# Ipsedo/MARLClassification

Measured on AMD Instinct MI355X. Metric: agent-env-steps/sec, higher is better.
Workload: dtype f32; 1 GPU; RESISC45 256x256x3, 16 agents, 16 steps, f=12, README dims (configs[2]); full train iteration: rollout + A2C loss + BPTT backward + Adam; batch_per_gpu=256, global_batch=256, parallelism=dp1, rng=library (Philox4x32-10), launch=eager

## Files before the change

include/marl_hip.h:

```cpp
#ifndef MARL_HIP_H
#define MARL_HIP_H

#include <stddef.h>
#include <stdint.h>

#ifdef __cplusplus
extern "C" {
#endif

#define MARL_ABI_VERSION 5

#define MARL_OK 0
#define MARL_EINVAL (-1)
#define MARL_ELIMIT (-2)
#define MARL_EHIP (-3)
#define MARL_ESIZE (-4)

#define MARL_COUNTERS_BYTES 32

#define MARL_MAX_CNN_LAYERS 5
#define MARL_MAX_ACTIONS 16

typedef struct marl_config {
    int32_t nb_agents;
// ... 55 lines not shown
int marl_graph_end(void* stream, void** graph_exec_out);
int marl_graph_launch(void* graph_exec, void* stream);
int marl_graph_destroy(void* graph_exec);

int marl_episode_forward(const marl_config* cfg, const void* weights_ws, size_t weights_ws_bytes,
                         void* episode_ws, size_t episode_ws_bytes,
                         const void* img, const int64_t* pos0,
                         const float* h0, const float* c0, const float* hc0, const float* cc0,
                         const float* noise, const int64_t* forced_actions,
                         uint64_t rng_seed, uint64_t rng_offset, const void* counters,
                         float* step_preds, float* step_logp, float* step_values,
                         int64_t* step_pos, int64_t* step_actions,
                         int train, void* stream);

int marl_episode_backward(const marl_config* cfg, void* weights_ws, size_t weights_ws_bytes,
                          void* episode_ws, size_t episode_ws_bytes,
                          const void* img, const float* g_preds, const float* g_logp,
                          const float* g_values, float* const* grads_host, void* stream);

int marl_episode_backward_img(const marl_config* cfg, void* weights_ws, size_t weights_ws_bytes,
                              void* episode_ws, size_t episode_ws_bytes,
                              const void* img, const float* g_preds, const float* g_logp,
                              const float* g_values, float* const* grads_host, float* d_img,
                              void* stream);

int marl_episode_forward_probs(const marl_config* cfg, const void* weights_ws, size_t weights_ws_bytes,
                               void* episode_ws, size_t episode_ws_bytes,
                               const void* img, const int64_t* pos0,
                               const float* h0, const float* c0, const float* hc0, const float* cc0,
                               const float* noise, const int64_t* forced_actions,
                               uint64_t rng_seed, uint64_t rng_offset, const void* counters,
                               float* step_preds, float* step_logp, float* step_values,
                               int64_t* step_pos, int64_t* step_actions, float* step_probs,
                               int train, void* stream);

int marl_episode_backward_probs(const marl_config* cfg, void* weights_ws, size_t weights_ws_bytes,
                                void* episode_ws, size_t episode_ws_bytes,
                                const void* img, const float* g_preds, const float* g_logp,
                                const float* g_values, float* const* grads_host, float* d_img,
                                const float* g_probs, void* stream);

int marl_backward_heads_event(void* hip_event);

int marl_comm_matrix(const float* m_dev, int nb_agents);

size_t marl_comm_grad_scratch_bytes(const marl_config* cfg);
int marl_comm_grad(const marl_config* cfg, const void* weights_ws, size_t weights_ws_bytes,
                   const void* ws, size_t ws_bytes, int nb_steps, float* d_comm,
                   void* scratch, size_t scratch_bytes, void* stream);

int marl_a2c_loss_fwd_bwd(const marl_config* cfg, void* episode_ws, size_t episode_ws_bytes,
                          const float* step_preds, const float* step_logp,
                          const float* step_values, const int64_t* y, float gamma,
                          float* g_preds, float* g_logp, float* g_values,
                          float* scalars_out, double* adv_stats, int phase, void* stream);

int marl_a2c_loss_entropy_fwd_bwd(const marl_config* cfg, void* episode_ws, size_t episode_ws_bytes,
                                  const float* step_preds, const float* step_logp,
                                  const float* step_values, const int64_t* y, float gamma,
                                  const float* step_probs, float entropy_coef,
                                  float* g_preds, float* g_logp, float* g_values, float* g_probs,
                                  float* scalars_out, double* adv_stats, int phase, void* stream);

int marl_advantages(const marl_config* cfg, void* episode_ws, size_t episode_ws_bytes,
                    const float* step_preds, const float* step_values, const int64_t* y,
                    float gamma, float lam, float* advn, float* ret, double* adv_stats, int phase,
                    void* stream);

int marl_ppo_loss_fwd_bwd(const marl_config* cfg, void* episode_ws, size_t episode_ws_bytes,
                          const float* step_preds, const float* step_logp, const float* step_values,
                          const int64_t* y, const float* old_logp, const float* advn, const float* ret,
                          float clip_eps, const float* step_probs, float entropy_coef,
                          float* g_preds, float* g_logp, float* g_values, float* g_probs,
                          float* scalars_out, void* stream);

#define MARL_GRAD_CLIP_BLOCKS 1024
#define MARL_GRAD_CLIP_SCRATCH_BYTES (MARL_GRAD_CLIP_BLOCKS * 8)
int marl_grad_clip(float* grads, int64_t n, float max_norm, float grad_scale, float* norm_out,
                   void* scratch, size_t scratch_bytes, void* stream);

int marl_adam_step(float* params, const float* grads, float* exp_avg, float* exp_avg_sq,
                   int64_t n, int64_t step, float lr, float beta1, float beta2, float eps,
                   float grad_scale, const void* counters, void* stream);

int marl_step_forward(const marl_config* cfg, const void* weights_ws, size_t weights_ws_bytes,
                      void* episode_ws, size_t episode_ws_bytes,
                      const float* obs, const float* msg, const float* norm_pos,
                      const float* h, const float* c, const float* hc, const float* cc,
                      float* probs, float* values, float* preds, float* new_msg,
                      float* h_out, float* c_out, float* hc_out, float* cc_out,
                      const float* noise, uint64_t rng_seed, uint64_t rng_offset,
                      int64_t* actions_out, float* logp_out, void* stream);

int marl_step_forward_train(const marl_config* cfg, const void* weights_ws, size_t weights_ws_bytes,
                            void* step_ws, size_t step_ws_bytes,
                            const float* obs, const float* msg, const float* norm_pos,
                            const float* h, const float* c, const float* hc, const float* cc,
                            float* probs, float* values, float* preds, float* new_msg,
                            float* h_out, float* c_out, float* hc_out, float* cc_out,
                            const float* noise, uint64_t rng_seed, uint64_t rng_offset,
                            int64_t* actions_out, float* logp_out, void* stream);

int marl_step_backward(const marl_config* cfg, void* weights_ws, size_t weights_ws_bytes,
                       void* step_ws, size_t step_ws_bytes, const float* obs,
                       const float* g_probs, const float* g_logp, const float* g_values,
                       const float* g_preds, const float* g_msg, const float* g_h, const float* g_c,
                       const float* g_hc, const float* g_cc, float* const* grads_host,
                       float* d_msg, float* d_h, float* d_c, float* d_hc, float* d_cc, void* stream);

int marl_normalize_positions(const int64_t* pos, float* out, int rows, int h, int w, void* stream);

int marl_gemm_nt(const float* a, int lda, const float* b, int ldb, const float* bias,
                 float* c, int ldc, int m, int n, int k, int accumulate, void* stream);
int marl_gemm_nt_weights(const float* a, int lda, const float* b, int ldb, const float* bias,
                         float* c, int ldc, int m, int n, int k, int accumulate,
                         void* image_scratch, void* stream);
size_t marl_gemm_weight_image_bytes(int n, int k);
int marl_gemm_tn(const float* a, int lda, const float* b, int ldb, float* c, int ldc,
                 int ni, int nj, int64_t rows, float* scratch, size_t scratch_bytes, void* stream);
size_t marl_gemm_tn_scratch(int ni, int nj, int64_t rows);
size_t marl_image_bytes(int64_t rows, int k);
int marl_image_build(const float* src, int ld, int64_t rows, int k, void* image, void* stream);
int marl_gemm_nt_images(const void* a3, const void* b3, const float* bias, float* c, int ldc, int m, int n,
                        int k, int accumulate, int variant, void* stream);
int marl_gemm_nt_images_batch(int count, const void* const* a3, const void* const* b3, float* const* c,
                              const int* n, const int* ldc, int m, int k, int accumulate, int variant,
                              void* stream);
int marl_lstm_images(const void* u3, int nin, const void* h3, const void* wih3, const void* whh3,
                     const float* bias, const float* c_prev, float* h_next, float* c_next, float* gates,
                     void* h3_next, int m, int n, int ld_state, int ld_gates, int variant, int cells,
                     void* stream);
size_t marl_gemm_tn_images_scratch(int ni, int nj, int64_t rows);
int marl_gemm_tn_images(const void* a3, const void* b3, float* c, int ldc, int ni, int nj, int64_t rows,
                        float* colsum, float* scratch, size_t scratch_bytes, void* stream);
size_t marl_gemm_tn_images_cell_scratch(int ni, int nih, int nhh, int64_t rows);
int marl_gemm_tn_images_cell(const void* g3, int ni, const void* u3, int nih, const void* h3, int nhh, int64_t rows,
                             float* c_ih, int ld_ih, float* c_hh, int ld_hh, float* colsum, float* scratch,
                             size_t scratch_bytes, void* stream);
int marl_ln_silu_fwd(const float* z, int ldz, const float* gamma, const float* beta,
                     float* out, int ldo, float* stats, int m, int n, void* stream);

int marl_cnn_wgrad(const float* dz, const void* img, int img_u8, const int32_t* pos,
                   const float* zin, const float* gst, const float* gamma, const float* beta,
                   int64_t rows, int nb, int c_img, int h, int w, int cin, int cout, int hin,
                   int groups, float* dw, float* db, float* scratch, size_t scratch_bytes,
                   void* stream);
size_t marl_cnn_wgrad_scratch(int64_t rows, int cin, int cout, int hin, int groups, int first);

int marl_tune(const char* key, int value);
int marl_tune_get(const char* key, int dflt);

int marl_profile_begin(int kernel_class, int max_launches);
int marl_profile_end(double* total_ms, int* launches);

int marl_debug_buffer(const marl_config* cfg, int train, const char* name, int t,
                      int64_t* offset_floats, int* ld);

int marl_plan_query(const marl_config* cfg, int train, const char* key, int* value);

#ifdef __cplusplus
}
#endif
#endif
```

marlclassification_amd/_lib.py:

```python

from __future__ import annotations

import ctypes as C
import os
from typing import Optional

MARL_MAX_CNN_LAYERS = 5
MARL_MAX_ACTIONS = 16
MARL_ABI_VERSION = 5
MARL_COUNTERS_BYTES = 32
MARL_GRAD_CLIP_SCRATCH_BYTES = 1024 * 8

_HERE = os.path.dirname(os.path.abspath(__file__))
LIB_PATH = os.environ.get("MARL_LIB_PATH") or os.path.join(_HERE, "csrc", "libmarl_hip.so")


class MarlConfig(C.Structure):

    _fields_ = [
        ("nb_agents", C.c_int32),
        ("batch", C.c_int32),
        ("nb_steps", C.c_int32),
        ("img_c", C.c_int32),
        ("img_h", C.c_int32),
        ("img_w", C.c_int32),
        ("window", C.c_int32),
        ("cnn_layers", C.c_int32),
        ("cnn_ch", C.c_int32 * (MARL_MAX_CNN_LAYERS + 1)),
        ("cnn_groups", C.c_int32 * MARL_MAX_CNN_LAYERS),
        ("n_b", C.c_int32),
        ("n_a", C.c_int32),
        ("n_m", C.c_int32),
        ("n_m_o", C.c_int32),
        ("n_d", C.c_int32),
        ("nb_action", C.c_int32),
        ("nb_class", C.c_int32),
        ("nlb", C.c_int32),
        ("nla", C.c_int32),
        ("actions", (C.c_int32 * 2) * MARL_MAX_ACTIONS),
        ("img_u8", C.c_int32),
    ]


_NAMES = (
    "POS_W POS_B POS_LNW POS_LNB "
    "ENC_W0 ENC_B0 ENC_LN0W ENC_LN0B ENC_W1 ENC_B1 ENC_LN1W ENC_LN1B "
    "DEC_W0 DEC_B0 DEC_LN0W DEC_LN0B DEC_W1 DEC_B1 DEC_LN1W DEC_LN1B "
    "LB_WIH LB_WHH LB_BIH LB_BHH LA_WIH LA_WHH LA_BIH LA_BHH "
    "POL_W0 POL_B0 POL_LNW POL_LNB POL_W1 POL_B1 "
    "CRI_W0 CRI_B0 CRI_LNW CRI_LNB CRI_W1 CRI_B1 "
    "PRE_W0 PRE_B0 PRE_LNW PRE_LNB PRE_W1 PRE_B1"
).split()
P = {name: 20 + i for i, name in enumerate(_NAMES)}
MARL_NPARAMS = 20 + len(_NAMES)

EXPORTS = (
    "marl_abi_version marl_last_error marl_param_numel marl_workspace_sizes marl_pack_weights "
    "marl_patch_gather marl_transition marl_episode_forward marl_episode_backward "
    "marl_a2c_loss_fwd_bwd marl_adam_step marl_step_forward marl_gemm_nt marl_gemm_tn "
    "marl_gemm_tn_scratch marl_gemm_nt_weights marl_gemm_weight_image_bytes marl_ln_silu_fwd marl_debug_buffer "
    "marl_profile_begin marl_profile_end marl_normalize_positions "
    "marl_cnn_wgrad marl_cnn_wgrad_scratch marl_tune marl_tune_get marl_draw_episode "
    "marl_counters_set marl_counters_tick marl_graph_begin marl_graph_end marl_graph_launch "
    "marl_graph_destroy marl_image_bytes marl_image_build marl_gemm_nt_images marl_gemm_nt_images_batch "
    "marl_lstm_images marl_gemm_tn_images marl_gemm_tn_images_scratch marl_plan_query "
    "marl_gemm_tn_images_cell marl_gemm_tn_images_cell_scratch marl_backward_heads_event "
    "marl_step_forward_train marl_step_backward marl_episode_backward_img "
    "marl_episode_forward_probs marl_episode_backward_probs marl_a2c_loss_entropy_fwd_bwd "
    "marl_advantages marl_ppo_loss_fwd_bwd marl_grad_clip marl_comm_matrix "
    "marl_comm_grad marl_comm_grad_scratch_bytes"
).split()

_lib: Optional[C.CDLL] = None

_vp, _i, _i64, _f, _sz = C.c_void_p, C.c_int, C.c_int64, C.c_float, C.c_size_t
_u64 = C.c_uint64
_cfgp = C.POINTER(MarlConfig)


def _declare(lib: C.CDLL) -> None:
    lib.marl_abi_version.restype = _i
    lib.marl_last_error.restype = C.c_char_p
    lib.marl_param_numel.restype = _i64
    lib.marl_param_numel.argtypes = [_cfgp, _i]
    lib.marl_workspace_sizes.argtypes = [_cfgp, _i, C.POINTER(_sz), C.POINTER(_sz)]
    lib.marl_pack_weights.argtypes = [_cfgp, C.POINTER(_vp), _vp, _sz, _vp]
    lib.marl_patch_gather.argtypes = [_vp, _vp, _vp, _i, _i, _i, _i, _i, _i, _vp]
    lib.marl_transition.argtypes = [_vp, _vp, _vp, C.POINTER(C.c_int32), _i, _i, _i, _i, _i, _vp]
    lib.marl_episode_forward.argtypes = ([_cfgp, _vp, _sz, _vp, _sz] + [_vp] * 8 + [_u64, _u64, _vp] + [_vp] * 5 +
                                         [_i, _vp])
    lib.marl_episode_forward_probs.argtypes = ([_cfgp, _vp, _sz, _vp, _sz] + [_vp] * 8 + [_u64, _u64, _vp] +
                                               [_vp] * 6 + [_i, _vp])
    lib.marl_draw_episode.argtypes = [_cfgp, _u64, _u64, _vp] + [_vp] * 7
    lib.marl_counters_set.argtypes = [_vp, _u64, _i64, _f, _f, _f, _vp]
    lib.marl_counters_tick.argtypes = [_vp, _f, _f, _f, _vp]
    lib.marl_graph_begin.argtypes = [_vp]
    lib.marl_graph_end.argtypes = [_vp, C.POINTER(_vp)]
    lib.marl_graph_launch.argtypes = [_vp, _vp]
    lib.marl_graph_destroy.argtypes = [_vp]
    lib.marl_episode_backward.argtypes = [_cfgp, _vp, _sz, _vp, _sz, _vp, _vp, _vp, _vp, C.POINTER(_vp), _vp]
    lib.marl_episode_backward_img.argtypes = ([_cfgp, _vp, _sz, _vp, _sz, _vp, _vp, _vp, _vp, C.POINTER(_vp), _vp,
                                               _vp])
    lib.marl_episode_backward_probs.argtypes = ([_cfgp, _vp, _sz, _vp, _sz, _vp, _vp, _vp, _vp, C.POINTER(_vp), _vp,
                                                 _vp, _vp])
    lib.marl_a2c_loss_entropy_fwd_bwd.argtypes = (
        [_cfgp, _vp, _sz, _vp, _vp, _vp, _vp, _f, _vp, _f, _vp, _vp, _vp, _vp, _vp, _vp, _i, _vp]
    )
    lib.marl_a2c_loss_fwd_bwd.argtypes = (
        [_cfgp, _vp, _sz, _vp, _vp, _vp, _vp, _f, _vp, _vp, _vp, _vp, _vp, _i, _vp]
    )
    lib.marl_advantages.argtypes = [_cfgp, _vp, _sz, _vp, _vp, _vp, _f, _f, _vp, _vp, _vp, _i, _vp]
    lib.marl_ppo_loss_fwd_bwd.argtypes = ([_cfgp, _vp, _sz] + [_vp] * 7 + [_f, _vp, _f] + [_vp] * 6)
    lib.marl_grad_clip.argtypes = [_vp, _i64, _f, _f, _vp, _vp, _sz, _vp]
    lib.marl_adam_step.argtypes = [_vp, _vp, _vp, _vp, _i64, _i64, _f, _f, _f, _f, _f, _vp, _vp]
    lib.marl_step_forward.argtypes = ([_cfgp, _vp, _sz, _vp, _sz] + [_vp] * 15 + [_vp, _u64, _u64, _vp, _vp] +
                                      [_vp])
    lib.marl_step_forward_train.argtypes = lib.marl_step_forward.argtypes
    lib.marl_step_backward.argtypes = [_cfgp, _vp, _sz, _vp, _sz] + [_vp] * 10 + [C.POINTER(_vp)] + [_vp] * 6
    lib.marl_normalize_positions.argtypes = [_vp, _vp, _i, _i, _i, _vp]
    lib.marl_gemm_nt.argtypes = [_vp, _i, _vp, _i, _vp, _vp, _i, _i, _i, _i, _i, _vp]
    lib.marl_gemm_nt_weights.argtypes = [_vp, _i, _vp, _i, _vp, _vp, _i, _i, _i, _i, _i, _vp, _vp]
    lib.marl_gemm_weight_image_bytes.restype = _sz
    lib.marl_gemm_weight_image_bytes.argtypes = [_i, _i]
    lib.marl_gemm_tn.argtypes = [_vp, _i, _vp, _i, _vp, _i, _i, _i, _i64, _vp, _sz, _vp]
    lib.marl_gemm_tn_scratch.restype = _sz
    lib.marl_gemm_tn_scratch.argtypes = [_i, _i, _i64]
    lib.marl_ln_silu_fwd.argtypes = [_vp, _i, _vp, _vp, _vp, _i, _vp, _i, _i, _vp]
    lib.marl_image_bytes.restype = _sz
    lib.marl_image_bytes.argtypes = [_i64, _i]
    lib.marl_image_build.argtypes = [_vp, _i, _i64, _i, _vp, _vp]
    lib.marl_gemm_nt_images.argtypes = [_vp, _vp, _vp, _vp, _i, _i, _i, _i, _i, _i, _vp]
    lib.marl_gemm_nt_images_batch.argtypes = [_i, C.POINTER(_vp), C.POINTER(_vp), C.POINTER(_vp), C.POINTER(_i),
                                              C.POINTER(_i), _i, _i, _i, _i, _vp]
    lib.marl_gemm_tn_images_scratch.restype = _sz
    lib.marl_gemm_tn_images_scratch.argtypes = [_i, _i, _i64]
    lib.marl_gemm_tn_images.argtypes = [_vp, _vp, _vp, _i, _i, _i, _i64, _vp, _vp, _sz, _vp]
    lib.marl_lstm_images.argtypes = [_vp, _i] + [_vp] * 9 + [_i] * 6 + [_vp]
    lib.marl_cnn_wgrad.argtypes = ([_vp, _vp, _i, _vp, _vp, _vp, _vp, _vp, _i64] + [_i] * 8 +
                                   [_vp, _vp, _vp, _sz, _vp])
    lib.marl_cnn_wgrad_scratch.restype = _sz
    lib.marl_cnn_wgrad_scratch.argtypes = [_i64, _i, _i, _i, _i, _i]
    lib.marl_tune.argtypes = [C.c_char_p, _i]
    lib.marl_tune_get.argtypes = [C.c_char_p, _i]
    lib.marl_profile_begin.argtypes = [_i, _i]
    lib.marl_profile_end.argtypes = [C.POINTER(C.c_double), C.POINTER(_i)]
    lib.marl_debug_buffer.argtypes = [_cfgp, _i, C.c_char_p, _i, C.POINTER(_i64), C.POINTER(_i)]
    lib.marl_gemm_tn_images_cell_scratch.restype = _sz
    lib.marl_gemm_tn_images_cell_scratch.argtypes = [_i, _i, _i, _i64]
    lib.marl_gemm_tn_images_cell.argtypes = [_vp, _i, _vp, _i, _vp, _i, _i64, _vp, _i, _vp, _i, _vp, _vp, _sz, _vp]
    lib.marl_plan_query.argtypes = [_cfgp, _i, C.c_char_p, C.POINTER(_i)]
    lib.marl_backward_heads_event.argtypes = [_vp]
    lib.marl_comm_matrix.argtypes = [_vp, _i]
    lib.marl_comm_grad_scratch_bytes.restype = _sz
    lib.marl_comm_grad_scratch_bytes.argtypes = [_cfgp]
    lib.marl_comm_grad.argtypes = [_cfgp, _vp, _sz, _vp, _sz, _i, _vp, _vp, _sz, _vp]
    for name in EXPORTS:
        fn = getattr(lib, name)
        if fn.restype is C.c_int and name not in ("marl_abi_version", "marl_tune_get"):
            fn.restype = _i


def load() -> C.CDLL:
    global _lib
    if _lib is not None:
        return _lib
    if not os.path.exists(LIB_PATH):
        raise RuntimeError(
            f"{LIB_PATH} is missing: the HIP library is the only implementation of this "
            "package (no CPU fallback). Build it with `make -C marlclassification_amd/csrc` "
            "or `python -c 'import __graft_entry__ as g; g.build()'`."
        )
    lib = C.CDLL(LIB_PATH)
    missing = [s for s in EXPORTS if not hasattr(lib, s)]
    if missing:
        raise RuntimeError(f"{LIB_PATH} lacks symbols {missing}")
    _declare(lib)
    if lib.marl_abi_version() != MARL_ABI_VERSION:
        raise RuntimeError("libmarl_hip.so ABI version mismatch; rebuild it")
    _lib = lib
    return lib


def check(rc: int) -> None:
    if rc != 0:
        msg = load().marl_last_error().decode("utf-8", "replace")
        raise RuntimeError(f"libmarl_hip error {rc}: {msg}")
```

marlclassification_amd/csrc/common.h:

```cpp
#pragma once

#include <hip/hip_runtime.h>
#include <stdint.h>
#include <stdio.h>

#include "../../include/marl_hip.h"
#include "split.h"

namespace marl {

constexpr int kWave = 64;

inline int p4(int x) { return (x + 3) & ~3; }
inline int64_t cdiv(int64_t a, int64_t b) { return (a + b - 1) / b; }

void set_error(const char* fmt, ...);

int tune_get(const char* key, int dflt);
int tune_set(const char* key, int value);

__device__ __forceinline__ float rcp_fast(float x) { return __builtin_amdgcn_rcpf(x); }
__device__ __forceinline__ float sigmoid_acc(float x) { return rcp_fast(1.0f + __expf(-x)); }
__device__ __forceinline__ float tanh_fast(float x) { return 1.0f - 2.0f * rcp_fast(1.0f + __expf(2.0f * x)); }
__device__ __forceinline__ float silu_fast(float y) { return y * sigmoid_acc(y); }
// ... 6 lines not shown
    int x = __float_as_int(v);
#define MARL_DPP_ADD(ctrl, rmask)                         \
    x = __float_as_int(__int_as_float(x) +                \
                       __int_as_float(__builtin_amdgcn_update_dpp(0, x, ctrl, rmask, 0xf, false)))
    MARL_DPP_ADD(0x111, 0xf);
    MARL_DPP_ADD(0x112, 0xf);
    MARL_DPP_ADD(0x114, 0xf);
    MARL_DPP_ADD(0x118, 0xf);
    MARL_DPP_ADD(0x142, 0xa);
    MARL_DPP_ADD(0x143, 0xc);
#undef MARL_DPP_ADD
    return __int_as_float(__builtin_amdgcn_readlane(x, 63));
}

#define MARL_HIP_CHECK(expr)                                                        \
    do {                                                                            \
        hipError_t e_ = (expr);                                                     \
        if (e_ != hipSuccess) {                                                     \
            marl::set_error("%s failed: %s (%s:%d)", #expr, hipGetErrorString(e_),  \
                            __FILE__, __LINE__);                                    \
            return MARL_EHIP;                                                       \
        }                                                                           \
    } while (0)

#define MARL_LAUNCH_CHECK() MARL_HIP_CHECK(hipGetLastError())

#define MARL_TRY(expr)             \
    do {                           \
        int rc_ = (expr);          \
        if (rc_ != MARL_OK) return rc_; \
    } while (0)

struct GemmSeg {
    const float* a;
    const float* b;
    int lda, ldb, k;
    const void* b3;
    int kt3;
};

struct GemmProb {
    GemmSeg seg[2];
    int nseg;
    int m, n;
    float* c;
    int ldc;
    const float* bias;
    int accumulate;
    const float* c_prev;
    float* h_next;
    float* c_next;
    float* gates;
    int ld_state, ld_gates;
};

constexpr int kMaxGemmBatch = 4;
struct GemmBatch {
    GemmProb p[kMaxGemmBatch];
    int count;
    int gx, gy;
    int xcd_map;
    int single_buf;
#ifdef MARL_KERNEL_TS
    long long* ts;
#endif
};

__device__ __forceinline__ void xcd_tile(unsigned gx, unsigned gy, unsigned gz, unsigned& bx,
                                         unsigned& by, unsigned& bz) {
    const unsigned T = gx * gy * gz, L = blockIdx.x;
    const unsigned per = T >> 3, rem = T & 7, xcd = L & 7, slot = L >> 3;
    const unsigned q = (xcd < rem ? xcd * (per + 1) : rem * (per + 1) + (xcd - rem) * per) + slot;
    bz = q / (gx * gy);
    const unsigned r = q - bz * gx * gy;
    bx = r / gy;
    by = r - bx * gy;
}
int xcd_map_enabled();

GemmProb gemm_prob(const float* a, int lda, const float* b, int ldb, int k, float* c, int ldc,
                   int m, int n, const float* bias = nullptr, int accumulate = 0);
void gemm_add_seg(GemmProb& p, const float* a, int lda, const float* b, int ldb, int k);

int launch_gemm_nt(const GemmBatch& batch, hipStream_t st);
int launch_gemm_lstm(const GemmBatch& batch, hipStream_t st);

int split_mode();
size_t split_image_floats(int rows, int k);
struct SplitDesc {
    const float* src;
    void* dst;
    int rows, k, ld, kt;
};
constexpr int kMaxSplitDesc = 64;
struct SplitBatch {
    SplitDesc d[kMaxSplitDesc];
    int count;
};
int launch_split_weights(const SplitBatch& b, hipStream_t st);
void split_registry_reset();
void split_registry_add(const float* base, int rows, int ld, int k, const void* image);
struct SplitRegistryScope {
    SplitRegistryScope() = default;
    SplitRegistryScope(const SplitRegistryScope&) = delete;
    ~SplitRegistryScope() { split_registry_reset(); }
};
int launch_gemm_nt_split(const GemmBatch& batch, int max_m, int max_n, int64_t blocks128, hipStream_t st);
int launch_gemm_lstm_split(const GemmBatch& batch, int max_m, int max_n, hipStream_t st);
int launch_gemm_tn_split(const float* a, int lda, const float* b, int ldb, float* out, int ldo,
                         int64_t stride, int ni, int nj, int64_t rows, int64_t rows_per_split,
                         float* csum, dim3 grid, int gx, int gy, int gz, hipStream_t st);

struct G3Seg {
    const char* a3;
    const char* b3;
    int a_row0, b_row0;
    int steps;
};
struct G3Prob {
    G3Seg seg[2];
    int nseg;
    int m, n;
    float* c;
    int ldc;
    const float* bias;
    int accumulate;
    const float* c_prev;
    float* h_next;
    float* c_next;
    float* gates;
    int ld_state, ld_gates;
    char* h3;
    int h3_row0, h3_steps;
};
constexpr int kMaxG3 = 4;
struct G3Batch {
    G3Prob p[kMaxG3];
    int count;
    int gx, gy, xcd_map;
    int safe;
#ifdef MARL_G3_ABLATE
    long long* clk;
#endif
};
G3Prob g3_prob(const void* a3, int a_row0, const void* b3, int b_row0, int k, float* c, int ldc, int m, int n,
               const float* bias = nullptr, int accumulate = 0);
void g3_add_seg(G3Prob& p, const void* a3, int a_row0, const void* b3, int b_row0, int k);
int launch_gemm_nt3(const G3Batch& batch, hipStream_t st, int variant = 0);
int launch_gemm_lstm3(const G3Batch& batch, hipStream_t st, int variant = 0);
int g3_lstm_plan(const G3Batch& batch);
struct G3TnArgs {
    const char* a3;
    const char* b3;
    int a_steps, b_steps;
    int a_row0, b_row0;
    float* out;
    int ldo;
    int64_t out_split_stride;
    int ni, nj;
    int64_t rows, rows_per_split;
    float* csum;
    int gx, gy, gz, safe;
    int j_first;
#ifdef MARL_G3_ABLATE
    int abl;
#endif
};
struct G3TnPlan {
    int variant, splits;
    int64_t rows_per_split;
};
G3TnPlan g3_tn_plan(int ni, int nj, int64_t rows);
constexpr int kMaxTnCell = 4;
struct G3TnCell {
    G3TnArgs t[kMaxTnCell];
    int nt, n256;
    int gx, gz;
    int teams;
};
bool g3_tn_cell_ok(int ni, int nj_ih, int nj_hh, int64_t rows);
G3TnPlan g3_tn_cell_plan(int ni, int nj_ih, int nj_hh, int64_t rows);
size_t g3_tn_cell_scratch_bytes(int ni, int nj_ih, int nj_hh, int64_t rows);
int launch_gemm_tn3_cell(G3TnArgs ih, G3TnArgs hh, const G3TnPlan& plan, hipStream_t st);
size_t g3_tn_scratch_bytes(int ni, int nj, int64_t rows);
int launch_gemm_tn3(G3TnArgs a, const G3TnPlan& plan, hipStream_t st);

struct ImgDesc {
    const float* src;
    void* dst;
    int64_t rows;
    int k, ld;
};
constexpr int kMaxImgDesc = 64;
struct ImgBatch {
    ImgDesc d[kMaxImgDesc];
    int count;
};
int launch_images(const ImgBatch& b, hipStream_t st);

constexpr int kProfClasses = 6;
void prof_before(int cls, hipStream_t st);
void prof_after(int cls, hipStream_t st);
int profile_begin(int cls, int max_launches);
int profile_end(double* total_ms, int* launches);

struct RedQueue;
size_t gemm_tn_scratch_bytes(int ni, int nj, int64_t rows);
struct TnQueue;
int launch_gemm_tn(const float* a, int lda, const float* b, int ldb, float* c, int ldc, int ni,
                   int nj, int64_t rows, float* scratch, size_t scratch_bytes, hipStream_t st,
                   float* colsum_out = nullptr, RedQueue* q = nullptr, TnQueue* tq = nullptr);

struct TnBatchProb {
    const float* a;
    const float* b;
    float* out;
    float* csum;
    int64_t stride, rows, rows_per_split;
    int lda, ldb, ldo, ni, nj, gx, gy, first_block;
};
constexpr int kMaxTnBatch = 12;
struct TnBatch {
    TnBatchProb p[kMaxTnBatch];
    int count;
};
struct TnQueue {
    struct Item {
        const float* a;
        const float* b;
        float* c;
        float* colsum;
// ... 43 lines not shown
                       float* dot_out = nullptr);
int ln_bwd_blocks(int64_t m, int n);
int launch_ln_silu_bwd_rank(const float* g, int ldg, int kin, const float* bt, int ldbt,
                            const float* z, int ldz, const float* stats, const float* gamma,
                            const float* beta, float* dz, int lddz, float* part, int64_t m, int n,
                            hipStream_t st);
int launch_ln_silu_bwd(const float* da, int ldda, const float* z, int ldz, const float* stats,
                       const float* gamma, const float* beta, float* dz, int lddz, float* part,
                       int64_t m, int n, hipStream_t st);
int launch_reduce_affine(float* part, int64_t nparts, int n, float* dgamma, float* dbeta,
                         int accumulate, hipStream_t st, RedQueue* q = nullptr);

int gn_fwd_im2col_supported(int P, int C);
int launch_gn_silu_fwd(const float* z, const float* gamma, const float* beta, float* out,
                       int64_t ldo, int out_chw, float* stats, int64_t rows, int P, int C, int G,
                       hipStream_t st, float* cols = nullptr, int ldk = 0, int hin = 0);
int gn_bwd_blocks(int64_t rows, int C);
int launch_gn_silu_bwd(const float* da, int64_t ldda, int da_chw, const float* z,
                       const float* stats, const float* gamma, const float* beta, float* dz,
                       float* part, int64_t rows, int P, int C, int G, hipStream_t st);

int launch_agg_msg(const float* m, float* out, int ld, int na, int nb, int n, hipStream_t st);
int launch_mix_msg(const float* m, float* out, int ld, int na, int nb, int n, const float* mix, int transpose,
                   hipStream_t st);
int mix_msg_max_agents();
int comm_grad_blocks(int64_t pairs, int* per_out);
int comm_grad_supported(int na, int n, int n2, int ldw);
int launch_comm_grad(const float* dz, int lddz, const float* msg, int ldmsg, const float* w, int ldw, int na, int nb,
                     int steps, int n2, int n, float* part, float* out, hipStream_t st);

int launch_pos_embed_fwd(const int32_t* pos, const float* npos_in, int h, int w, const float* W, const float* b,
                         const float* gamma, const float* beta, float* npos4, float* z, int ldz,
                         float* stats, float* out, int ldo, int64_t rows, int nd, hipStream_t st);

int launch_lstm_cell_bwd(const float* dh, int lddh, float* dc, int lddc, float* gates, int ldg,
                         const float* c_prev, const float* c_new, int ldc, int64_t rows, int n,
                         hipStream_t st);
struct LstmBwdBatch;
int launch_lstm_cell_bwd_batch(LstmBwdBatch& b, int count, hipStream_t st);
int launch_lstm_cell_bwd2(const float* dh0, int lddh0, float* dc0, int lddc0, float* gates0,
                          int ldg0, const float* cp0, const float* cn0, int ldc0, int n0,
                          const float* dh1, int lddh1, float* dc1, int lddc1, float* gates1,
                          int ldg1, const float* cp1, const float* cn1, int ldc1, int n1,
                          int64_t rows, hipStream_t st);

struct SampleArgs {
    const float* a_pol;
    int ld_a, nla;
    const float* w1;
    int ldw;
    const float* b1;
    const float* noise;
    uint64_t rng_seed, rng_ctr;
    const uint64_t* rng_off_dev;
    int rng_on;
    const int64_t* forced;
    const int32_t* pos_in;
    int32_t* pos_out;
    int64_t* step_pos;
    int64_t* step_actions;
    float* step_logp;
    float* probs;
    int32_t* actions_i32;
    int R, nA, H, W, f;
    int32_t table[MARL_MAX_ACTIONS][2];
    const float* pe_W;
    const float* pe_b;
    const float* pe_gamma;
    const float* pe_beta;
    float* pe_npos;
    float* pe_z;
    float* pe_stats;
    float* pe_out;
    int pe_ldz, pe_ldo, pe_nd;
    char* pe_img;
    int pe_row0, pe_steps, pe_col0;
};
int launch_sample(const SampleArgs& a, hipStream_t st);

int launch_draw_episode(uint64_t seed, uint64_t offset, const uint64_t* offset_dev, int64_t* pos0,
                        int R, int H, int W, int f, float* h0, float* c0, int n_b, float* hc0,
                        float* cc0, int n_a, float* noise, int64_t n_noise, hipStream_t st);

struct PermDesc {
    const float* src;
    float* dst;
    int rows, cols;
    int dst_ld;
    int rd, rs1, rs2;
    int cd, cs1, cs2;
    const float* src2;
};
constexpr int kMaxPerm = 56;
struct PermBatch {
    PermDesc d[kMaxPerm];
    int count;
};
int launch_permute(const PermBatch& b, hipStream_t st);

struct Counters {
    uint64_t rng_offset;
    uint64_t step;
    float lr_over_bc1;
    float inv_sqrt_bc2;
    float pad[2];
};
static_assert(sizeof(Counters) == MARL_COUNTERS_BYTES, "counter block layout");
int launch_counters_set(Counters* c, uint64_t rng_offset, int64_t step, float lr, float beta1,
                        float beta2, int tick, hipStream_t st);

int launch_adam(float* p, const float* g, float* m, float* v, int64_t n, float lr_over_bc1,
                float inv_sqrt_bc2, float beta1, float beta2, float eps, float grad_scale,
                hipStream_t st, const Counters* cnt = nullptr);

int launch_fill(float* p, int64_t n, float v, hipStream_t st);
int launch_add2d(const float* a, int64_t lda, const float* b, int64_t ldb, float* out, int64_t ldo,
                 int64_t rows, int cols, hipStream_t st);
int launch_copy2d(const float* src, int64_t lds, float* dst, int64_t ldd, int64_t rows, int cols,
                  hipStream_t st);
int launch_i64_to_i32(const int64_t* src, int32_t* dst, int64_t n, hipStream_t st);
int launch_policy_dlogits(const float* dlogp, const float* probs, const int32_t* actions,
                          float* out, int ld, int64_t rows, int nA, hipStream_t st);
int launch_policy_dlogits_probs(const float* dlogp, const float* dprobs, const float* probs,
                                const int32_t* actions, float* out, int ld, int64_t rows, int nA,
                                hipStream_t st);
int launch_acc2d(float* dst, int64_t ldd, const float* src, int64_t lds, int64_t rows, int cols,
                 hipStream_t st);
int launch_rowdot(const float* a, int lda, const float* w, const float* b, float* out,
                  int64_t rows, int n, hipStream_t st);

struct PanelLayer {
    const float* w;
    int ldw;
    const float* bias;
    const float* gamma;
    const float* beta;
    int n;
    float* z;
    int ldz;
    float* stats;
    float* a;
    int lda;
    char* a3;
    int a3_row0, a3_steps, a3_col0;
};
constexpr int kPanelMaxLayers = 4;
struct PanelFwdProb {
    const float* x;
    int ldx, k0;
    int agg_na, agg_nb;
    float* xbar;
    int m, nlayers;
    PanelLayer layer[kPanelMaxLayers];
    int by_batch, g_na, g_nb, agg_at, ld_xbar;
    const float* mix;
};
struct PanelFwdBatch {
    PanelFwdProb p[2];
    int count;
    int off_panel1, off_red, off_part, off_prm;
    int off_mix;
    int has_sample, panel_blocks;
    int epi_prob;
    int ln_narrow_max;
    SampleArgs sample;
#ifdef MARL_KERNEL_TS
    long long* ts;
#endif
};
int panel_chain_supported(int na, int n_msg, int threads);
int panel_supported(int k0, int n0, int n1);
int panel_sample_supported(int n_actions);
int launch_panel_fwd(PanelFwdBatch& b, hipStream_t st);

struct LstmBwdArgs {
    const float* dh;
    float* dc;
    float* gates;
    const float* c_prev;
    const float* c_new;
    int lddh, lddc, ldg, ldc, n;
// ... 312 lines not shown
```

marlclassification_amd/csrc/episode.hip:

```cpp
#include <math.h>
#include <stdlib.h>
#include <string.h>

#include "common.h"

namespace marl {

struct Dims {
    int na, nb, ns;
    int64_t R, NR;
    int H, W, c_img, f;
    int L;
    int ch[MARL_MAX_CNN_LAYERS + 1];
    int grp[MARL_MAX_CNN_LAYERS];
    int hw[MARL_MAX_CNN_LAYERS + 1];
    int P[MARL_MAX_CNN_LAYERS];
    int K[MARL_MAX_CNN_LAYERS];
    int ldk[MARL_MAX_CNN_LAYERS];
    int nf, nin;
    int n_b, n_a, n_m, nm2, n_mo, n_d, nA, nC, nlb, nla;
    int ld_nin, ld_nb, ld_na, ld_nm, ld_nm2, ld_nmo, ld_nd, ld_nla, ld_nlb, ld_gb, ld_ga, ld_nC,
        ld_nA;
    int ld_dbl;
};
// ... 814 lines not shown
    pe.x = c.Hs(t + 1);
    pe.ldx = d.ld_nb;
    pe.k0 = d.n_b;
    pe.m = (int)d.R;
    pe.nlayers = 2;
    pe.layer[0] = PanelLayer{c.wp(MARL_P_ENC_W0), d.ld_nb, c.wp(MARL_P_ENC_B0),
                             c.wp(MARL_P_ENC_LN0W), c.wp(MARL_P_ENC_LN0B), d.nm2,
                             keep ? c.at(c.e.ZE1, t) : nullptr, d.ld_nm2,
                             keep ? c.at(c.e.STE1, t) : nullptr, c.at(c.e.AE1, t), d.ld_nm2};
    pe.layer[1] = PanelLayer{c.wp(MARL_P_ENC_W1), d.ld_nm2, c.wp(MARL_P_ENC_B1),
                             c.wp(MARL_P_ENC_LN1W), c.wp(MARL_P_ENC_LN1B), d.n_m,
                             keep ? c.at(c.e.ZE2, t) : nullptr, d.ld_nm,
                             keep ? c.at(c.e.STE2, t) : nullptr, c.MSGs(t + 1), d.ld_nm};
}
static void fill_pol_prob(const Ctx& c, int t, PanelFwdProb& pp) {
    const Dims& d = c.d;
    const bool keep = c.train != 0;
    pp.x = c.HCs(t + 1);
    pp.ldx = d.ld_na;
    pp.k0 = d.n_a;
    pp.m = (int)d.R;
    pp.nlayers = 1;
    pp.layer[0] = PanelLayer{c.wp(MARL_P_POL_W0), d.ld_na, c.wp(MARL_P_POL_B0),
                             c.wp(MARL_P_POL_LNW), c.wp(MARL_P_POL_LNB), d.nla,
                             keep ? c.at(c.e.ZP1, t) : nullptr, d.ld_nla,
                             keep ? c.at(c.e.STP1, t) : nullptr, c.at(c.e.AP1, t), d.ld_nla};
}

static int step_encode_policy(const Ctx& c, int t, int which) {
    const Dims& d = c.d;
    const int R = (int)d.R;
    hipStream_t st = c.st;
    if (use_panels(d)) {
        PanelFwdBatch pb{};
        pb.count = 0;
        if (which & 1) fill_enc_prob(c, t, pb.p[pb.count++]);
        if (which & 2) fill_pol_prob(c, t, pb.p[pb.count++]);
        return launch_panel_fwd(pb, st);
    }
    if (which == 3) {
        MARL_TRY(gemm2(c,
                       gemm_prob(c.Hs(t + 1), d.ld_nb, c.wp(MARL_P_ENC_W0), d.ld_nb, d.n_b,
                                 c.at(c.e.ZE1, t), d.ld_nm2, R, d.nm2, c.wp(MARL_P_ENC_B0)),
                       gemm_prob(c.HCs(t + 1), d.ld_na, c.wp(MARL_P_POL_W0), d.ld_na, d.n_a,
                                 c.at(c.e.ZP1, t), d.ld_nla, R, d.nla, c.wp(MARL_P_POL_B0))));
    } else if (which == 1) {
        MARL_TRY(gemm1(c, gemm_prob(c.Hs(t + 1), d.ld_nb, c.wp(MARL_P_ENC_W0), d.ld_nb, d.n_b,
                                    c.at(c.e.ZE1, t), d.ld_nm2, R, d.nm2, c.wp(MARL_P_ENC_B0))));
    } else {
        MARL_TRY(gemm1(c, gemm_prob(c.HCs(t + 1), d.ld_na, c.wp(MARL_P_POL_W0), d.ld_na, d.n_a,
                                    c.at(c.e.ZP1, t), d.ld_nla, R, d.nla, c.wp(MARL_P_POL_B0))));
    }
    if (which & 2)
        MARL_TRY(launch_ln_silu_fwd(c.at(c.e.ZP1, t), d.ld_nla, c.wp(MARL_P_POL_LNW),
                                    c.wp(MARL_P_POL_LNB), c.at(c.e.AP1, t), d.ld_nla,
                                    c.at(c.e.STP1, t), d.R, d.nla, st));
    if (which & 1) {
        MARL_TRY(launch_ln_silu_fwd(c.at(c.e.ZE1, t), d.ld_nm2, c.wp(MARL_P_ENC_LN0W),
                                    c.wp(MARL_P_ENC_LN0B), c.at(c.e.AE1, t), d.ld_nm2,
                                    c.at(c.e.STE1, t), d.R, d.nm2, st));
        MARL_TRY(gemm1(c, gemm_prob(c.at(c.e.AE1, t), d.ld_nm2, c.wp(MARL_P_ENC_W1), d.ld_nm2,
                                    d.nm2, c.at(c.e.ZE2, t), d.ld_nm, R, d.n_m,
                                    c.wp(MARL_P_ENC_B1))));
        MARL_TRY(launch_ln_silu_fwd(c.at(c.e.ZE2, t), d.ld_nm, c.wp(MARL_P_ENC_LN1W),
                                    c.wp(MARL_P_ENC_LN1B), c.MSGs(t + 1), d.ld_nm,
                                    c.at(c.e.STE2, t), d.R, d.n_m, st));
    }
    return MARL_OK;
}

static bool use_chain(const Dims& d) {
    return use_panels(d) && panel_chain_supported(d.na, d.n_m, 256) && d.n_mo <= 384 && d.nm2 <= 384 &&
           d.n_m <= 384 && tune_get("panel_chain", 1) != 0 &&
           (!g_comm || d.n_b <= 384);
}
static bool use_panel_sample(const Dims& d) {
    static int enabled = -1;
    if (enabled < 0) {
        const char* e = getenv("MARL_PANEL_SAMPLE");
        enabled = (e && e[0] == '0') ? 0 : 1;
    }
    return enabled && panel_sample_supported(d.nA);
}
static int step_chain(const Ctx& c, int t, const SampleArgs* sample = nullptr) {
    const Dims& d = c.d;
    PanelFwdBatch pb{};
    pb.count = 2;
    PanelFwdProb& pe = pb.p[0];
    fill_enc_prob(c, t, pe);
    pe.by_batch = panel_chain_by_batch(d.na);
    pe.g_na = d.na;
    pe.g_nb = d.nb;
    if (t + 1 < d.ns) {
        fill_dec_layers(c, t + 1, pe.layer + 2);
        pe.nlayers = 4;
        pe.agg_at = 2;
        pe.xbar = c.at(c.e.MBAR, t + 1);
        pe.ld_xbar = d.ld_nm;
        pe.mix = g_comm;
    }
    fill_pol_prob(c, t, pb.p[1]);
    if (sample && use_panel_sample(d)) {
        pb.epi_prob = 2;
        pb.sample = *sample;
    }
    return launch_panel_fwd(pb, c.st);
}

static int step_core(const Ctx& c, int t, const StepIn& in) {
    MARL_TRY(step_cnn(c, t, in));
    MARL_TRY(step_decode(c, t));
    MARL_TRY(step_pos_lstm(c, t, in));
    return step_encode_policy(c, t, 3);
}

struct SideStream {
    hipStream_t s = nullptr;
    hipEvent_t ev[64];
    int next = 0;
    int init() {
        if (s) return MARL_OK;
        MARL_HIP_CHECK(hipStreamCreateWithFlags(&s, hipStreamNonBlocking));
        for (auto& e : ev) MARL_HIP_CHECK(hipEventCreateWithFlags(&e, hipEventDisableTiming));
        return MARL_OK;
    }
    int order(hipStream_t from, hipStream_t to) {
        hipEvent_t e = ev[next];
        next = (next + 1) % 64;
        MARL_HIP_CHECK(hipEventRecord(e, from));
        MARL_HIP_CHECK(hipStreamWaitEvent(to, e, 0));
        return MARL_OK;
    }
};
static SideStream g_side;

static bool use_side_stream() {
    static int enabled = -1;
    (void)enabled;
    return false;
}

static int heads_batched(const Ctx& c, int t0, int64_t rows, float* values, float* preds) {
    const Dims& d = c.d;
    hipStream_t st = c.st;
    if (c.e.g3 && tune_get("g3_lstm", 1) != 0) {
        const int r1 = (int)((int64_t)(t0 + 1) * d.R);
        G3Batch g{};
        g.p[0] = g3_prob(c.img(c.e.HC3), r1, c.wp3k(MARL_P_CRI_W0), 0, d.n_a, c.at(c.e.ZC1), d.ld_nla, (int)rows, d.nla,
                         c.wp(MARL_P_CRI_B0));
        g.p[1] = g3_prob(c.img(c.e.H3), r1, c.wp3k(MARL_P_PRE_W0), 0, d.n_b, c.at(c.e.ZQ1), d.ld_nlb, (int)rows, d.nlb,
                         c.wp(MARL_P_PRE_B0));
        g.count = 2;
        MARL_TRY(launch_gemm_nt3(g, st));
    } else
    MARL_TRY(gemm2(c,
                   gemm_prob(c.HCs(t0 + 1), d.ld_na, c.wp(MARL_P_CRI_W0), d.ld_na, d.n_a,
                             c.at(c.e.ZC1), d.ld_nla, (int)rows, d.nla, c.wp(MARL_P_CRI_B0)),
                   gemm_prob(c.Hs(t0 + 1), d.ld_nb, c.wp(MARL_P_PRE_W0), d.ld_nb, d.n_b,
                             c.at(c.e.ZQ1), d.ld_nlb, (int)rows, d.nlb, c.wp(MARL_P_PRE_B0))));
    const bool vdot = d.nla <= 384;
    MARL_TRY(launch_ln_silu_fwd(c.at(c.e.ZC1), d.ld_nla, c.wp(MARL_P_CRI_LNW), c.wp(MARL_P_CRI_LNB),
                                c.at(c.e.AC1), d.ld_nla, c.at(c.e.STC1), rows, d.nla, st,
                                vdot ? c.wp(MARL_P_CRI_W1) : nullptr, c.wp(MARL_P_CRI_B1), values));
    MARL_TRY(launch_ln_silu_fwd(c.at(c.e.ZQ1), d.ld_nlb, c.wp(MARL_P_PRE_LNW), c.wp(MARL_P_PRE_LNB),
                                c.at(c.e.AQ1), d.ld_nlb, c.at(c.e.STQ1), rows, d.nlb, st));
    if (!vdot)
// ... 69 lines not shown
static int load_state(const Ctx& c, const float* h, const float* cc_, const float* hc,
                      const float* cca, const float* msg) {
    const Dims& d = c.d;
    PermQueue q(c.st);
    q.push(copy_desc(h, d.n_b, c.Hs(0), d.ld_nb, d.R, d.n_b));
    q.push(copy_desc(cc_, d.n_b, c.Cs(0), d.ld_nb, d.R, d.n_b));
    q.push(copy_desc(hc, d.n_a, c.HCs(0), d.ld_na, d.R, d.n_a));
    q.push(copy_desc(cca, d.n_a, c.CCs(0), d.ld_na, d.R, d.n_a));
    q.push(copy_desc(msg, d.n_m, c.MSGs(0), d.ld_nm, d.R, msg ? d.n_m : d.ld_nm));
    q.flush();
    MARL_TRY(q.rc);
    if (c.e.g3) {
        ImgBatch ib{};
        ib.d[0] = ImgDesc{h, c.img(c.e.H3), d.R, d.n_b, d.n_b};
        ib.d[1] = ImgDesc{hc, c.img(c.e.HC3), d.R, d.n_a, d.n_a};
        ib.count = 2;
        MARL_TRY(launch_images(ib, c.st));
    }
    return MARL_OK;
}


static int pack_weights(const Dims& d, const WLayout& w, const float* const* params, float* W,
                        hipStream_t st) {
    PermQueue q(st);
    for (int i = 0; i < MARL_NPARAMS; ++i) {
        const ParamMeta m = param_meta(d, i);
        if (m.kind == PK_NONE) continue;
        const float* src = params[i];
        if (!src) {
            set_error("parameter %d is null", i);
            return MARL_EINVAL;
        }
        if (m.kind == PK_MATRIX) {
            q.push(perm(src, W + w.wp[i], m.n, m.k, w.ldp[i], 1, m.k, 0, 1, 1, 0));
            q.push(perm(src, W + w.wt[i], m.k, m.n, w.ldt[i], 1, 1, 0, 1, m.k, 0));
        } else if (m.kind == PK_CONV) {
            const int ci = m.k / 9;
            q.push(perm(src, W + w.wp[i], m.n, m.k, w.ldp[i], 1, m.k, 0, ci, 1, 9));
            q.push(perm(src, W + w.wt[i], m.k, m.n, w.ldt[i], ci, 1, 9, 1, m.k, 0));
        } else {
            q.push(perm(src, W + w.wp[i], 1, m.n, m.n, 1, 0, 0, 1, 1, 0));
        }
    }
    q.push(perm(params[MARL_P_LB_BIH], W + w.bsum_b, 1, 4 * d.n_b, 4 * d.n_b, 1, 0, 0, 1, 1, 0,
                params[MARL_P_LB_BHH]));
    q.push(perm(params[MARL_P_LA_BIH], W + w.bsum_a, 1, 4 * d.n_a, 4 * d.n_a, 1, 0, 0, 1, 1, 0,
                params[MARL_P_LA_BHH]));
    q.flush();
    MARL_TRY(q.rc);
    for (int i = 0; i < MARL_NPARAMS; ++i) {
        const ParamMeta m = param_meta(d, i);
        if (!w.wf[i]) continue;
        const int steps = m.k / 16;
        q.push(perm(W + w.wp[i], W + w.wf[i], (m.n / 16) * steps * 4, 64, 64, steps * 4, 16 * w.ldp[i], 4, 4,
                    w.ldp[i], 1));
    }
    q.flush();
    MARL_TRY(q.rc);
    SplitBatch sb{};
    sb.count = 0;
    for (int i = 0; i < MARL_NPARAMS; ++i) {
        const ParamMeta m = param_meta(d, i);
        if (m.kind != PK_MATRIX) continue;
        sb.d[sb.count++] = SplitDesc{W + w.wp[i], W + w.wp3[i], m.n, m.k, w.ldp[i], (m.k + 31) / 32};
        sb.d[sb.count++] = SplitDesc{W + w.wt[i], W + w.wt3[i], m.k, m.n, w.ldt[i], (m.n + 31) / 32};
    }
    MARL_TRY(launch_split_weights(sb, st));
    ImgBatch ib{};
    ib.count = 0;
    for (int i = 0; i < MARL_NPARAMS; ++i) {
        const ParamMeta m = param_meta(d, i);
        if (m.kind != PK_MATRIX || !w.wp3k[i]) continue;
        if (ib.count + 2 > kMaxImgDesc) {
            MARL_TRY(launch_images(ib, st));
            ib.count = 0;
        }
        ib.d[ib.count++] = ImgDesc{W + w.wp[i], W + w.wp3k[i], m.n, m.k, w.ldp[i]};
        ib.d[ib.count++] = ImgDesc{W + w.wt[i], W + w.wt3k[i], m.k, m.n, w.ldt[i]};
    }
    return launch_images(ib, st);
}

static void register_split_images(const Dims& d, const WLayout& w, const float* W) {
    split_registry_reset();
    for (int i = 0; i < MARL_NPARAMS; ++i) {
        const ParamMeta m = param_meta(d, i);
        if (m.kind != PK_MATRIX) continue;
        split_registry_add(W + w.wp[i], m.n, w.ldp[i], m.k, W + w.wp3[i]);
        split_registry_add(W + w.wt[i], m.k, w.ldt[i], m.n, W + w.wt3[i]);
    }
}

static int unpack_grads(const Ctx& c, float* const* grads, int which = 0) {
    PermQueue q(c.st);
    for (int i = 0; i < MARL_NPARAMS; ++i) {
        const bool head = i >= MARL_P_POL_W0 && i <= MARL_P_PRE_B1;
        if ((which == 1 && !head) || (which == 2 && head)) continue;
        const ParamMeta m = param_meta(c.d, i);
        if (m.kind == PK_MATRIX) {
            q.push(perm(c.gp(i), grads[i], m.n, m.k, m.k, 1, c.w.ldp[i], 0, 1, 1, 0));
        } else if (m.kind == PK_CONV) {
            const int ci = m.k / 9;
            q.push(perm(c.gp(i), grads[i], m.n, m.k, m.k, 1, c.w.ldp[i], 0, 9, 1, ci));
        }
    }
    if (which != 1) {
        q.push(perm(grads[MARL_P_LB_BIH], grads[MARL_P_LB_BHH], 1, 4 * c.d.n_b, 4 * c.d.n_b, 1, 0, 0, 1, 1, 0));
        q.push(perm(grads[MARL_P_LA_BIH], grads[MARL_P_LA_BHH], 1, 4 * c.d.n_a, 4 * c.d.n_a, 1, 0, 0, 1, 1, 0));
    }
    q.flush();
    return q.rc;
}

static int tn(const Ctx& c, const float* a, int lda, const float* b, int ldb, int pidx, int ni,
              int nj, int64_t rows, float* bias = nullptr) {
    RedQueue* q = c.defer_this(gemm_tn_scratch_bytes(ni, nj, rows)) ? c.rq : nullptr;
    return launch_gemm_tn(a, lda, b, ldb, c.gp(pidx), c.w.ldp[pidx], ni, nj, rows, c.at(c.e.TNS),
                          c.e.tns_bytes, c.st, bias, q, q ? c.tq : nullptr);
}
static int tn3(const Ctx& c, const char* a3, int ni, const char* b3, int nj, int pidx, int64_t rows, float* bias) {
    const G3TnPlan plan = g3_tn_plan(ni, nj, rows);
    if (g3_tn_scratch_bytes(ni, nj, rows) > c.e.tns_bytes) {
        set_error("tn3: scratch too small");
        return MARL_ESIZE;
    }
    float* scratch = c.at(c.e.TNS);
    G3TnArgs a{};
    a.a3 = a3;
    a.b3 = b3;
    a.a_steps = img_steps(ni);
    a.b_steps = img_steps(nj);
    a.out = scratch;
    a.ldo = nj;
    a.out_split_stride = (int64_t)ni * nj;
    a.ni = ni;
    a.nj = nj;
    a.rows = rows;
    a.csum = bias ? scratch + (size_t)plan.splits * ni * nj : nullptr;
    MARL_TRY(launch_gemm_tn3(a, plan, c.st));
    return launch_slab_reduce(scratch, (int64_t)ni * nj, plan.splits, c.gp(pidx), c.w.ldp[pidx], ni, nj, a.csum, bias, c.st);
}
static int tn3_cell(const Ctx& c, const char* g3, int ni, const char* u3, int nin, int p_ih, const char* h3, int nh,
                    int p_hh, int64_t rows, float* bias) {
    const G3TnPlan plan = g3_tn_cell_plan(ni, nin, nh, rows);
    if (g3_tn_cell_scratch_bytes(ni, nin, nh, rows) > c.e.tns_bytes) {
        set_error("tn3_cell: scratch too small");
        return MARL_ESIZE;
    }
    float* s_ih = c.at(c.e.TNS);
    float* s_hh = s_ih + (size_t)plan.splits * ni * nin;
    float* s_cs = s_hh + (size_t)plan.splits * ni * nh;
    G3TnArgs ih{}, hh{};
    ih.a3 = hh.a3 = g3;
    ih.a_steps = hh.a_steps = img_steps(ni);
    ih.ni = hh.ni = ni;
    ih.rows = hh.rows = rows;
    ih.b3 = u3;
    ih.b_steps = img_steps(nin);
    ih.nj = ih.ldo = nin;
    ih.out = s_ih;
    ih.out_split_stride = (int64_t)ni * nin;
    ih.csum = bias ? s_cs : nullptr;
    hh.b3 = h3;
    hh.b_steps = img_steps(nh);
    hh.nj = hh.ldo = nh;
// ... 129 lines not shown
                                    c.at(c.e.DAP1), d.ld_nla, (int)NR, d.nla)));
        MARL_TRY(ln_bwd(c, c.at(c.e.DAP1), d.ld_nla, c.at(c.e.ZP1, 0), d.ld_nla, c.at(c.e.STP1, 0),
                        MARL_P_POL_LNW, MARL_P_POL_LNB, NR, d.nla, grads, 0));
    }
    MARL_TRY(tn(c, c.at(c.e.DAP1), d.ld_nla, c.HCs(1), d.ld_na, MARL_P_POL_W0, d.nla, d.n_a, NR, grads[MARL_P_POL_B0]));
    {
        GemmProb ph = gemm_prob(c.at(c.e.DAQ1), d.ld_nlb, c.wt(MARL_P_PRE_W0), d.ld_nlb, d.nlb,
                                c.DHs(1), d.ld_nb, (int)NR, d.n_b);
        GemmProb pa = gemm_prob(c.at(c.e.DAP1), d.ld_nla, c.wt(MARL_P_POL_W0), d.ld_nla, d.nla,
                                c.DHCs(1), d.ld_na, (int)NR, d.n_a);
        gemm_add_seg(pa, c.at(c.e.DAC1), d.ld_nla, c.wt(MARL_P_CRI_W0), d.ld_nla, d.nla);
        MARL_TRY(gemm2(c, ph, pa));
    }
    if (sb) {
        MARL_TRY(launch_acc2d(c.DHs(ns), d.ld_nb, sb->g_h, d.n_b, d.R, d.n_b, st));
        MARL_TRY(launch_acc2d(c.DHCs(ns), d.ld_na, sb->g_hc, d.n_a, d.R, d.n_a, st));
    }

    const bool heads_early = g_heads_event != nullptr && !sb;
    if (heads_early) {
        if (c.tq) MARL_TRY(launch_tn_queue(tq, c.rq, st));
        MARL_TRY(rq.flush());
        MARL_TRY(unpack_grads(c, grads, 1));
        MARL_HIP_CHECK(hipEventRecord(g_heads_event, st));
    }

    const size_t s_nmo = (size_t)d.R * d.ld_dbl, s_nm2 = (size_t)d.R * d.ld_nm2,
                 s_nm = (size_t)d.R * d.ld_nm;
    const bool panels = use_panels(d) && d.n_mo <= 384 && d.nm2 <= 384 && d.n_m <= 384;
    if (!panels) {
        MARL_TRY(launch_tn_queue(tq, c.rq, st));
        c.rq = nullptr;
        c.tq = nullptr;
    }
    const bool enc_last = sb && sb->g_msg;
    if (enc_last) {
        const int t = ns - 1;
        float* dze2 = c.at(c.e.DZE2) + (size_t)t * s_nm;
        float* dae1 = c.at(c.e.DAE1) + (size_t)t * s_nm2;
        MARL_TRY(launch_copy2d(sb->g_msg, d.n_m, dze2, d.ld_nm, d.R, d.n_m, st));
        MARL_TRY(ln_bwd(c, dze2, d.ld_nm, c.at(c.e.ZE2, t), d.ld_nm, c.at(c.e.STE2, t), MARL_P_ENC_LN1W,
                        MARL_P_ENC_LN1B, d.R, d.n_m, grads, 0));
        MARL_TRY(gemm1(c, gemm_prob(dze2, d.ld_nm, c.wt(MARL_P_ENC_W1), p4(d.n_m), d.n_m, dae1, d.ld_nm2, R,
                                    d.nm2)));
        MARL_TRY(ln_bwd(c, dae1, d.ld_nm2, c.at(c.e.ZE1, t), d.ld_nm2, c.at(c.e.STE1, t), MARL_P_ENC_LN0W,
                        MARL_P_ENC_LN0B, d.R, d.nm2, grads, 0));
        MARL_TRY(gemm1(c, gemm_prob(dae1, d.ld_nm2, c.wt(MARL_P_ENC_W0), p4(d.nm2), d.nm2, c.DHs(ns), d.ld_nb, R,
                                    d.n_b, nullptr, 1)));
    }
    const bool ride = panels && !use_side_stream();
    const bool dl_in_loop = ride;
    bool action_done = false;
    bool belief_done = false;
    const bool chain = ride && use_chain(d);
    const bool g3 = c.e.g3;
    const int skip_f32 = g3 && dl_in_loop && g3_tn_enabled(d);
    const int pln_blocks = chain ? panel_chain_blocks(d.na, d.nb) : panel_bwd_blocks(R);
    for (int t = ns - 1; t >= 0; --t) {
        const int first = (t == ns - 1);
        {
            LstmBwdBatch lb{};
            int nc = 0;
            if (!belief_done)
                lb.a[nc++] = LstmBwdArgs{c.DHs(t + 1), c.at(c.e.DC), c.at(c.e.GB, t), c.Cs(t), c.Cs(t + 1), d.ld_nb,
                                         d.ld_nb, d.ld_gb, d.ld_nb, d.n_b, g3 ? c.img(c.e.GB3) : nullptr,
                                         (int)((int64_t)t * d.R), img_steps(4 * d.n_b), skip_f32};
            if (!action_done)
                lb.a[nc++] = LstmBwdArgs{c.DHCs(t + 1), c.at(c.e.DCC), c.at(c.e.GA, t), c.CCs(t), c.CCs(t + 1), d.ld_na,
                                         d.ld_na, d.ld_ga, d.ld_na, d.n_a, g3 ? c.img(c.e.GA3) : nullptr,
                                         (int)((int64_t)t * d.R), img_steps(4 * d.n_a), skip_f32};
            lb.rows = d.R;
            if (nc) MARL_TRY(launch_lstm_cell_bwd_batch(lb, nc, st));
        }
        action_done = belief_done = false;
        const bool side = panels && use_side_stream();
        Ctx cs = c;
        if (side) {
            MARL_TRY(g_side.init());
            cs.st = g_side.s;
            MARL_TRY(g_side.order(c.st, cs.st));
        }
        hipStream_t st = cs.st;
        float* ddbar = c.at(c.e.DDBAR) + (size_t)t * s_nmo;
        {
            GemmBatch gb{};
            gb.p[0] = gemm_prob(c.at(c.e.GB, t), d.ld_gb, c.wt(MARL_P_LB_WHH), d.ld_gb, 4 * d.n_b,
                                c.DHs(t), d.ld_nb, R, d.n_b, nullptr, 1);
            gb.p[1] = gemm_prob(c.at(c.e.GA, t), d.ld_ga, c.wt(MARL_P_LA_WHH), d.ld_ga, 4 * d.n_a,
                                c.DHCs(t), d.ld_na, R, d.n_a, nullptr, 1);
            GemmProb p = gemm_prob(c.at(c.e.GB, t), d.ld_gb,
                                   c.wt(MARL_P_LB_WIH) + (size_t)d.nf * d.ld_gb, d.ld_gb, 4 * d.n_b,
                                   ddbar, d.ld_dbl, R, d.n_mo);
            gemm_add_seg(p, c.at(c.e.GA, t), d.ld_ga, c.wt(MARL_P_LA_WIH) + (size_t)d.nf * d.ld_ga,
                         d.ld_ga, 4 * d.n_a);
            if (side) {
                gb.count = 2;
                MARL_TRY(launch_gemm_nt(gb, c.st));
                MARL_TRY(gemm1(cs, p));
            } else if (dl_in_loop) {
                gb.p[2] = gemm_prob(c.at(c.e.GB, t), d.ld_gb,
                                    c.wt(MARL_P_LB_WIH) + (size_t)d.nf * d.ld_gb, d.ld_gb, 4 * d.n_b,
                                    ddbar, d.ld_dbl, R, d.n_mo + d.n_d);
                gb.p[3] = gemm_prob(c.at(c.e.GA, t), d.ld_ga,
                                    c.wt(MARL_P_LA_WIH) + (size_t)d.nf * d.ld_ga, d.ld_ga, 4 * d.n_a,
                                    c.at(c.e.DDBAR2) + (size_t)t * s_nmo, d.ld_dbl, R, d.n_mo + d.n_d);
                gb.count = 4;
                if (g3) {
                    const int r0 = (int)((int64_t)t * d.R);
                    G3Batch g{};
                    g.p[0] = g3_prob(c.img(c.e.GB3), r0, c.wt3k(MARL_P_LB_WHH), 0, 4 * d.n_b, c.DHs(t), d.ld_nb, R,
                                     d.n_b, nullptr, 1);
                    g.p[1] = g3_prob(c.img(c.e.GA3), r0, c.wt3k(MARL_P_LA_WHH), 0, 4 * d.n_a, c.DHCs(t), d.ld_na, R,
                                     d.n_a, nullptr, 1);
                    g.p[2] = g3_prob(c.img(c.e.GB3), r0, c.wt3k(MARL_P_LB_WIH), d.nf, 4 * d.n_b, ddbar, d.ld_dbl, R,
                                     d.n_mo + d.n_d);
                    g.p[3] = g3_prob(c.img(c.e.GA3), r0, c.wt3k(MARL_P_LA_WIH), d.nf, 4 * d.n_a,
                                     c.at(c.e.DDBAR2) + (size_t)t * s_nmo, d.ld_dbl, R, d.n_mo + d.n_d);
                    g.count = 4;
                    MARL_TRY(launch_gemm_nt3(g, c.st));
                } else {
                    MARL_TRY(launch_gemm_nt(gb, c.st));
                }
            } else {
                gb.p[2] = p;
                gb.count = 3;
                MARL_TRY(launch_gemm_nt(gb, c.st));
            }
        }
        float* dad1 = c.at(c.e.DAD1) + (size_t)t * s_nm2;
        if (panels) {
            const size_t pblk = (size_t)pln_blocks * 2;
            PanelBwdProb pd{};
            pd.da = ddbar;
            pd.ldda = d.ld_dbl;
            if (dl_in_loop) {
                pd.da2 = c.at(c.e.DDBAR2) + (size_t)t * s_nmo;
                pd.ldda2 = d.ld_dbl;
            }
            pd.m = R;
            pd.nlayers = 2;
            pd.layer[0] = PanelBwdLayer{c.at(c.e.ZD2, t), d.ld_nmo, c.at(c.e.STD2, t),
                                        c.wp(MARL_P_DEC_LN1W), c.wp(MARL_P_DEC_LN1B), d.n_mo, ddbar,
                                        d.ld_dbl, c.at(c.e.PLN[0]) + (size_t)t * pblk * d.n_mo,
                                        c.wt(MARL_P_DEC_W1), p4(d.n_mo), d.nm2};
            pd.layer[1] = PanelBwdLayer{c.at(c.e.ZD1, t), d.ld_nm2, c.at(c.e.STD1, t),
                                        c.wp(MARL_P_DEC_LN0W), c.wp(MARL_P_DEC_LN0B), d.nm2, dad1,
                                        d.ld_nm2, c.at(c.e.PLN[1]) + (size_t)t * pblk * d.nm2,
                                        c.wt(MARL_P_DEC_W0), p4(d.nm2), d.n_m};
            pd.dx = c.at(c.e.DMBAR);
            pd.lddx = d.ld_nm;
            pd.accumulate = 0;
            if (ride && t > 0) {
                pd.has_cell = 1;
                pd.cell = LstmBwdArgs{c.DHCs(t), c.at(c.e.DCC), c.at(c.e.GA, t - 1), c.CCs(t - 1),
                                      c.CCs(t), d.ld_na, d.ld_na, d.ld_ga, d.ld_na, d.n_a,
                                      g3 ? c.img(c.e.GA3) : nullptr, (int)((int64_t)(t - 1) * d.R), img_steps(4 * d.n_a),
                                      skip_f32};
                pd.cell_rows = d.R;
                action_done = true;
            }
            if (chain) {
                pd.by_batch = panel_chain_by_batch(d.na);
                pd.g_na = d.na;
                pd.g_nb = d.nb;
                if (t > 0) {
                    pd.nlayers = 4;
                    pd.agg_at = 2;
                    pd.mix = g_comm;
                    pd.layer[2] = PanelBwdLayer{c.at(c.e.ZE2, t - 1), d.ld_nm, c.at(c.e.STE2, t - 1),
                                                c.wp(MARL_P_ENC_LN1W), c.wp(MARL_P_ENC_LN1B), d.n_m,
                                                c.at(c.e.DZE2) + (size_t)(t - 1) * s_nm, d.ld_nm,
                                                c.at(c.e.PLN[2]) + (size_t)(t - 1) * pblk * d.n_m,
                                                c.wt(MARL_P_ENC_W1), p4(d.n_m), d.nm2};
                    pd.layer[3] = PanelBwdLayer{c.at(c.e.ZE1, t - 1), d.ld_nm2, c.at(c.e.STE1, t - 1),
                                                c.wp(MARL_P_ENC_LN0W), c.wp(MARL_P_ENC_LN0B), d.nm2,
                                                c.at(c.e.DAE1) + (size_t)(t - 1) * s_nm2, d.ld_nm2,
                                                c.at(c.e.PLN[3]) + (size_t)(t - 1) * pblk * d.nm2,
                                                c.wt(MARL_P_ENC_W0), p4(d.nm2), d.n_b};
                    pd.dx = c.DHs(t);
                    pd.lddx = d.ld_nb;
                    pd.accumulate = 1;
                    pd.has_cellb = 1;
                    pd.cellb = LstmBwdArgs{c.DHs(t), c.at(c.e.DC), c.at(c.e.GB, t - 1), c.Cs(t - 1), c.Cs(t),
                                           d.ld_nb, d.ld_nb, d.ld_gb, d.ld_nb, d.n_b, g3 ? c.img(c.e.GB3) : nullptr,
                                           (int)((int64_t)(t - 1) * d.R), img_steps(4 * d.n_b), skip_f32};
                    belief_done = true;
                }
                MARL_TRY(launch_panel_bwd(pd, st));
                MARL_TRY(gate_image_fallback(c, pd, t - 1));
                continue;
            }
            MARL_TRY(launch_panel_bwd(pd, st));
            MARL_TRY(gate_image_fallback(c, pd, t - 1));
            if (t > 0) {
                float* dze2 = c.at(c.e.DZE2) + (size_t)(t - 1) * s_nm;
                float* dae1 = c.at(c.e.DAE1) + (size_t)(t - 1) * s_nm2;
                PanelBwdProb pe{};
                pe.da = c.at(c.e.DMBAR);
                pe.ldda = d.ld_nm;
                pe.agg_na = d.na;
                pe.agg_nb = d.nb;
                if (g_comm) {
                    MARL_TRY(launch_mix_msg(c.at(c.e.DMBAR), c.at(c.e.DMBAR), d.ld_nm, d.na, d.nb, d.ld_nm, g_comm,
                                            1, st));
                    pe.agg_na = pe.agg_nb = 0;
                }
                pe.m = R;
                pe.nlayers = 2;
                pe.layer[0] = PanelBwdLayer{c.at(c.e.ZE2, t - 1), d.ld_nm, c.at(c.e.STE2, t - 1),
// ... 297 lines not shown
    }
    WLayout w;
    make_wlayout(d, w);
    if (weights_ws_bytes < w.total * sizeof(float)) {
        set_error("pack_weights: weights workspace too small (%zu of %zu bytes)", weights_ws_bytes,
                  w.total * sizeof(float));
        return MARL_ESIZE;
    }
    return pack_weights(d, w, params_host, static_cast<float*>(weights_ws),
                        static_cast<hipStream_t>(stream));
}

int marl_patch_gather(const float* img, const int64_t* pos, float* obs, int nb_agents, int batch,
                      int c, int h, int w, int f, void* stream) {
    if (!img || !pos || !obs || nb_agents < 1 || batch < 1 || c < 1 || f < 1 || h < f || w < f) {
        set_error("patch_gather: bad argument");
        return MARL_EINVAL;
    }
    return launch_patch_gather(img, pos, obs, nb_agents, batch, c, h, w, f,
                               static_cast<hipStream_t>(stream));
}

}

namespace marl {
__global__ void transition_kernel(const int64_t* __restrict__ pos_in,
                                  const int64_t* __restrict__ actions,
                                  int64_t* __restrict__ pos_out, SampleArgs tbl, int rows, int nA,
                                  int H, int W, int f) {
    const int r = blockIdx.x * blockDim.x + threadIdx.x;
    if (r >= rows) return;
    int a = (int)actions[r];
    a = a < 0 ? 0 : (a >= nA ? nA - 1 : a);
    const int64_t p0 = pos_in[r * 2], p1 = pos_in[r * 2 + 1];
    const int64_t q0 = p0 + tbl.table[a][0], q1 = p1 + tbl.table[a][1];
    const bool ok = q0 >= 0 && q0 + f < H && q1 >= 0 && q1 + f < W;
    pos_out[r * 2] = ok ? q0 : p0;
    pos_out[r * 2 + 1] = ok ? q1 : p1;
}
}

extern "C" {

int marl_transition(const int64_t* pos_in, const int64_t* actions, int64_t* pos_out,
                    const int32_t* table_host, int nb_action, int rows, int h, int w, int f,
                    void* stream) {
    if (!pos_in || !actions || !pos_out || !table_host || nb_action < 1 ||
        nb_action > MARL_MAX_ACTIONS || rows < 1) {
        set_error("transition: bad argument");
        return MARL_EINVAL;
    }
    SampleArgs tbl;
    memset(&tbl, 0, sizeof(tbl));
    for (int j = 0; j < nb_action; ++j) {
        tbl.table[j][0] = table_host[2 * j];
        tbl.table[j][1] = table_host[2 * j + 1];
    }
    hipLaunchKernelGGL(transition_kernel, dim3((unsigned)cdiv(rows, 256)), dim3(256), 0,
                       static_cast<hipStream_t>(stream), pos_in, actions, pos_out, tbl, rows,
                       nb_action, h, w, f);
    MARL_LAUNCH_CHECK();
    return MARL_OK;
}

static int episode_forward_all(const marl_config* cfg, const void* weights_ws, size_t weights_ws_bytes,
                               void* episode_ws, size_t episode_ws_bytes, const void* img, const int64_t* pos0,
                               const float* h0, const float* c0, const float* hc0, const float* cc0,
                               const float* noise, const int64_t* forced_actions, uint64_t rng_seed,
                               uint64_t rng_offset, const void* counters, float* step_preds, float* step_logp,
                               float* step_values, int64_t* step_pos, int64_t* step_actions, float* step_probs,
                               int train, void* stream) {
    Ctx c;
    SplitRegistryScope reg_scope;
    MARL_TRY(make_ctx(cfg, weights_ws, weights_ws_bytes, episode_ws, episode_ws_bytes, train, stream, c));
    if (!img || !pos0 || !h0 || !c0 || !hc0 || !cc0 || !step_preds || !step_logp || !step_values) {
        set_error("episode_forward: null argument");
        return MARL_EINVAL;
    }
    if (c.d.ns >= 65536) {
        set_error("episode_forward: more than 65535 steps");
        return MARL_ELIMIT;
    }
    const Dims& d = c.d;
    MARL_TRY(launch_i64_to_i32(pos0, c.POSs(0), d.R * 2, c.st));
    MARL_TRY(load_state(c, h0, c0, hc0, cc0, nullptr));
    StepIn in;
    in.img = img;
    in.img_u8 = cfg->img_u8 != 0;
    const bool side = use_side_stream();
    Ctx c2 = c;
    if (side) {
        MARL_TRY(g_side.init());
        c2.st = g_side.s;
    }
    bool decoded_ahead = false;
    const bool chain = !side && use_chain(d);
    for (int t = 0; t < d.ns; ++t) {
        MARL_TRY(step_cnn(c, t, in));
        if (side && t > 0)
            MARL_TRY(g_side.order(c2.st, c.st));
        else if (!decoded_ahead)
            MARL_TRY(step_decode(c, t));
        MARL_TRY(step_pos_lstm(c, t, in, t > 0));
        SampleArgs a;
        fill_sample_args(c, cfg, t, a);
        a.noise = noise ? noise + (size_t)t * d.R * d.nA : nullptr;
        a.rng_on = !noise && !forced_actions;
        a.rng_seed = rng_seed ^ 0x9E3779B97F4A7C15ull;
        a.rng_ctr = (rng_offset << 16) + (uint64_t)t;
        a.rng_off_dev = counters ? &static_cast<const Counters*>(counters)->rng_offset : nullptr;
        a.forced = forced_actions ? forced_actions + (size_t)t * d.R : nullptr;
        a.step_pos = step_pos ? step_pos + (size_t)t * d.R * 2 : nullptr;
        a.step_actions = step_actions ? step_actions + (size_t)t * d.R : nullptr;
        a.step_logp = step_logp + (size_t)t * d.R;
        if (t + 1 < d.ns) {
            a.pe_W = c.wp(MARL_P_POS_W);
            a.pe_b = c.wp(MARL_P_POS_B);
            a.pe_gamma = c.wp(MARL_P_POS_LNW);
            a.pe_beta = c.wp(MARL_P_POS_LNB);
            a.pe_npos = c.at(c.e.NPOS, t + 1);
            a.pe_z = c.at(c.e.ZPOS, t + 1);
            a.pe_stats = c.at(c.e.STPOS, t + 1);
            a.pe_out = c.at(c.e.U, t + 1) + d.nf + d.n_mo;
            a.pe_ldz = d.ld_nd;
            a.pe_ldo = d.ld_nin;
            a.pe_nd = d.n_d;
            if (c.u3_by_producers) {
                a.pe_img = c.img(c.e.U3);
                a.pe_row0 = c.u3_row(t + 1);
                a.pe_steps = img_steps(d.nin);
                a.pe_col0 = d.nf + d.n_mo;
            }
        }
        if (chain) {
            MARL_TRY(step_chain(c, t, &a));
        } else if (side) {
            MARL_TRY(g_side.order(c.st, c2.st));
            MARL_TRY(step_encode_policy(c2, t, 1));
            if (t + 1 < d.ns) MARL_TRY(step_decode(c2, t + 1));
            MARL_TRY(step_encode_policy(c, t, 2));
        } else {
            MARL_TRY(step_encode_policy(c, t, 3));
        }
        decoded_ahead = chain && t + 1 < d.ns;
        if (!side && !chain && t + 1 < d.ns) MARL_TRY(step_decode(c, t + 1, &a, &decoded_ahead));
        if (chain ? !use_panel_sample(d) : !decoded_ahead) MARL_TRY(launch_sample(a, c.st));
    }
    if (side) MARL_TRY(g_side.order(c2.st, c.st));
    MARL_TRY(heads_batched(c, 0, d.NR, step_values, step_preds));
    if (step_probs) MARL_TRY(launch_copy2d(c.PROBSs(0), d.nA, step_probs, d.nA, d.NR, d.nA, c.st));
    return MARL_OK;
}

int marl_episode_forward(const marl_config* cfg, const void* weights_ws, size_t weights_ws_bytes,
                         void* episode_ws, size_t episode_ws_bytes, const void* img, const int64_t* pos0, const float* h0, const float* c0,
                         const float* hc0, const float* cc0, const float* noise,
                         const int64_t* forced_actions, uint64_t rng_seed, uint64_t rng_offset,
                         const void* counters, float* step_preds, float* step_logp,
                         float* step_values, int64_t* step_pos, int64_t* step_actions, int train,
                         void* stream) {
    return episode_forward_all(cfg, weights_ws, weights_ws_bytes, episode_ws, episode_ws_bytes, img, pos0, h0, c0,
                               hc0, cc0, noise, forced_actions, rng_seed, rng_offset, counters, step_preds,
                               step_logp, step_values, step_pos, step_actions, nullptr, train, stream);
}

int marl_episode_forward_probs(const marl_config* cfg, const void* weights_ws, size_t weights_ws_bytes,
                               void* episode_ws, size_t episode_ws_bytes, const void* img, const int64_t* pos0,
                               const float* h0, const float* c0, const float* hc0, const float* cc0,
                               const float* noise, const int64_t* forced_actions, uint64_t rng_seed,
                               uint64_t rng_offset, const void* counters, float* step_preds, float* step_logp,
                               float* step_values, int64_t* step_pos, int64_t* step_actions, float* step_probs,
                               int train, void* stream) {
    if (!step_probs) {
        set_error("episode_forward_probs: null step_probs");
        return MARL_EINVAL;
    }
    return episode_forward_all(cfg, weights_ws, weights_ws_bytes, episode_ws, episode_ws_bytes, img, pos0, h0, c0,
                               hc0, cc0, noise, forced_actions, rng_seed, rng_offset, counters, step_preds,
                               step_logp, step_values, step_pos, step_actions, step_probs, train, stream);
}

static int episode_backward_entry(const char* who, bool need_dimg, const marl_config* cfg, void* weights_ws,
                                  size_t weights_ws_bytes, void* episode_ws, size_t episode_ws_bytes, const void* img,
                                  const float* g_preds, const float* g_logp, const float* g_values,
                                  float* const* grads_host, float* d_img, const float* g_probs, void* stream) {
    Ctx c;
// ... 258 lines not shown
                          float gamma, float* g_preds, float* g_logp, float* g_values,
                          float* scalars_out, double* adv_stats, int phase, void* stream) {
    return a2c_loss_all(cfg, episode_ws, episode_ws_bytes, false, "a2c_loss", step_preds, step_logp, step_values, y,
                        gamma, nullptr, 0.f, g_preds, g_logp, g_values, nullptr, scalars_out, adv_stats, phase,
                        stream);
}

int marl_a2c_loss_entropy_fwd_bwd(const marl_config* cfg, void* episode_ws, size_t episode_ws_bytes,
                                  const float* step_preds, const float* step_logp, const float* step_values,
                                  const int64_t* y, float gamma, const float* step_probs, float entropy_coef,
                                  float* g_preds, float* g_logp, float* g_values, float* g_probs,
                                  float* scalars_out, double* adv_stats, int phase, void* stream) {
    return a2c_loss_all(cfg, episode_ws, episode_ws_bytes, !step_probs || !g_probs || !(entropy_coef >= 0.f),
                        "a2c_loss_entropy", step_preds, step_logp, step_values, y, gamma, step_probs, entropy_coef,
                        g_preds, g_logp, g_values, g_probs, scalars_out, adv_stats, phase, stream);
}

int marl_advantages(const marl_config* cfg, void* episode_ws, size_t episode_ws_bytes, const float* step_preds,
                    const float* step_values, const int64_t* y, float gamma, float lam, float* advn, float* ret,
                    double* adv_stats, int phase, void* stream) {
    AdvArgs a;
    MARL_TRY(loss_entry(cfg, episode_ws, episode_ws_bytes,
                        !episode_ws || !step_preds || !step_values || !y || !advn || !ret || !adv_stats ||
                            phase < 0 || phase > 2 || !(lam >= 0.f && lam <= 1.f),
                        "advantages", step_preds, step_values, y, a));
    a.advn = advn;
    a.ret = ret;
    a.adv_stats = adv_stats;
    a.gamma = gamma;
    a.lam = lam;
    a.phase = phase;
    return launch_advantages(a, static_cast<hipStream_t>(stream));
}

int marl_ppo_loss_fwd_bwd(const marl_config* cfg, void* episode_ws, size_t episode_ws_bytes,
                          const float* step_preds, const float* step_logp, const float* step_values,
                          const int64_t* y, const float* old_logp, const float* advn, const float* ret,
                          float clip_eps, const float* step_probs, float entropy_coef, float* g_preds, float* g_logp,
                          float* g_values, float* g_probs, float* scalars_out, void* stream) {
    PpoArgs a;
    MARL_TRY(loss_entry(cfg, episode_ws, episode_ws_bytes,
                        !episode_ws || !step_preds || !step_logp || !step_values || !y || !old_logp || !advn ||
                            !ret || !scalars_out || !(clip_eps > 0.f) ||
                            (step_probs == nullptr) != (g_probs == nullptr) ||
                            (step_probs && !(entropy_coef >= 0.f)),
                        "ppo_loss", step_preds, step_values, y, a));
    fill_loss_grads(a, cfg, step_logp, step_probs, entropy_coef, g_preds, g_logp, g_values, g_probs, scalars_out);
    a.old_logp = old_logp;
    a.advn = advn;
    a.ret = ret;
    a.clip_eps = clip_eps;
    return launch_ppo_loss(a, static_cast<hipStream_t>(stream));
}

int marl_grad_clip(float* grads, int64_t n, float max_norm, float grad_scale, float* norm_out, void* scratch,
                   size_t scratch_bytes, void* stream) {
    if (!grads || n < 0 || !(max_norm > 0.f) || !(grad_scale > 0.f) || !norm_out || !scratch ||
        (reinterpret_cast<uintptr_t>(scratch) & 7) != 0) {
        set_error("grad_clip: bad argument");
        return MARL_EINVAL;
    }
    if (scratch_bytes < MARL_GRAD_CLIP_SCRATCH_BYTES) {
        set_error("grad_clip: scratch too small (%zu of %d bytes)", scratch_bytes, MARL_GRAD_CLIP_SCRATCH_BYTES);
        return MARL_ESIZE;
    }
    return launch_grad_clip(grads, n, max_norm, grad_scale, norm_out, static_cast<double*>(scratch),
                            static_cast<hipStream_t>(stream));
}

int marl_adam_step(float* params, const float* grads, float* exp_avg, float* exp_avg_sq, int64_t n,
                   int64_t step, float lr, float beta1, float beta2, float eps, float grad_scale,
                   const void* counters, void* stream) {
    if (!params || !grads || !exp_avg || !exp_avg_sq || n < 0 || step < 1) {
        set_error("adam: bad argument");
        return MARL_EINVAL;
    }
    const double bc1 = 1.0 - pow((double)beta1, (double)step);
    const double bc2 = 1.0 - pow((double)beta2, (double)step);
    return launch_adam(params, grads, exp_avg, exp_avg_sq, n, (float)((double)lr / bc1),
                       (float)(1.0 / sqrt(bc2)), beta1, beta2, eps, grad_scale,
                       static_cast<hipStream_t>(stream), static_cast<const Counters*>(counters));
}

}

static int step_forward(const marl_config* cfg, const void* weights_ws, size_t weights_ws_bytes, void* episode_ws,
                        size_t episode_ws_bytes, const float* obs, const float* msg, const float* norm_pos,
                        const float* h, const float* cc_, const float* hc, const float* cca, float* probs,
                        float* values, float* preds, float* new_msg, float* h_out, float* c_out, float* hc_out,
                        float* cc_out, const float* noise, uint64_t rng_seed, uint64_t rng_offset,
                        int64_t* actions_out, float* logp_out, int train, void* stream) {
    Ctx c;
    SplitRegistryScope reg_scope;
    MARL_TRY(make_ctx(cfg, weights_ws, weights_ws_bytes, episode_ws, episode_ws_bytes, train, stream, c));
    if (!obs || !msg || !norm_pos || !h || !cc_ || !hc || !cca || !probs || !values || !preds ||
        !new_msg || !h_out || !c_out || !hc_out || !cc_out) {
        set_error("step_forward: null argument");
        return MARL_EINVAL;
    }
    const Dims& d = c.d;
    MARL_TRY(load_state(c, h, cc_, hc, cca, msg));
    StepIn in;
    in.obs = obs;
    in.npos = norm_pos;
    MARL_TRY(step_core(c, 0, in));
    SampleArgs a;
    fill_sample_args(c, cfg, 0, a);
    a.probs = probs;
    if (actions_out && logp_out) {
        a.noise = noise;
        a.rng_on = !noise;
        a.rng_seed = rng_seed ^ 0x9E3779B97F4A7C15ull;
        a.rng_ctr = rng_offset << 16;
        a.step_actions = actions_out;
        a.step_logp = logp_out;
    } else {
        a.step_logp = nullptr;
    }
    MARL_TRY(launch_sample(a, c.st));
    MARL_TRY(heads_batched(c, 0, d.R, values, preds));
    MARL_TRY(launch_copy2d(c.MSGs(1), d.ld_nm, new_msg, d.n_m, d.R, d.n_m, c.st));
    MARL_TRY(launch_copy2d(c.Hs(1), d.ld_nb, h_out, d.n_b, d.R, d.n_b, c.st));
    MARL_TRY(launch_copy2d(c.Cs(1), d.ld_nb, c_out, d.n_b, d.R, d.n_b, c.st));
    MARL_TRY(launch_copy2d(c.HCs(1), d.ld_na, hc_out, d.n_a, d.R, d.n_a, c.st));
    MARL_TRY(launch_copy2d(c.CCs(1), d.ld_na, cc_out, d.n_a, d.R, d.n_a, c.st));
    if (train)
        MARL_TRY(launch_copy2d(probs, d.nA, c.PROBSs(0), d.nA, d.R, d.nA, c.st));
    return MARL_OK;
}

extern "C" {

int marl_step_forward(const marl_config* cfg, const void* weights_ws, size_t weights_ws_bytes,
                      void* episode_ws, size_t episode_ws_bytes, const float* obs, const float* msg, const float* norm_pos, const float* h,
                      const float* cc_, const float* hc, const float* cca, float* probs,
                      float* values, float* preds, float* new_msg, float* h_out, float* c_out,
                      float* hc_out, float* cc_out, const float* noise, uint64_t rng_seed,
                      uint64_t rng_offset, int64_t* actions_out, float* logp_out, void* stream) {
    return step_forward(cfg, weights_ws, weights_ws_bytes, episode_ws, episode_ws_bytes, obs, msg, norm_pos, h, cc_,
                        hc, cca, probs, values, preds, new_msg, h_out, c_out, hc_out, cc_out, noise, rng_seed,
                        rng_offset, actions_out, logp_out, 0, stream);
}

int marl_step_forward_train(const marl_config* cfg, const void* weights_ws, size_t weights_ws_bytes,
                            void* step_ws, size_t step_ws_bytes, const float* obs, const float* msg,
                            const float* norm_pos, const float* h, const float* c, const float* hc,
                            const float* cc, float* probs, float* values, float* preds, float* new_msg,
                            float* h_out, float* c_out, float* hc_out, float* cc_out, const float* noise,
                            uint64_t rng_seed, uint64_t rng_offset, int64_t* actions_out, float* logp_out,
                            void* stream) {
    if (!cfg) {
        set_error("step_forward_train: null configuration");
        return MARL_EINVAL;
    }
    marl_config one = *cfg;
    one.nb_steps = 1;
    return step_forward(&one, weights_ws, weights_ws_bytes, step_ws, step_ws_bytes, obs, msg, norm_pos, h, c, hc, cc,
                        probs, values, preds, new_msg, h_out, c_out, hc_out, cc_out, noise, rng_seed, rng_offset,
                        actions_out, logp_out, 1, stream);
}

int marl_step_backward(const marl_config* cfg, void* weights_ws, size_t weights_ws_bytes, void* step_ws,
                       size_t step_ws_bytes, const float* obs, const float* g_probs, const float* g_logp,
                       const float* g_values, const float* g_preds, const float* g_msg, const float* g_h,
                       const float* g_c, const float* g_hc, const float* g_cc, float* const* grads_host,
                       float* d_msg, float* d_h, float* d_c, float* d_hc, float* d_cc, void* stream) {
// ... 260 lines not shown
```

marlclassification_amd/csrc/gemm.hip:

```cpp
#include <stdlib.h>

#include "common.h"

namespace marl {

typedef float f32x16 __attribute__((ext_vector_type(16)));

constexpr int BK = 32;



__device__ __forceinline__ void lds_barrier() {
    asm volatile("s_waitcnt lgkmcnt(0)\n\ts_barrier" ::: "memory");
}

template <int BM, int BN, int WM, int WN, bool LSTM, int GROUPS>
__global__ __launch_bounds__(256 * GROUPS) void gemm_nt_kernel(const GemmBatch batch) {
    constexpr int BK = 32;
    constexpr int LDS_K = BK + 4;
    constexpr int KC = BK / 4;
    constexpr int TM = BM / WM / 32;
    constexpr int TN = BN / WN / 32;
    constexpr int A_CH = BM * KC / 256;
    constexpr int B_CH = BN * KC / 256 / GROUPS;
// ... 744 lines not shown
int RedQueue::launch_pending() {
    if (rc == MARL_OK && stage1.count) rc = launch_red_batch(stage1, st);
    if (rc == MARL_OK && stage2.count) rc = launch_red_batch(stage2, st);
    stage1.count = stage2.count = 0;
    return rc;
}

int RedQueue::flush() {
    (void)launch_pending();
    off = 0;
    return rc;
}

GemmProb gemm_prob(const float* a, int lda, const float* b, int ldb, int k, float* c, int ldc,
                   int m, int n, const float* bias, int accumulate) {
    GemmProb p{};
    p.seg[0] = GemmSeg{a, b, lda, ldb, k};
    p.nseg = 1;
    p.m = m;
    p.n = n;
    p.c = c;
    p.ldc = ldc;
    p.bias = bias;
    p.accumulate = accumulate;
    return p;
}

void gemm_add_seg(GemmProb& p, const float* a, int lda, const float* b, int ldb, int k) {
    p.seg[1] = GemmSeg{a, b, lda, ldb, k};
    p.nseg = 2;
}


template <int BM, int BN, int WM, int WN, bool LSTM, int GROUPS>
static int launch_nt_variant(dim3 grid, const GemmBatch& batch_in, hipStream_t st) {
    GemmBatch batch = batch_in;
    batch.gx = (int)grid.x;
    batch.gy = (int)grid.y;
    batch.xcd_map = xcd_map_enabled() || (batch.count == 1 && !LSTM && tune_get("nt_xcd", 1));
    if (batch.xcd_map) grid = dim3(grid.x * grid.y * grid.z);
    constexpr size_t lds2 = (size_t)2 * (GROUPS * BM + BN) * (32 + 4) * sizeof(float);
    batch.single_buf = GROUPS == 1 && !LSTM && BM == 128 && true;
    const size_t lds = batch.single_buf ? lds2 / 2 : lds2;
    auto kern = gemm_nt_kernel<BM, BN, WM, WN, LSTM, GROUPS>;
    if (lds2 > 64 * 1024) {
        static bool raised = false;
        if (!raised) {
            MARL_HIP_CHECK(hipFuncSetAttribute(reinterpret_cast<const void*>(kern),
                                               hipFuncAttributeMaxDynamicSharedMemorySize, (int)lds2));
            raised = true;
        }
    }
    hipLaunchKernelGGL(kern, grid, dim3(256 * GROUPS), lds, st, batch);
    return MARL_OK;
}

int xcd_map_enabled() { return 0; }

static int gemm_groups() { return 1; }

static int check_prob(const GemmProb& p) {
    for (int s = 0; s < p.nseg; ++s) {
        const GemmSeg& g = p.seg[s];
        if (!g.a || !g.b || g.k <= 0 || (g.lda & 3) || (g.ldb & 3) ||
            (reinterpret_cast<uintptr_t>(g.a) & 15) || (reinterpret_cast<uintptr_t>(g.b) & 15) ||
            g.lda < p4(g.k) || g.ldb < p4(g.k)) {
            set_error("gemm: bad operand (seg %d: a=%p lda=%d b=%p ldb=%d k=%d)", s, (const void*)g.a,
                      g.lda, (const void*)g.b, g.ldb, g.k);
            return MARL_EINVAL;
        }
        const int64_t brows = p.h_next ? 4 * (int64_t)p.n : (int64_t)p.n;
        if ((int64_t)p.m * g.lda >= (1ll << 30) || brows * g.ldb >= (1ll << 30)) {
            set_error("gemm: operand of seg %d spans more than 4 GiB", s);
            return MARL_ELIMIT;
        }
    }
    if (p.m <= 0 || p.n <= 0) {
        set_error("gemm: empty problem m=%d n=%d", p.m, p.n);
        return MARL_EINVAL;
    }
    return MARL_OK;
}

int launch_gemm_nt(const GemmBatch& batch, hipStream_t st) {
    if (batch.count < 1 || batch.count > kMaxGemmBatch) return MARL_EINVAL;
    int max_m = 0, max_n = 0;
    int64_t blocks128 = 0;
    for (int i = 0; i < batch.count; ++i) {
        MARL_TRY(check_prob(batch.p[i]));
        if (!batch.p[i].c) return MARL_EINVAL;
        max_m = batch.p[i].m > max_m ? batch.p[i].m : max_m;
        max_n = batch.p[i].n > max_n ? batch.p[i].n : max_n;
        blocks128 += cdiv(batch.p[i].m, 128) * cdiv(batch.p[i].n, 128);
    }
    static const bool log_shapes = getenv("MARL_GEMM_LOG") != nullptr;
    if (log_shapes)
        for (int i = 0; i < batch.count; ++i)
            fprintf(stderr, "[gemm_nt] %d/%d m=%d n=%d k=%d+%d acc=%d bias=%d lda=%d ldc=%d\n", i,
                    batch.count, batch.p[i].m, batch.p[i].n, batch.p[i].seg[0].k,
                    batch.p[i].nseg > 1 ? batch.p[i].seg[1].k : 0, batch.p[i].accumulate,
                    batch.p[i].bias != nullptr, batch.p[i].seg[0].lda, batch.p[i].ldc);
    prof_before(1, st);
    if (split_mode()) {
        MARL_TRY(launch_gemm_nt_split(batch, max_m, max_n, blocks128, st));
    } else if (blocks128 >= 256 && max_n >= 96) {
        const int g = gemm_groups();
        dim3 grid((unsigned)cdiv(max_m, 128 * g), (unsigned)cdiv(max_n, 128), (unsigned)batch.count);
        if (g == 2)
            MARL_TRY((launch_nt_variant<128, 128, 2, 2, false, 2>(grid, batch, st)));
        else
            MARL_TRY((launch_nt_variant<128, 128, 2, 2, false, 1>(grid, batch, st)));
    } else {
        const int g = gemm_groups();
        dim3 grid((unsigned)cdiv(max_m, 64 * g), (unsigned)cdiv(max_n, 64), (unsigned)batch.count);
        if (g == 2)
            MARL_TRY((launch_nt_variant<64, 64, 2, 2, false, 2>(grid, batch, st)));
        else
            MARL_TRY((launch_nt_variant<64, 64, 2, 2, false, 1>(grid, batch, st)));
    }
    prof_after(1, st);
    MARL_LAUNCH_CHECK();
    return MARL_OK;
}

static int g_prof_class = -1;
static int g_prof_cap = 0, g_prof_n = 0;
static hipEvent_t* g_prof_ev = nullptr;

void prof_before(int cls, hipStream_t st) {
    if (cls == g_prof_class && g_prof_n < g_prof_cap) (void)hipEventRecord(g_prof_ev[2 * g_prof_n], st);
}
void prof_after(int cls, hipStream_t st) {
    if (cls == g_prof_class && g_prof_n < g_prof_cap) {
        (void)hipEventRecord(g_prof_ev[2 * g_prof_n + 1], st);
        ++g_prof_n;
    }
}

int profile_begin(int cls, int max_launches) {
    if (g_prof_ev) return MARL_EINVAL;
    g_prof_ev = new hipEvent_t[2 * (size_t)max_launches];
    for (int i = 0; i < 2 * max_launches; ++i) MARL_HIP_CHECK(hipEventCreate(&g_prof_ev[i]));
    g_prof_cap = max_launches;
    g_prof_n = 0;
    g_prof_class = cls;
    return MARL_OK;
}

int profile_end(double* total_ms, int* launches) {
    if (!g_prof_ev) return MARL_EINVAL;
    double tot = 0.0;
    for (int i = 0; i < g_prof_n; ++i) {
        MARL_HIP_CHECK(hipEventSynchronize(g_prof_ev[2 * i + 1]));
        float ms = 0.f;
        MARL_HIP_CHECK(hipEventElapsedTime(&ms, g_prof_ev[2 * i], g_prof_ev[2 * i + 1]));
        tot += ms;
    }
    for (int i = 0; i < 2 * g_prof_cap; ++i) (void)hipEventDestroy(g_prof_ev[i]);
    delete[] g_prof_ev;
    g_prof_ev = nullptr;
    if (total_ms) *total_ms = tot;
    if (launches) *launches = g_prof_n;
    g_prof_class = -1;
    g_prof_cap = g_prof_n = 0;
    return MARL_OK;
}

int launch_gemm_lstm(const GemmBatch& batch, hipStream_t st) {
    if (batch.count < 1 || batch.count > kMaxGemmBatch) return MARL_EINVAL;
    int max_m = 0, max_n = 0;
    for (int i = 0; i < batch.count; ++i) {
        const GemmProb& p = batch.p[i];
        MARL_TRY(check_prob(p));
        if (!p.bias || !p.c_prev || !p.h_next || !p.c_next) return MARL_EINVAL;
        max_m = p.m > max_m ? p.m : max_m;
        max_n = p.n > max_n ? p.n : max_n;
    }
    const int g = gemm_groups();
    dim3 grid((unsigned)cdiv(max_m, 128 * g), (unsigned)cdiv(max_n, 32), (unsigned)batch.count);
    prof_before(0, st);
    if (split_mode())
        MARL_TRY(launch_gemm_lstm_split(batch, max_m, max_n, st));
    else if (g == 2)
        MARL_TRY((launch_nt_variant<128, 128, 4, 1, true, 2>(grid, batch, st)));
    else
        MARL_TRY((launch_nt_variant<128, 128, 4, 1, true, 1>(grid, batch, st)));
    prof_after(0, st);
    MARL_LAUNCH_CHECK();
// ... 177 lines not shown
```

marlclassification_amd/csrc/gemm3.hip:

```cpp
#include <stdlib.h>

#include "common.h"
#include "split.h"

namespace marl {

typedef float f32x16 __attribute__((ext_vector_type(16)));
typedef short bf16x8 __attribute__((ext_vector_type(8)));
typedef __attribute__((address_space(3))) void* lds_ptr;

namespace {

template <int N>
__device__ __forceinline__ void wait_vm() {
    asm volatile("s_waitcnt vmcnt(%0)" ::"n"(N) : "memory");
}
__device__ __forceinline__ void wait_lgkm0() { asm volatile("s_waitcnt lgkmcnt(0)" ::: "memory"); }

typedef int i32x4 __attribute__((ext_vector_type(4)));
__device__ __forceinline__ i32x4 dma_rsrc(const void* base) {
    const unsigned long long a = reinterpret_cast<unsigned long long>(base);
    return i32x4{(int)__builtin_amdgcn_readfirstlane((unsigned)a), (int)(__builtin_amdgcn_readfirstlane((unsigned)(a >> 32)) & 0xffff),
                 0x7fffffff, 0x00020000};
}
// ... 1264 lines not shown
#endif
#define G3_LAUNCH(ABL_)                                                                                   \
    {                                                                                                     \
        auto kern = gemm_nt3_kernel<BM, BN, WM, WN, NST, LSTM, ABL_>;                                     \
        static bool raised = false;                                                                       \
        if (lds > 64 * 1024 && !raised) {                                                                 \
            MARL_HIP_CHECK(hipFuncSetAttribute(reinterpret_cast<const void*>(kern),                      \
                                               hipFuncAttributeMaxDynamicSharedMemorySize, (int)lds));    \
            raised = true;                                                                                \
        }                                                                                                 \
        hipLaunchKernelGGL(kern, grid, dim3(WM * WN * 64), lds, st, batch);                               \
    }
    if (abl == 0) G3_LAUNCH(0)
    else if (abl == 1) G3_LAUNCH(1)
#ifdef MARL_G3_ABLATE
    else if (abl == 2) G3_LAUNCH(2)
    else if (abl == 3) G3_LAUNCH(3)
    else if (abl == 4) G3_LAUNCH(4)
    else if (abl == 5) G3_LAUNCH(5)
    else if (abl == 6) G3_LAUNCH(6)
#endif
    else return MARL_EINVAL;
#undef G3_LAUNCH
#ifdef MARL_G3_ABLATE
    if (batch.clk) {
        long long h[4];
        MARL_HIP_CHECK(hipMemcpy(h, batch.clk, sizeof(h), hipMemcpyDeviceToHost));
        fprintf(stderr, "[g3 clk] block 0: %.1f us, %.0f MHz shader clock\n", (h[3] - h[1]) * 0.01,
                (double)(h[2] - h[0]) / ((h[3] - h[1]) * 0.01));
    }
#endif
    MARL_LAUNCH_CHECK();
    return MARL_OK;
}

template <int BM, int BN, int WM, int WN, int NST, bool LSTM>
static int launch_g3p_variant(G3Batch batch, int max_m, int max_n, hipStream_t st) {
    dim3 grid((unsigned)cdiv(max_m, BM), (unsigned)cdiv(max_n, LSTM ? 32 : BN), (unsigned)batch.count);
    batch.gx = (int)grid.x;
    batch.gy = (int)grid.y;
    bool same = true;
    for (int i = 1; i < batch.count; ++i) same = same && batch.p[i].m == batch.p[0].m && batch.p[i].n == batch.p[0].n;
    batch.xcd_map = tune_get("nt_xcd", 1) && !LSTM && (batch.count == 1 || same);
    if (batch.xcd_map) grid = dim3(grid.x * grid.y * grid.z);
    batch.safe = tune_get("g3_safe", 0);
#ifndef MARL_G3_ABLATE
    batch.safe = batch.safe != 0;
#endif
    constexpr size_t lds = (size_t)NST * (BM + BN) * kImgRowBytes;
    static_assert(lds <= 160 * 1024, "LDS ring");
    static_assert((size_t)WM * WN * 32 * 36 * 4 <= lds, "epilogue panels fit the ring");
    auto kern = gemm_nt3p_kernel<BM, BN, WM, WN, NST, LSTM>;
    static bool raised = false;
    if (!raised) {
        MARL_HIP_CHECK(hipFuncSetAttribute(reinterpret_cast<const void*>(kern), hipFuncAttributeMaxDynamicSharedMemorySize, (int)lds));
        raised = true;
    }
    hipLaunchKernelGGL(kern, grid, dim3(WM * WN * 64), lds, st, batch);
    MARL_LAUNCH_CHECK();
    return MARL_OK;
}

static int check_g3(const G3Prob& p, bool lstm) {
    if (p.m <= 0 || p.n <= 0 || p.nseg < 1 || p.nseg > 2) {
        set_error("g3: empty problem m=%d n=%d nseg=%d", p.m, p.n, p.nseg);
        return MARL_EINVAL;
    }
    for (int s = 0; s < p.nseg; ++s) {
        const G3Seg& g = p.seg[s];
        if (!g.a3 || !g.b3 || g.steps <= 0 || g.a_row0 < 0 || g.b_row0 < 0 ||
            (reinterpret_cast<uintptr_t>(g.a3) & 15) || (reinterpret_cast<uintptr_t>(g.b3) & 15)) {
            set_error("g3: bad operand image (seg %d)", s);
            return MARL_EINVAL;
        }
        const int64_t brows = g.b_row0 + (lstm ? 4 * (int64_t)p.n : (int64_t)p.n) + 32;
        if ((brows >> 5) * g.steps * kImgChunkBytes >= (1ll << 31) || 10ll * g.steps * kImgChunkBytes >= (1ll << 31)) {
            set_error("g3: operand image of seg %d too large for 32-bit offsets", s);
            return MARL_ELIMIT;
        }
    }
    return MARL_OK;
}

int launch_gemm_nt3(const G3Batch& batch, hipStream_t st, int variant) {
    if (batch.count < 1 || batch.count > kMaxG3) return MARL_EINVAL;
    int max_m = 0, max_n = 0;
    int64_t blocks128 = 0;
    for (int i = 0; i < batch.count; ++i) {
        MARL_TRY(check_g3(batch.p[i], false));
        if (!batch.p[i].c) return MARL_EINVAL;
        max_m = batch.p[i].m > max_m ? batch.p[i].m : max_m;
        max_n = batch.p[i].n > max_n ? batch.p[i].n : max_n;
        blocks128 += cdiv(batch.p[i].m, 128) * cdiv(batch.p[i].n, 128);
    }
    if (!variant) variant = tune_get("g3_nt_variant", 0);
    if (!variant) {
        variant = max_n >= 96 && blocks128 >= 256 ? 2 : 7;
        if (variant == 2 && blocks128 >= 1024 && batch.count == 1 && max_n % 256 == 0) variant = 21;
    }
    prof_before(1, st);
    int rc;
    if (variant == 1)
        rc = launch_g3_variant<256, 128, 4, 2, 4, false>(batch, max_m, max_n, st);
    else if (variant == 2)
        rc = launch_g3_variant<128, 128, 2, 2, 3, false>(batch, max_m, max_n, st);
#ifdef MARL_G3_ABLATE
    else if (variant == 4)
        rc = launch_g3_variant<128, 128, 2, 2, 6, false>(batch, max_m, max_n, st);
    else if (variant == 5)
        rc = launch_g3_variant<128, 128, 4, 2, 3, false>(batch, max_m, max_n, st);
    else if (variant == 6)
        rc = launch_g3_variant<256, 128, 4, 2, 3, false>(batch, max_m, max_n, st);
#endif
    else if (variant == 7)
        rc = launch_g3_variant<64, 64, 2, 2, 4, false>(batch, max_m, max_n, st);
    else if (variant == 11)
        rc = launch_g3_variant<128, 64, 4, 2, 3, false>(batch, max_m, max_n, st);
    else if (variant == 12)
        rc = launch_g3_variant<64, 64, 2, 2, 3, false>(batch, max_m, max_n, st);
    else if (variant == 21)
        rc = launch_g3p_variant<256, 256, 2, 4, 3, false>(batch, max_m, max_n, st);
    else if (variant == 22)
        rc = launch_g3p_variant<256, 128, 4, 2, 4, false>(batch, max_m, max_n, st);

    else
        rc = launch_g3_variant<128, 64, 2, 2, 4, false>(batch, max_m, max_n, st);
    prof_after(1, st);
    return rc;
}

int g3_lstm_plan(const G3Batch& batch) {
    int64_t t128 = 0, t64 = 0;
    for (int i = 0; i < batch.count; ++i) {
        t128 += cdiv(batch.p[i].m, 128) * cdiv(batch.p[i].n, 32);
        t64 += cdiv(batch.p[i].m, 64) * cdiv(batch.p[i].n, 32);
    }
    if (t128 >= 192) return 2;
    return t64 >= 384 ? 4 : 3;
}

int launch_gemm_lstm3(const G3Batch& batch, hipStream_t st, int variant) {
    if (batch.count < 1 || batch.count > kMaxG3) return MARL_EINVAL;
    int max_m = 0, max_n = 0;
    for (int i = 0; i < batch.count; ++i) {
        const G3Prob& p = batch.p[i];
        MARL_TRY(check_g3(p, true));
        if (!p.bias || !p.c_prev || !p.h_next || !p.c_next) return MARL_EINVAL;
        max_m = p.m > max_m ? p.m : max_m;
        max_n = p.n > max_n ? p.n : max_n;
    }
    if (!variant) variant = tune_get("g3_lstm_variant", 0);
    if (!variant) variant = g3_lstm_plan(batch);
    prof_before(0, st);
    int rc;
    if (variant == 1)
        rc = launch_g3_variant<256, 128, 8, 1, 4, true>(batch, max_m, max_n, st);
    else if (variant == 3)
        rc = launch_g3_variant<32, 128, 1, 4, 4, true>(batch, max_m, max_n, st);
    else if (variant == 4)
        rc = launch_g3_variant<64, 128, 2, 4, 4, true>(batch, max_m, max_n, st);
    else if (variant == 5)
        rc = launch_g3p_variant<256, 128, 4, 2, 4, true>(batch, max_m, max_n, st);
    else if (variant == 6)
        rc = launch_g3p_variant<256, 128, 2, 2, 4, true>(batch, max_m, max_n, st);
#ifdef MARL_G3_ABLATE
    else if (variant == 7)
        rc = launch_g3p_variant<256, 128, 2, 2, 3, true>(batch, max_m, max_n, st);
#endif
    else
        rc = launch_g3_variant<128, 128, 4, 1, 3, true>(batch, max_m, max_n, st);
    prof_after(0, st);
    return rc;
}

static bool tn_pipe() { return tune_get("g3_tn_pipe", 1) != 0; }

template <int BI, int BJ, int WI, int WJ, int NST, bool DB, int ABL = 0, bool PIPE = false>
static int launch_tn3_variant(const G3TnArgs& a, dim3 grid, hipStream_t st) {
    constexpr size_t lds = (size_t)NST * ((BI + BJ) / 16) * 16 * kImgRowBytes;
    static_assert(lds <= 160 * 1024 && (size_t)WI * WJ * 32 * 36 * 4 <= lds, "LDS ring / epilogue panels");
    auto kern = gemm_tn3_kernel<BI, BJ, WI, WJ, NST, DB, ABL, PIPE>;
    static bool raised = false;
// ... 343 lines not shown
```

marlclassification_amd/csrc/gemm_split.hip:

```cpp
#include <stdlib.h>

#include "common.h"

namespace marl {

typedef float f32x16 __attribute__((ext_vector_type(16)));
typedef short bf16x8 __attribute__((ext_vector_type(8)));
typedef __bf16 bf16x2_t __attribute__((ext_vector_type(2)));
typedef float f32x2_t __attribute__((ext_vector_type(2)));
typedef uint32_t u32x4 __attribute__((ext_vector_type(4)));

namespace {

constexpr int SK = 32;
constexpr int SROW = 80;

__device__ __forceinline__ void lds_barrier() {
    asm volatile("s_waitcnt lgkmcnt(0)\n\ts_barrier" ::: "memory");
}

__device__ __forceinline__ void split_store4(char* dst, int plane, float a, float b, float c, float d) {
    uint32_t a0, a1, a2, b0, b1, b2;
    split_pair(a, b, a0, a1, a2);
    split_pair(c, d, b0, b1, b2);
// ... 495 lines not shown
        o[32] = p2;
    }
}

size_t split_image_floats(int rows, int k) { return (size_t)rows * ((k + 31) / 32) * 48; }

int launch_split_weights(const SplitBatch& b, hipStream_t st) {
    if (b.count <= 0) return MARL_OK;
    if (b.count > kMaxSplitDesc) return MARL_EINVAL;
    int64_t mx = 0;
    for (int i = 0; i < b.count; ++i) {
        const int64_t t = (int64_t)b.d[i].rows * b.d[i].kt * 16;
        mx = t > mx ? t : mx;
    }
    int64_t gx = cdiv(mx, 256);
    gx = gx > 512 ? 512 : (gx < 1 ? 1 : gx);
    hipLaunchKernelGGL(split_weights_kernel, dim3((unsigned)gx, (unsigned)b.count), dim3(256), 0, st, b);
    MARL_LAUNCH_CHECK();
    return MARL_OK;
}

namespace {
struct SplitReg {
    const float* base;
    size_t floats;
    int ld, k;
    const char* image;
};
thread_local SplitReg g_reg[kMaxSplitDesc];
thread_local int g_nreg = 0;
bool split_lookup(const GemmSeg& g, const void*& b3, int& kt) {
    for (int i = 0; i < g_nreg; ++i) {
        const SplitReg& r = g_reg[i];
        if (g.b < r.base || g.b >= r.base + r.floats || g.ldb != r.ld || g.k != r.k) continue;
        const size_t off = (size_t)(g.b - r.base);
        if (off % (size_t)r.ld) return false;
        kt = (r.k + 31) / 32;
        b3 = r.image + (off / (size_t)r.ld) * (size_t)kt * 192;
        return true;
    }
    return false;
}
}

void split_registry_reset() { g_nreg = 0; }
void split_registry_add(const float* base, int rows, int ld, int k, const void* image) {
    if (g_nreg < kMaxSplitDesc)
        g_reg[g_nreg++] = SplitReg{base, (size_t)rows * ld, ld, k, static_cast<const char*>(image)};
}

int split_mode() { return tune_get("mfma_split", 1); }

template <int BN, bool LSTM>
static int launch_nt_split_variant(dim3 grid, const GemmBatch& batch_in, hipStream_t st) {
    GemmBatch batch = batch_in;
    batch.gx = (int)grid.x;
    batch.gy = (int)grid.y;
    batch.xcd_map = batch.count == 1 && !LSTM && tune_get("nt_xcd", 1);
    if (batch.xcd_map) grid = dim3(grid.x * grid.y * grid.z);
    bool pre = true;
    for (int i = 0; i < batch.count && pre; ++i)
        for (int sg = 0; sg < batch.p[i].nseg && pre; ++sg) {
            GemmSeg& g = batch.p[i].seg[sg];
            pre = split_lookup(g, g.b3, g.kt3);
            if (pre && (int64_t)(LSTM ? 4 : 1) * batch.p[i].n * g.kt3 * 192 >= (1ll << 32)) pre = false;
        }
    constexpr size_t lds = (size_t)3 * (128 + BN) * SROW;
#ifdef MARL_KERNEL_TS
    static long long* d_ts = nullptr;
    static int calls = 0;
    const int rec = ts_begin(&d_ts, calls++);
    batch.ts = rec ? d_ts : nullptr;
#endif
    if (pre)
        hipLaunchKernelGGL((gemm_nt_split_kernel<BN, LSTM, true>), grid, dim3(256), lds, st, batch);
    else
        hipLaunchKernelGGL((gemm_nt_split_kernel<BN, LSTM, false>), grid, dim3(256), lds, st, batch);
#ifdef MARL_KERNEL_TS
    if (rec) ts_report(pre ? "nt_split_pre" : "nt_split", d_ts, 4);
#endif
    return MARL_OK;
}

int launch_gemm_nt_split(const GemmBatch& batch, int max_m, int max_n, int64_t blocks128, hipStream_t st) {
    if (blocks128 >= 384 && max_n >= 96) {
        dim3 grid((unsigned)cdiv(max_m, 128), (unsigned)cdiv(max_n, 128), (unsigned)batch.count);
        return launch_nt_split_variant<128, false>(grid, batch, st);
    }
    dim3 grid((unsigned)cdiv(max_m, 128), (unsigned)cdiv(max_n, 64), (unsigned)batch.count);
    return launch_nt_split_variant<64, false>(grid, batch, st);
}

int launch_gemm_lstm_split(const GemmBatch& batch, int max_m, int max_n, hipStream_t st) {
    dim3 grid((unsigned)cdiv(max_m, 128), (unsigned)cdiv(max_n, 32), (unsigned)batch.count);
    return launch_nt_split_variant<128, true>(grid, batch, st);
}

int launch_gemm_tn_split(const float* a, int lda, const float* b, int ldb, float* out, int ldo,
                         int64_t stride, int ni, int nj, int64_t rows, int64_t rows_per_split,
                         float* csum, dim3 grid, int gx, int gy, int gz, hipStream_t st) {
    if (tune_get("tn_split_waves", 8) == 8)
        hipLaunchKernelGGL(gemm_tn_split_kernel<8>, grid, dim3(512), (size_t)3 * 256 * SROW, st, a, lda, b, ldb,
                           out, ldo, stride, ni, nj, rows, rows_per_split, csum, gx, gy, gz);
    else
        hipLaunchKernelGGL(gemm_tn_split_kernel<4>, grid, dim3(256), (size_t)3 * 256 * SROW, st, a, lda, b, ldb,
                           out, ldo, stride, ni, nj, rows, rows_per_split, csum, gx, gy, gz);
    return MARL_OK;
}

}
```

marlclassification_amd/csrc/rowops.hip:

```cpp
#include <stdarg.h>
#include <stdlib.h>

#include <ctype.h>
#include <stdlib.h>
#include <string.h>

#include "common.h"
#include "sample.h"

namespace marl {

static thread_local char g_err[512] = "";
void set_error(const char* fmt, ...) {
    va_list ap;
    va_start(ap, fmt);
    vsnprintf(g_err, sizeof(g_err), fmt, ap);
    va_end(ap);
}
const char* last_error() { return g_err; }

namespace {
struct Knob {
    char key[32];
    int value;
// ... 1098 lines not shown
                const float* dr = Ds + a * ldw;
                const float* mr = Ms + a2 * l.ldm;
                float s = 0.f;
                for (int k = 0; k < n; ++k) s = fmaf(dr[k], mr[k], s);
                acc[i] += s;
            }
        }
        __syncthreads();
    }
#pragma unroll
    for (int i = 0; i < 4; ++i) {
        const int e = tid + i * kCommGradThreads;
        if (e < nn) part[(size_t)blockIdx.x * nn + e] = acc[i];
    }
}

constexpr int kCommSumEntries = 16, kCommSumSlices = kCommGradThreads / kCommSumEntries;
__global__ __launch_bounds__(kCommGradThreads) void comm_grad_sum_kernel(const float* __restrict__ part, int blocks,
                                                                         int nn, float* __restrict__ out) {
    __shared__ double sl[kCommSumSlices][kCommSumEntries];
    const int el = threadIdx.x % kCommSumEntries, slice = threadIdx.x / kCommSumEntries;
    const int e = blockIdx.x * kCommSumEntries + el;
    const int chunk = (blocks + kCommSumSlices - 1) / kCommSumSlices;
    const int b0 = slice * chunk, b1 = b0 + chunk < blocks ? b0 + chunk : blocks;
    double s = 0.0;
    if (e < nn) {
        int b = b0;
        for (; b + 8 <= b1; b += 8) {
            float v[8];
#pragma unroll
            for (int u = 0; u < 8; ++u) v[u] = part[(size_t)(b + u) * nn + e];
#pragma unroll
            for (int u = 0; u < 8; ++u) s += (double)v[u];
        }
        for (; b < b1; ++b) s += (double)part[(size_t)b * nn + e];
    }
    sl[slice][el] = s;
    __syncthreads();
    if (slice == 0 && e < nn) {
        double t = 0.0;
#pragma unroll
        for (int q = 0; q < kCommSumSlices; ++q) t += sl[q][el];
        out[e] = (float)t;
    }
}

int comm_grad_max_agents() { return 32; }

int comm_grad_blocks(int64_t pairs, int* per_out) {
    if (pairs < 1) pairs = 1;
    const int64_t per = cdiv(pairs, (int64_t)kCommGradMaxBlocks);
    if (per_out) *per_out = (int)per;
    return (int)cdiv(pairs, per);
}

int comm_grad_supported(int na, int n, int n2, int ldw) {
    return na >= 1 && na <= comm_grad_max_agents() && n >= 1 && n2 >= 1 && ldw >= n && (ldw & 3) == 0 &&
           comm_grad_lds(na, n, n2, ldw).total * sizeof(float) <= kCommGradMaxLds;
}

int launch_comm_grad(const float* dz, int lddz, const float* msg, int ldmsg, const float* w, int ldw, int na, int nb,
                     int steps, int n2, int n, float* part, float* out, hipStream_t st) {
    if (!comm_grad_supported(na, n, n2, ldw) || n2 > lddz || n > ldmsg || nb < 1 || steps < 1) {
        set_error("mixing-matrix gradient: %d agents, %d x %d decoder weight outside the kernel's range (<= %d agents, "
                  "%zu bytes of LDS)", na, n2, n, comm_grad_max_agents(), kCommGradMaxLds);
        return MARL_ELIMIT;
    }
    const size_t lds = comm_grad_lds(na, n, n2, ldw).total * sizeof(float);
    if (lds > 64 * 1024)
        MARL_HIP_CHECK(hipFuncSetAttribute(reinterpret_cast<const void*>(comm_grad_kernel),
                                           hipFuncAttributeMaxDynamicSharedMemorySize, (int)kCommGradMaxLds));
    const int64_t pairs = (int64_t)steps * nb;
    int per = 1;
    const int blocks = comm_grad_blocks(pairs, &per);
    hipLaunchKernelGGL(comm_grad_kernel, dim3((unsigned)blocks), dim3(kCommGradThreads), lds, st, dz, lddz, msg, ldmsg,
                       w, ldw, na, nb, n2, n, pairs, per, part);
    MARL_LAUNCH_CHECK();
    hipLaunchKernelGGL(comm_grad_sum_kernel, dim3((unsigned)cdiv(na * na, kCommSumEntries)), dim3(kCommGradThreads), 0, st,
                       part, blocks, na * na, out);
    MARL_LAUNCH_CHECK();
    return MARL_OK;
}

__global__ void pos_embed_fwd_kernel(const int32_t* __restrict__ pos,
                                     const float* __restrict__ npos_in, int H, int W_,
                                     const float* __restrict__ W, const float* __restrict__ b,
                                     const float* __restrict__ gamma,
                                     const float* __restrict__ beta, float* __restrict__ npos4,
                                     float* __restrict__ z, int ldz, float* __restrict__ stats,
                                     float* __restrict__ out, int ldo, int64_t rows, int nd) {
    const int64_t r = (int64_t)blockIdx.x * blockDim.x + threadIdx.x;
    if (r >= rows) return;
    const float p0 = npos_in ? npos_in[r * 2] : (float)pos[r * 2] / (float)H;
    const float p1 = npos_in ? npos_in[r * 2 + 1] : (float)pos[r * 2 + 1] / (float)W_;
    if (npos4) {
        npos4[r * 4] = p0;
        npos4[r * 4 + 1] = p1;
    }
    float* zr = z + r * ldz;
    float s = 0.f;
    for (int j = 0; j < nd; ++j) {
        const float v = b[j] + p0 * W[4 * j] + p1 * W[4 * j + 1];
        zr[j] = v;
        s += v;
    }
    const float mean = s / (float)nd;
    float q = 0.f;
    for (int j = 0; j < nd; ++j) {
        const float d = zr[j] - mean;
        q += d * d;
    }
    const float rstd = 1.0f / sqrtf(q / (float)nd + 1e-5f);
    if (stats) {
        stats[r * 2] = mean;
        stats[r * 2 + 1] = rstd;
    }
    float* orow = out + r * ldo;
    for (int j = 0; j < nd; ++j) orow[j] = silu_f((zr[j] - mean) * rstd * gamma[j] + beta[j]);
}

int launch_pos_embed_fwd(const int32_t* pos, const float* npos_in, int h, int w, const float* W,
                         const float* b, const float* gamma, const float* beta, float* npos4,
                         float* z, int ldz, float* stats, float* out, int ldo, int64_t rows, int nd,
                         hipStream_t st) {
    hipLaunchKernelGGL(pos_embed_fwd_kernel, dim3((unsigned)cdiv(rows, 128)), dim3(128), 0, st, pos,
                       npos_in, h, w, W, b, gamma, beta, npos4, z, ldz, stats, out, ldo, rows, nd);
    MARL_LAUNCH_CHECK();
    return MARL_OK;
}

__global__ void lstm_cell_bwd_kernel(const LstmBwdBatch B) {
    if (B.vec4)
        lstm_cell_bwd_elem4(B.a[blockIdx.y], B.rows, (int64_t)blockIdx.x * blockDim.x + threadIdx.x);
    else
        lstm_cell_bwd_elem(B.a[blockIdx.y], B.rows, (int64_t)blockIdx.x * blockDim.x + threadIdx.x);
}

int launch_lstm_cell_bwd_batch(LstmBwdBatch& b, int count, hipStream_t st) {
    int nmax = 0;
    b.vec4 = 1;
    for (int i = 0; i < count; ++i) {
        nmax = b.a[i].n > nmax ? b.a[i].n : nmax;
        if (!lstm_bwd_vec4_ok(b.a[i])) b.vec4 = 0;
    }
    if (!b.vec4)
        for (int i = 0; i < count; ++i)
            if (b.a[i].g3) {
                set_error("lstm_cell_bwd: the gate-gradient image needs the 4-wide form");
                return MARL_EINVAL;
            }
    hipLaunchKernelGGL(lstm_cell_bwd_kernel, dim3((unsigned)cdiv(b.rows * (b.vec4 ? nmax / 4 : nmax), 256), (unsigned)count),
                       dim3(256), 0, st, b);
    MARL_LAUNCH_CHECK();
    return MARL_OK;
}

int launch_lstm_cell_bwd(const float* dh, int lddh, float* dc, int lddc, float* gates, int ldg,
                         const float* c_prev, const float* c_new, int ldc, int64_t rows, int n,
                         hipStream_t st) {
    LstmBwdBatch b{};
    b.a[0] = LstmBwdArgs{dh, dc, gates, c_prev, c_new, lddh, lddc, ldg, ldc, n, nullptr, 0, 0, 0};
    b.rows = rows;
    return launch_lstm_cell_bwd_batch(b, 1, st);
}

int launch_lstm_cell_bwd2(const float* dh0, int lddh0, float* dc0, int lddc0, float* gates0,
                          int ldg0, const float* cp0, const float* cn0, int ldc0, int n0,
                          const float* dh1, int lddh1, float* dc1, int lddc1, float* gates1,
                          int ldg1, const float* cp1, const float* cn1, int ldc1, int n1,
                          int64_t rows, hipStream_t st) {
    LstmBwdBatch b{};
    b.a[0] = LstmBwdArgs{dh0, dc0, gates0, cp0, cn0, lddh0, lddc0, ldg0, ldc0, n0, nullptr, 0, 0, 0};
    b.a[1] = LstmBwdArgs{dh1, dc1, gates1, cp1, cn1, lddh1, lddc1, ldg1, ldc1, n1, nullptr, 0, 0, 0};
    b.rows = rows;
    return launch_lstm_cell_bwd_batch(b, 2, st);
}

template <int MAXA>
__global__ __launch_bounds__(256) void sample_kernel(const SampleArgs A) {
    const int lane = threadIdx.x & 63;
    const int r = blockIdx.x * 4 + (threadIdx.x >> 6);
    if (r >= A.R) return;
    float p[MAXA];
    SamplePre<MAXA> S;
    sample_prefetch<MAXA>(A, r, lane, S);
    sample_row_logits<MAXA>(A, r, p, lane);
    sample_finish<MAXA>(A, r, p, lane, S);
}

int launch_sample(const SampleArgs& a, hipStream_t st) {
    if (a.nA > MARL_MAX_ACTIONS) return MARL_ELIMIT;
    if (a.nA <= 4)
        hipLaunchKernelGGL(sample_kernel<4>, dim3((unsigned)cdiv(a.R, 4)), dim3(256), 0, st, a);
    else
        hipLaunchKernelGGL(sample_kernel<MARL_MAX_ACTIONS>, dim3((unsigned)cdiv(a.R, 4)), dim3(256), 0, st, a);
    MARL_LAUNCH_CHECK();
    return MARL_OK;
}

__global__ __launch_bounds__(256) void draw_episode_kernel(
    uint64_t seed, uint64_t offset, const uint64_t* __restrict__ offset_dev,
// ... 15 lines not shown
                pos0[e] = (int64_t)(((uint64_t)uv[i] * span) >> 32);
            }
        }
        return;
    }
    rel -= q_pos;
    float* dst = nullptr;
    int64_t n = 0;
    uint32_t stream = 1;
    bool normal = true;
    if (rel < q_b) {
        dst = h0, n = nb_el, stream = 1;
    } else if ((rel -= q_b) < q_b) {
        dst = c0, n = nb_el, stream = 2;
    } else if ((rel -= q_b) < q_a) {
        dst = hc0, n = na_el, stream = 3;
    } else if ((rel -= q_a) < q_a) {
        dst = cc0, n = na_el, stream = 4;
    } else if ((rel -= q_a) < q_n) {
        dst = noise, n = n_noise, stream = 5, normal = false;
    } else {
        return;
    }
    const Philox4 u = philox4x32_10(seed, offset, (uint32_t)rel, stream | ((uint32_t)(rel >> 32) << 8));
    float v[4];
    if (normal) {
        const float r0 = sqrtf(-2.0f * logf(philox_u01(u.x))), r1 = sqrtf(-2.0f * logf(philox_u01(u.z)));
        const float a0 = 6.283185307179586f * philox_u01(u.y), a1 = 6.283185307179586f * philox_u01(u.w);
        v[0] = r0 * cosf(a0);
        v[1] = r0 * sinf(a0);
        v[2] = r1 * cosf(a1);
        v[3] = r1 * sinf(a1);
    } else {
        v[0] = -logf(philox_u01(u.x));
        v[1] = -logf(philox_u01(u.y));
        v[2] = -logf(philox_u01(u.z));
        v[3] = -logf(philox_u01(u.w));
    }
#pragma unroll
    for (int i = 0; i < 4; ++i)
        if (rel * 4 + i < n) dst[rel * 4 + i] = v[i];
}

int launch_draw_episode(uint64_t seed, uint64_t offset, const uint64_t* offset_dev, int64_t* pos0,
                        int R, int H, int W, int f, float* h0, float* c0, int n_b, float* hc0,
                        float* cc0, int n_a, float* noise, int64_t n_noise, hipStream_t st) {
    const int64_t nb_el = (int64_t)R * n_b, na_el = (int64_t)R * n_a;
    const int64_t q_pos = cdiv((int64_t)R * 2, 4), q_b = cdiv(nb_el, 4), q_a = cdiv(na_el, 4),
                  q_n = noise ? cdiv(n_noise, 4) : 0;
    const int64_t total = q_pos + 2 * q_b + 2 * q_a + q_n;
    hipLaunchKernelGGL(draw_episode_kernel, dim3((unsigned)cdiv(total, 256)), dim3(256), 0, st, seed,
                       offset, offset_dev, pos0, R, H, W, f, h0, c0, nb_el, hc0, cc0, na_el, noise, n_noise, q_pos,
                       q_b, q_a, q_n);
    MARL_LAUNCH_CHECK();
    return MARL_OK;
}

__global__ void permute_kernel(const PermBatch B) {
    const PermDesc& d = B.d[blockIdx.y];
    const int64_t tot = (int64_t)d.rows * d.cols;
    for (int64_t idx = (int64_t)blockIdx.x * blockDim.x + threadIdx.x; idx < tot;
         idx += (int64_t)gridDim.x * blockDim.x) {
        const int r = (int)(idx / d.cols), c = (int)(idx % d.cols);
        const int64_t so = (int64_t)(r / d.rd) * d.rs1 + (int64_t)(r % d.rd) * d.rs2 +
                           (int64_t)(c / d.cd) * d.cs1 + (int64_t)(c % d.cd) * d.cs2;
        float v = d.src ? d.src[so] : 0.f;
        if (d.src2) v += d.src2[so];
        d.dst[(int64_t)r * d.dst_ld + c] = v;
    }
}

int launch_permute(const PermBatch& b, hipStream_t st) {
    if (b.count <= 0) return MARL_OK;
    if (b.count > kMaxPerm) return MARL_EINVAL;
    int64_t mx = 0;
    for (int i = 0; i < b.count; ++i) {
        const int64_t t = (int64_t)b.d[i].rows * b.d[i].cols;
        mx = t > mx ? t : mx;
    }
    int64_t gx = cdiv(mx, 256);
    if (gx > 1024) gx = 1024;
    if (gx < 1) gx = 1;
    hipLaunchKernelGGL(permute_kernel, dim3((unsigned)gx, (unsigned)b.count), dim3(256), 0, st, b);
    MARL_LAUNCH_CHECK();
    return MARL_OK;
}

__global__ void adam_kernel(float* __restrict__ p, const float* __restrict__ g,
                            float* __restrict__ m, float* __restrict__ v, int64_t n,
                            float step_size, float inv_sqrt_bc2, float beta1, float beta2,
                            float eps, float grad_scale, const Counters* __restrict__ cnt) {
    if (cnt) {
        step_size = cnt->lr_over_bc1;
        inv_sqrt_bc2 = cnt->inv_sqrt_bc2;
    }
    for (int64_t i = (int64_t)blockIdx.x * blockDim.x + threadIdx.x; i < n;
         i += (int64_t)gridDim.x * blockDim.x) {
        const float gr = g[i] * grad_scale;
        const float mi = m[i] + (1.0f - beta1) * (gr - m[i]);
        const float vi = v[i] * beta2 + (1.0f - beta2) * (gr * gr);
        m[i] = mi;
        v[i] = vi;
        const float denom = sqrtf(vi) * inv_sqrt_bc2 + eps;
        p[i] = p[i] - step_size * (mi / denom);
    }
}

int launch_adam(float* p, const float* g, float* m, float* v, int64_t n, float lr_over_bc1,
                float inv_sqrt_bc2, float beta1, float beta2, float eps, float grad_scale,
                hipStream_t st, const Counters* cnt) {
    if (n <= 0) return MARL_OK;
    int64_t gx = cdiv(n, 256);
    if (gx > 4096) gx = 4096;
    hipLaunchKernelGGL(adam_kernel, dim3((unsigned)gx), dim3(256), 0, st, p, g, m, v, n,
                       lr_over_bc1, inv_sqrt_bc2, beta1, beta2, eps, grad_scale, cnt);
    MARL_LAUNCH_CHECK();
    return MARL_OK;
}

__global__ void counters_kernel(Counters* c, uint64_t rng_offset, int64_t step, float lr, float beta1,
                                float beta2, int tick) {
    if (blockIdx.x != 0 || threadIdx.x != 0) return;
    uint64_t off = rng_offset, st = (uint64_t)step;
    if (tick) {
        off = c->rng_offset + 1;
        st = c->step + 1;
    }
    c->rng_offset = off;
    c->step = st;
    const double bc1 = 1.0 - pow((double)beta1, (double)st);
    const double bc2 = 1.0 - pow((double)beta2, (double)st);
    c->lr_over_bc1 = (float)((double)lr / bc1);
    c->inv_sqrt_bc2 = (float)(1.0 / sqrt(bc2));
}

int launch_counters_set(Counters* c, uint64_t rng_offset, int64_t step, float lr, float beta1,
                        float beta2, int tick, hipStream_t st) {
    hipLaunchKernelGGL(counters_kernel, dim3(1), dim3(64), 0, st, c, rng_offset, step, lr, beta1, beta2, tick);
    MARL_LAUNCH_CHECK();
    return MARL_OK;
}

__global__ void fill_kernel(float* p, int64_t n, float v) {
    for (int64_t i = (int64_t)blockIdx.x * blockDim.x + threadIdx.x; i < n;
         i += (int64_t)gridDim.x * blockDim.x)
        p[i] = v;
}
int launch_fill(float* p, int64_t n, float v, hipStream_t st) {
    if (n <= 0) return MARL_OK;
    int64_t gx = cdiv(n, 256);
    if (gx > 8192) gx = 8192;
    hipLaunchKernelGGL(fill_kernel, dim3((unsigned)gx), dim3(256), 0, st, p, n, v);
    MARL_LAUNCH_CHECK();
    return MARL_OK;
}

__global__ void copy2d_kernel(const float* __restrict__ src, int64_t lds, float* __restrict__ dst,
                              int64_t ldd, int64_t rows, int cols) {
    const int64_t tot = rows * cols;
    for (int64_t i = (int64_t)blockIdx.x * blockDim.x + threadIdx.x; i < tot;
         i += (int64_t)gridDim.x * blockDim.x) {
        const int64_t r = i / cols;
        const int c = (int)(i % cols);
        dst[r * ldd + c] = src[r * lds + c];
    }
}
// ... 189 lines not shown
```

marlclassification_amd/engine.py:

```python

from __future__ import annotations

import ctypes as C
from dataclasses import dataclass, field
from typing import Dict, List, Optional, Sequence, Tuple

import torch as th

from . import _lib
from ._lib import MARL_NPARAMS, MarlConfig, P, check

CNN_SPECS: Dict[str, Tuple[List[int], List[int]]] = {
    "mnist": ([1, 8, 16], [2, 4]),
    "resisc45": ([3, 16, 32, 64], [2, 4, 8]),
    "aid": ([3, 16, 32, 64, 128], [2, 4, 8, 16]),
    "worldstrat": ([3, 16, 32, 64, 128, 256], [2, 4, 8, 16, 32]),
    "skin_cancer": ([3, 16, 32, 64], [2, 4, 8]),
}

_MW = "_ModelsWrapper__"
_CNN_PREFIX = _MW + "map_obs._Generic2dCnnModule__layers."
_LSTM = "._LSTMCellWrapper__lstm."


# ... 484 lines not shown

    def _check_ppo_bufs(self, out: EpisodeTensors, bufs: Tuple[th.Tensor, ...], what: str) -> None:
        if (len(bufs) not in (7, 8) or bufs[3].numel() != 7 or bufs[5].shape != out.step_values.shape or
                bufs[6].shape != out.step_values.shape):
            raise ValueError(f"{what}: buffers from new_ppo_bufs(out, entropy) needed")

    def advantages(
        self, out: EpisodeTensors, y: th.Tensor, gamma: float, lam: float, phase: int = 0,
        bufs: Optional[Tuple[th.Tensor, ...]] = None,
    ) -> Tuple[th.Tensor, ...]:
        cfg = self.cfg
        assert cfg is not None
        if not 0.0 <= lam <= 1.0:
            raise ValueError(f"gae_lambda must lie in [0, 1], got {lam}")
        if phase not in (0, 1, 2):
            raise ValueError(f"phase must be 0, 1 or 2, got {phase}")
        y = _need(y, th.int64, "y")
        if bufs is None:
            bufs = self.new_ppo_bufs(out, out.step_probs is not None)
        self._check_ppo_bufs(out, bufs, "advantages")
        ews = self.episode_ws(True)
        check(self.lib.marl_advantages(
            C.byref(cfg), ews.data_ptr(), _nbytes(ews), out.step_preds.data_ptr(), out.step_values.data_ptr(),
            y.data_ptr(), C.c_float(gamma), C.c_float(lam), bufs[5].data_ptr(), bufs[6].data_ptr(),
            bufs[4].data_ptr(), phase, _stream(self.device)))
        return bufs

    def ppo_loss(
        self, out: EpisodeTensors, y: th.Tensor, old_logp: th.Tensor, advn: th.Tensor, ret: th.Tensor,
        clip_eps: float, bufs: Optional[Tuple[th.Tensor, ...]] = None, entropy_coef: float = 0.0,
    ) -> Tuple[th.Tensor, ...]:
        cfg = self.cfg
        assert cfg is not None
        if not clip_eps > 0.0:
            raise ValueError(f"ppo_clip must be > 0, got {clip_eps}")
        if not entropy_coef >= 0.0:
            raise ValueError(f"entropy_coef must be >= 0, got {entropy_coef}")
        y = _need(y, th.int64, "y")
        ent = entropy_coef > 0.0
        if ent and out.step_probs is None:
            raise ValueError("ppo_loss(entropy_coef > 0) needs the episode's step_probs: episode_forward(probs=True)")
        want = tuple(out.step_log_probas.shape)
        ins = []
        for t, name in ((old_logp, "old_logp"), (advn, "advn"), (ret, "ret")):
            if not isinstance(t, th.Tensor) or tuple(t.shape) != want:
                raise ValueError(f"ppo_loss: {name} must be a tensor of shape {want}, got "
                                 f"{tuple(getattr(t, 'shape', ()))}")
            ins.append(_need(t, th.float32, name))
        if bufs is None:
            bufs = self.new_ppo_bufs(out, ent)
        self._check_ppo_bufs(out, bufs, "ppo_loss")
        if ent and (len(bufs) != 8 or bufs[7].shape != out.step_probs.shape):
            raise ValueError("ppo_loss(entropy_coef > 0): buffers from new_ppo_bufs(out, True) needed")
        probs = _need(out.step_probs, th.float32, "step_probs") if ent else None
        ews = self.episode_ws(True)
        check(self.lib.marl_ppo_loss_fwd_bwd(
            C.byref(cfg), ews.data_ptr(), _nbytes(ews), out.step_preds.data_ptr(),
            out.step_log_probas.data_ptr(), out.step_values.data_ptr(), y.data_ptr(), ins[0].data_ptr(),
            ins[1].data_ptr(), ins[2].data_ptr(), C.c_float(clip_eps), _ptr(probs), C.c_float(entropy_coef),
            bufs[0].data_ptr(), bufs[1].data_ptr(), bufs[2].data_ptr(), bufs[7].data_ptr() if ent else None,
            bufs[3].data_ptr(), _stream(self.device)))
        return bufs

    def grad_clip(self, grads: th.Tensor, max_norm: float, grad_scale: float = 1.0) -> th.Tensor:
        if not max_norm > 0.0:
            raise ValueError(f"max_grad_norm must be > 0, got {max_norm}")
        if not grad_scale > 0.0:
            raise ValueError(f"grad_scale must be > 0, got {grad_scale}")
        if not grads.is_cuda or grads.dtype != th.float32 or not grads.is_contiguous():
            raise RuntimeError("grad_clip: the gradient buffer must be a contiguous fp32 GPU tensor")
        if self._clip_scratch is None:
            self._clip_scratch = th.zeros(_lib.MARL_GRAD_CLIP_SCRATCH_BYTES // 8 + 1, dtype=th.float64,
                                          device=self.device)
        sc = self._clip_scratch
        check(self.lib.marl_grad_clip(grads.data_ptr(), grads.numel(), C.c_float(max_norm), C.c_float(grad_scale),
                                      sc[-1:].data_ptr(),
                                      sc.data_ptr(), _lib.MARL_GRAD_CLIP_SCRATCH_BYTES, _stream(self.device)))
        return sc[-1:].view(th.float32)[0]

    def adam(
        self, params: th.Tensor, grads: th.Tensor, exp_avg: th.Tensor, exp_avg_sq: th.Tensor,
        step: int, lr: float, betas: Tuple[float, float] = (0.9, 0.999), eps: float = 1e-8,
        grad_scale: float = 1.0, counters: Optional[th.Tensor] = None,
    ) -> None:
        for t in (params, grads, exp_avg, exp_avg_sq):
            if not t.is_cuda or t.dtype != th.float32 or not t.is_contiguous():
                raise RuntimeError("adam buffers must be contiguous fp32 GPU tensors")
        check(self.lib.marl_adam_step(
            params.data_ptr(), grads.data_ptr(), exp_avg.data_ptr(), exp_avg_sq.data_ptr(),
            params.numel(), step, lr, betas[0], betas[1], eps, grad_scale, _ptr(counters),
            _stream(self.device)))

    def step_forward(
        self, obs: th.Tensor, msg: th.Tensor, norm_pos: th.Tensor, h: th.Tensor, c: th.Tensor,
        hc: th.Tensor, cc: th.Tensor, noise: Optional[th.Tensor] = None,
        rng: Optional[Tuple[int, int]] = None, ws: Optional[th.Tensor] = None,
    ) -> Tuple[th.Tensor, ...]:
        cfg = self.cfg
        assert cfg is not None
        na, nb = cfg.nb_agents, cfg.batch
        dev = self.device
        ins = [_need(t, th.float32, n) for t, n in (
            (obs, "obs"), (msg, "msg"), (norm_pos, "norm_pos"), (h, "h"), (c, "c"), (hc, "hc"),
            (cc, "cc"))]
        outs = (
            th.empty(na, nb, cfg.nb_action, device=dev), th.empty(na, nb, device=dev),
            th.empty(na, nb, cfg.nb_class, device=dev), th.empty(na, nb, cfg.n_m, device=dev),
            th.empty(na, nb, cfg.n_b, device=dev), th.empty(na, nb, cfg.n_b, device=dev),
            th.empty(na, nb, cfg.n_a, device=dev), th.empty(na, nb, cfg.n_a, device=dev),
        )
        extra: Tuple[th.Tensor, ...] = ()
        nz = act = lp = None
        if noise is not None or rng is not None:
            nz = None if noise is None else _need(noise, th.float32, "noise")
            act = th.empty(na, nb, dtype=th.int64, device=dev)
            lp = th.empty(na, nb, device=dev)
            extra = (act, lp)
        seed, offset = rng if rng is not None else (0, 0)
        wws = self.packed_weights_ws()
        if ws is not None:
            if cfg.nb_steps != 1:
                raise RuntimeError("step_forward(ws=...): configure the engine with nb_steps = 1")
            self._check_ws(ws, "step_forward")
            fn, ews = self.lib.marl_step_forward_train, ws
        else:
            fn, ews = self.lib.marl_step_forward, self.episode_ws(False)
        self._agg(
            fn, C.byref(cfg), wws.data_ptr(), _nbytes(wws), ews.data_ptr(), _nbytes(ews),
            *[t.data_ptr() for t in ins], *[t.data_ptr() for t in outs], _ptr(nz), seed & _U64,
            offset & _U64, _ptr(act), _ptr(lp), _stream(dev))
        return outs + extra

    def _check_ws(self, ws: th.Tensor, what: str) -> None:
        if getattr(ws, "_marl_key", None) != (self._cfg_key, _tune_epoch):
            raise RuntimeError(
                f"{what}: the engine was re-configured (other batch size / image shape / layout knob) since "
                "this workspace was acquired - it no longer fits")

    def step_backward(
        self, ws: th.Tensor, obs: th.Tensor, grads: Dict[str, th.Tensor],
        g_probs: Optional[th.Tensor] = None, g_logp: Optional[th.Tensor] = None,
        g_values: Optional[th.Tensor] = None, g_preds: Optional[th.Tensor] = None,
        g_msg: Optional[th.Tensor] = None, g_h: Optional[th.Tensor] = None,
        g_c: Optional[th.Tensor] = None, g_hc: Optional[th.Tensor] = None,
        g_cc: Optional[th.Tensor] = None, want: Sequence[bool] = (True,) * 5,
        d_comm: Optional[th.Tensor] = None,
    ) -> Tuple[Optional[th.Tensor], ...]:
        cfg = self.cfg
        assert cfg is not None
        self._check_ws(ws, "step_backward")
        if d_comm is not None and self.comm is None:
            raise ValueError("step_backward(d_comm=...): the engine has no communication matrix")
        na, nb, dev = cfg.nb_agents, cfg.batch, self.device
        obs = _need(obs, th.float32, "obs")
        ups = [None if t is None else _need(t, th.float32, n) for t, n in (
            (g_probs, "g_probs"), (g_logp, "g_logp"), (g_values, "g_values"), (g_preds, "g_preds"),
            (g_msg, "g_msg"), (g_h, "g_h"), (g_c, "g_c"), (g_hc, "g_hc"), (g_cc, "g_cc"))]
        widths = (cfg.n_m, cfg.n_b, cfg.n_b, cfg.n_a, cfg.n_a)
        outs = tuple(th.empty(na, nb, n, device=dev) if w else None for n, w in zip(widths, want))
        wws = self.packed_weights_ws()
        self._agg(
            self.lib.marl_step_backward,
            C.byref(cfg), wws.data_ptr(), _nbytes(wws), ws.data_ptr(), _nbytes(ws), obs.data_ptr(),
            *[_ptr(t) for t in ups], self._table(grads), *[_ptr(t) for t in outs], _stream(dev))
        if d_comm is not None:
            self.comm_grad(ws, 1, d_comm)
        return outs

    def draw_episode(self, seed: int, offset: int, with_noise: bool = False,
                     into: Optional[Tuple[th.Tensor, ...]] = None,
                     counters: Optional[th.Tensor] = None):
        cfg = self.cfg
        assert cfg is not None
        na, nb, ns, dev = cfg.nb_agents, cfg.batch, cfg.nb_steps, self.device
# ... 87 lines not shown
```

marlclassification_amd/fused.py:

```python

from __future__ import annotations

from dataclasses import dataclass
from typing import Callable, Dict, List, Optional, Sequence, Tuple

import torch as th

from .engine import EpisodeTensors, HipEngine, ModelSpec


@dataclass
class EpisodeDraws:

    pos0: th.Tensor
    h0: th.Tensor
    c0: th.Tensor
    hc0: th.Tensor
    cc0: th.Tensor
    noise: Optional[th.Tensor]
    rng: Optional[Tuple[int, int]] = None


def draw_episode(spec: ModelSpec, na: int, nb: int, ns: int, sizes, device,
                 generator: Optional[th.Generator] = None) -> EpisodeDraws:
# ... 39 lines not shown

    def _views(self, flat: th.Tensor) -> Dict[str, th.Tensor]:
        out = {}
        for k, s in self.shapes.items():
            n = 1
            for d in s:
                n *= d
            out[k] = flat[self.offsets[k]: self.offsets[k] + n].view(s)
        return out

    def param_views(self) -> Dict[str, th.Tensor]:
        return self._views(self.params)

    def grad_views(self) -> Dict[str, th.Tensor]:
        return self._views(self.grads)

    def load(self, tensors: Dict[str, th.Tensor]) -> None:
        views = self.param_views()
        with th.no_grad():
            for k in self.names:
                views[k].copy_(tensors[k])


def check_ppo_options(ppo_epochs: int, ppo_clip: float, gae_lambda: float, max_grad_norm: Optional[float]) -> None:
    if isinstance(ppo_epochs, bool) or not isinstance(ppo_epochs, int) or ppo_epochs < 1:
        raise ValueError(f"ppo_epochs must be an integer >= 1, got {ppo_epochs!r}")
    if not ppo_clip > 0.0:
        raise ValueError(f"ppo_clip must be > 0, got {ppo_clip}")
    if not 0.0 <= gae_lambda <= 1.0:
        raise ValueError(f"gae_lambda must lie in [0, 1], got {gae_lambda}")
    if max_grad_norm is not None and not max_grad_norm > 0.0:
        raise ValueError(f"max_grad_norm must be > 0 or None, got {max_grad_norm}")


def ppo_options_on(ppo_epochs: int, ppo_clip: float, gae_lambda: float, max_grad_norm: Optional[float]) -> bool:
    return ppo_epochs != 1 or ppo_clip != 0.2 or gae_lambda != 1.0 or max_grad_norm is not None


class CommUpdate:

    def __init__(self, source, leaves: Sequence[th.Tensor], lr: float) -> None:
        if not lr > 0.0:
            raise ValueError(f"comm_lr must be > 0 or None, got {lr}")
        leaves = list(leaves)
        if not leaves:
            raise ValueError("comm_lr: the live communication source has no leaf that requires grad (a plain "
                             "callable offers no parameters(): pass a module or a tensor)")
        self.source = source
        self.opt = th.optim.Adam(leaves, lr=lr)
        self._d: Optional[th.Tensor] = None

    def buffer(self, eng: HipEngine) -> th.Tensor:
        na = eng.cfg.nb_agents
        if self._d is None or self._d.shape[0] != na or self._d.device != eng.device:
            self._d = th.empty(na, na, device=eng.device)
        return self._d

    def step(self, live: Optional[th.Tensor], allreduce, scale: float) -> None:
        if live is None or not live.requires_grad:
            raise RuntimeError("comm_lr: the communication source was evaluated without a graph (grad mode off, or a "
                               "source that does not depend on its leaves): nothing to update")
        d = self._d
        if allreduce is not None:
            allreduce(d)
        self.opt.zero_grad(set_to_none=True)
        live.backward((d if scale == 1.0 else d * scale).to(live.dtype))
        self.opt.step()


def comm_update_for(current: Optional[CommUpdate], source, leaves, comm_lr: Optional[float]) -> Optional[CommUpdate]:
    if comm_lr is None or source is None:
        return None
    if current is not None and current.source is source:
        return current
    return CommUpdate(source, leaves(), comm_lr)


def ppo_bufs_fit(bufs, out: EpisodeTensors, entropy: bool) -> bool:
    return (bufs is not None and len(bufs) == (8 if entropy else 7) and bufs[0].shape == out.step_preds.shape and
            (not entropy or bufs[7].shape == out.step_probs.shape))


def apply_update(eng: HipEngine, flat: "FlatParams", gp, gl, gv, g_probs, gviews, lr: float, allreduce,
                 max_grad_norm: Optional[float], repack: Callable[[], None],
                 comm: Optional[CommUpdate] = None) -> Optional[th.Tensor]:
    bucketed = hasattr(allreduce, "before_backward")
    if bucketed:
        allreduce.before_backward(eng)
    try:
        d_comm = {} if comm is None else {"d_comm": comm.buffer(eng)}
        eng.episode_backward(gp, gl, gv, gviews, g_probs=g_probs, **d_comm)
    finally:
        if bucketed:
            allreduce.after_backward(eng)
    scale = rank_scale = 1.0 if allreduce is None else allreduce(flat.grads)
    norm = None
    if max_grad_norm is not None:
        norm = eng.grad_clip(flat.grads, max_grad_norm, grad_scale=scale)
        scale = 1.0
    flat.step += 1
    eng.adam(flat.params, flat.grads, flat.exp_avg, flat.exp_avg_sq, flat.step, lr, grad_scale=scale)
    if comm is not None:
        comm.step(eng.comm_live, allreduce, rank_scale)
    repack()
    return norm


def ppo_epochs_loop(eng: HipEngine, flat: "FlatParams", out: EpisodeTensors, y: th.Tensor, bufs, epochs: int,
                    clip: float, beta: float, lr: float, allreduce, max_grad_norm: Optional[float], gviews,
                    replay: Callable[[], EpisodeTensors], repack: Callable[[], None],
                    comm: Optional[CommUpdate] = None) -> Optional[th.Tensor]:
    gp, gl, gv, _, _, advn, ret = bufs[:7]
    gpr = bufs[7] if beta > 0 else None
    old_logp = out.step_log_probas
    cur, norm = out, None
    for k in range(epochs):
        if k > 0:
            cur = replay()
            if cur.step_log_probas.data_ptr() == old_logp.data_ptr():
                raise RuntimeError("PPO replay wrote over the rollout's log-probabilities (persistent output "
                                   "tensors?): the ratios would all be 1")
        eng.ppo_loss(cur, y, old_logp, advn, ret, clip, bufs, entropy_coef=beta)
        norm = apply_update(eng, flat, gp, gl, gv, gpr, gviews, lr, allreduce, max_grad_norm, repack, comm)
    return norm


class FusedA2C:

    def __init__(self, engine: HipEngine, flat: FlatParams, lr: float, gamma: float,
                 allreduce: Optional[Callable[[th.Tensor], float]] = None,
                 use_graph: bool = False, entropy_coef: float = 0.0, ppo_epochs: int = 1,
                 ppo_clip: float = 0.2, gae_lambda: float = 1.0,
                 max_grad_norm: Optional[float] = None, comm_lr: Optional[float] = None) -> None:
        if use_graph and allreduce is not None:
            raise ValueError("hipGraph replay covers the single-GPU iteration (no collective inside)")
        if comm_lr is not None and not comm_lr > 0.0:
            raise ValueError(f"comm_lr must be > 0 or None, got {comm_lr}")
        if use_graph and comm_lr is not None and engine.comm_source is not None:
            raise ValueError("hipGraph replay does not cover the update of a live communication source (torch "
                             "launches between the captured calls): use_graph with comm_lr and a live source")
        self.comm_lr = None if comm_lr is None else float(comm_lr)
        self._comm_update: Optional[CommUpdate] = None
        if not entropy_coef >= 0.0:
            raise ValueError(f"entropy_coef must be >= 0, got {entropy_coef}")
        check_ppo_options(ppo_epochs, ppo_clip, gae_lambda, max_grad_norm)
        self.ppo_epochs, self.ppo_clip, self.gae_lambda = int(ppo_epochs), float(ppo_clip), float(gae_lambda)
        self.max_grad_norm = None if max_grad_norm is None else float(max_grad_norm)
        self._ppo = ppo_options_on(ppo_epochs, ppo_clip, gae_lambda, max_grad_norm)
        if use_graph and self._ppo:
            raise ValueError("hipGraph replay covers the one-update A2C iteration: ppo_epochs / ppo_clip / "
                             "gae_lambda / max_grad_norm must stay at their defaults with use_graph")
        self._ppo_bufs = None
        self.last_grad_norm: Optional[th.Tensor] = None
        self.entropy_coef = float(entropy_coef)
        self._graph = None
        self.engine = engine
        self.flat = flat
        self.lr = lr
        self.gamma = gamma
        self.allreduce = allreduce
        self._pviews = flat.param_views()
        self._gviews = flat.grad_views()
        self._loss_bufs = None
        self._packed_gen = -1

    def pack(self) -> None:
        self.engine.pack(self._pviews)
        self._packed_gen = self.engine.weights_generation

    def rollout(self, img: th.Tensor, draws: EpisodeDraws, train: bool,
                forced_actions: Optional[th.Tensor] = None, probs: bool = False) -> EpisodeTensors:
        if self._packed_gen != self.engine.weights_token():
            self.pack()
        if self.engine.comm_source is not None:
            self.engine.refresh_comm()
        return self.engine.episode_forward(img, draws.pos0, draws.h0, draws.c0, draws.hc0,
                                           draws.cc0, draws.noise, forced_actions, train,
                                           rng=draws.rng, probs=probs)

    def iteration_graph(self, img: th.Tensor, y: th.Tensor, seed: int,
                        offset: int) -> Tuple[EpisodeTensors, th.Tensor]:
        eng = self.engine
        if self._ppo:
            raise ValueError("iteration_graph captures the one-update A2C iteration: ppo_epochs / ppo_clip / "
                             "gae_lambda / max_grad_norm must stay at their defaults")
        if self.comm_lr is not None and eng.comm_source is not None:
            raise ValueError("iteration_graph does not cover the update of a live communication source (torch "
                             "launches between the captured calls): run iteration(), or drop comm_lr")
        from . import engine as _engine_mod

        beta = self.entropy_coef
        key = (img.data_ptr(), y.data_ptr(), eng._cfg_key, seed, _engine_mod._tune_epoch, beta,
               None if eng.comm is None else eng.comm.data_ptr())
        if self._graph is None or self._graph[0] != key:
            if self._graph is not None:
                eng.lib.marl_graph_destroy(self._graph[1])
                self._graph = None
            eager = self.iteration(img, y, draw_episode_device(eng, seed, offset))
            offset += 1
            stream = th.cuda.Stream(device=eng.device)
            out = eng.new_outputs(beta > 0)
            draws = eng.draw_episode(seed, 0)
            cnt = eng.new_counters()
            gviews = self._gviews
            stream.wait_stream(th.cuda.current_stream(eng.device))
            with th.cuda.stream(stream):
                eng.counters_set(cnt, offset, self.flat.step + 1, self.lr)
                th.cuda.synchronize(eng.device)
                eng.graph_begin()
                try:
                    eng.draw_episode(seed, 0, into=draws, counters=cnt)
                    eng.episode_forward(img, draws[0], draws[1], draws[2], draws[3], draws[4], None,
                                        None, True, rng=(seed, 0), out=out, counters=cnt)
                    bufs = eng.a2c_loss(out, y, self.gamma, 0, self._loss_bufs, entropy_coef=beta)
                    gp, gl, gv, scalars = bufs[:4]
                    eng.episode_backward(gp, gl, gv, gviews, g_probs=bufs[5] if beta > 0 else None)
                    eng.adam(self.flat.params, self.flat.grads, self.flat.exp_avg,
                             self.flat.exp_avg_sq, 1, self.lr, counters=cnt)
                    eng.pack(self._pviews)
                    eng.counters_tick(cnt, self.lr)
                except BaseException:
                    try:
                        eng.graph_end()
                    except Exception:
                        pass
                    raise
                handle = eng.graph_end()
            self._graph = (key, handle, stream, (out, draws, cnt, scalars),
                           {"offset": offset, "step": self.flat.step + 1, "cap_lr": self.lr})
            return eager
        _, handle, stream, (out, _draws, cnt, scalars), expect = self._graph
        stream.wait_stream(th.cuda.current_stream(eng.device))
        with th.cuda.stream(stream):
            if (expect["offset"] != offset or expect["step"] != self.flat.step + 1 or
                    expect["cap_lr"] != self.lr):
                eng.counters_set(cnt, offset, self.flat.step + 1, self.lr)
            eng.graph_launch(handle)
        th.cuda.current_stream(eng.device).wait_stream(stream)
        self.flat.step += 1
        eng.fwd_generation += 1
        expect.update(offset=offset + 1, step=self.flat.step + 1)
        return out, scalars

    def iteration(self, img: th.Tensor, y: th.Tensor, draws: EpisodeDraws) -> Tuple[EpisodeTensors, th.Tensor]:
        eng = self.engine
        beta = self.entropy_coef
        if self._ppo:
            return self._iteration_ppo(img, y, draws)
        out = self.rollout(img, draws, True, probs=beta > 0)
        if (self._loss_bufs is None or self._loss_bufs[0].shape != out.step_preds.shape or
                len(self._loss_bufs) != (6 if beta > 0 else 5)):
            self._loss_bufs = eng.new_loss_bufs(out, beta > 0)
        bufs = eng.a2c_loss(out, y, self.gamma, 0, self._loss_bufs, entropy_coef=beta)
        gp, gl, gv, scalars = bufs[:4]
        apply_update(eng, self.flat, gp, gl, gv, bufs[5] if beta > 0 else None, self._gviews, self.lr,
                     self.allreduce, None, self.pack, self._comm())
        return out, scalars

    def _comm(self) -> Optional[CommUpdate]:
        from . import comm as _comm_mod

        src = self.engine.comm_source
        self._comm_update = comm_update_for(self._comm_update, src, lambda: _comm_mod.leaves(src), self.comm_lr)
        return self._comm_update

    def _iteration_ppo(self, img: th.Tensor, y: th.Tensor, draws: EpisodeDraws) -> Tuple[EpisodeTensors, th.Tensor]:
        eng, beta = self.engine, self.entropy_coef
        ent = beta > 0
        out = self.rollout(img, draws, True, probs=ent)
        bufs = self._ppo_bufs
        if not ppo_bufs_fit(bufs, out, ent):
            bufs = self._ppo_bufs = eng.new_ppo_bufs(out, ent)
        eng.advantages(out, y, self.gamma, self.gae_lambda, 0, bufs)
        norm = ppo_epochs_loop(
            eng, self.flat, out, y, bufs, self.ppo_epochs, self.ppo_clip, beta, self.lr, self.allreduce,
            self.max_grad_norm, self._gviews,
            replay=lambda: self.rollout(img, draws, True, forced_actions=out.step_actions, probs=ent),
            repack=self.pack, comm=self._comm())
        if norm is not None:
            self.last_grad_norm = norm
        return out, bufs[3]
```

marlclassification_amd/networks/models.py:

```python

from dataclasses import dataclass
from typing import Dict, List, Optional, Tuple

import torch as th
from torch import nn

from ..engine import HipEngine, ModelSpec
from ..fused import FlatParams
from .blocks import LSTMCellWrapper, head, linear_ln_silu, mlp_two_norms
from .init import init_layers
from .vision import VisionCnnModule


class _StepLease:

    def __init__(self, eng: HipEngine) -> None:
        self.eng = eng
        self.ws: Optional[th.Tensor] = eng.train_ws_acquire()

    def release(self) -> None:
        ws, self.ws = self.ws, None
        if ws is not None:
            self.eng.train_ws_release(ws)

# ... 198 lines not shown
        img_patch: th.Tensor,
        msg_t: th.Tensor,
        norm_pos: th.Tensor,
        recurrent_hidden: RecurrentOutput,
    ) -> Tuple[ModelOutput, RecurrentOutput]:
        na, nb = img_patch.shape[:2]
        eng = self.hip_engine(None)
        eng.configure(na, nb, 1, (img_patch.shape[2], img_patch.shape[3] + 1, img_patch.shape[4] + 1))
        self.ensure_packed(eng)
        rh = recurrent_hidden
        state = (msg_t, rh.h, rh.c, rh.h_caret, rh.c_caret)
        if step_needs_graph(self, img_patch, norm_pos, *state, comm=eng.comm_live):
            named = list(self.named_parameters())
            probs, values, preds, msg, h, c, hc, cc = _StepFunction.apply(
                eng, img_patch, norm_pos, None, None, tuple(k for k, _ in named), eng.comm_live, *state,
                *[p for _, p in named])
        else:
            probs, values, preds, msg, h, c, hc, cc = eng.step_forward(
                img_patch, msg_t, norm_pos, rh.h, rh.c, rh.h_caret, rh.c_caret)
        return ModelOutput(probs, values, preds, msg), RecurrentOutput(h, c, hc, cc)

    def model_spec(self, actions: Optional[List[List[int]]]) -> ModelSpec:
        cnn = self.__map_obs
        if actions is None:
            actions = [[0, 0]] * self.__nb_action
        if len(actions) != self.__nb_action:
            raise ValueError(f"model has {self.__nb_action} actions, environment {len(actions)}")
        return ModelSpec(ft_extr=cnn.hip_name, window=cnn.window, actions=[list(a) for a in actions],
                         **self.__dims)

    def hip_engine(self, actions: Optional[List[List[int]]]) -> HipEngine:
        dev = self.device
        if dev.type != "cuda":
            raise RuntimeError(
                "ModelsWrapper runs on the GPU only: move it with .to('cuda') (the HIP library "
                "is the only implementation; there is no CPU fallback)"
            )
        key = (str(dev), None if actions is None else tuple(map(tuple, actions)))
        eng = self.__engines.get(key)
        if eng is None:
            eng = HipEngine(self.model_spec(actions), dev)
            self.__engines[key] = eng
        if self.__comm_source:
            eng.comm_source = self.__comm_source[0]
            eng.refresh_comm()
        else:
            eng.comm_source = eng.comm_live = None
            eng.comm = self.comm_matrix
        return eng

    def flat_state(self) -> FlatParams:
        dev = self.device
        named = list(self.named_parameters())
        flat = self.__flat
        ok = flat is not None and flat.params.device == dev
        if ok:
            views = flat.param_views()
            ok = all(p.data_ptr() == views[k].data_ptr() for k, p in named)
        if not ok:
            fresh = FlatParams({k: tuple(p.shape) for k, p in named}, dev)
            views = fresh.param_views()
            with th.no_grad():
                for k, p in named:
                    views[k].copy_(p.data)
                    p.data = views[k]
            if flat is not None and flat.params.device == dev and flat.numel == fresh.numel:
                fresh.exp_avg.copy_(flat.exp_avg)
                fresh.exp_avg_sq.copy_(flat.exp_avg_sq)
                fresh.step = flat.step
            self.__flat = fresh
            self.__packed_token = {}
        return self.__flat

    def _version_token(self) -> Tuple:
        return tuple(p._version for p in self.parameters())

    def ensure_packed(self, eng: HipEngine) -> None:
        flat = self.flat_state()
        token = self._version_token() + (eng.weights_token(),)
        if self.__packed_token.get(id(eng)) != token:
            eng.pack(flat.param_views())
            self.__packed_token[id(eng)] = token

    def mark_updated(self, eng: HipEngine) -> None:
        eng.pack(self.flat_state().param_views())
        self.__packed_token = {id(eng): self._version_token() + (eng.weights_token(),)}
```

marlclassification_amd/training/trainer.py:

```python

from typing import Callable, Dict, Iterable, Optional, Tuple

import torch as th

from ..core import EpisodeSampler
from ..engine import EpisodeTensors
from ..fused import (CommUpdate, apply_update, check_ppo_options, comm_update_for, ppo_bufs_fit, ppo_epochs_loop,
                     ppo_options_on)
from ..metrics import ConfusionMeter, LossMeter
from ..networks import ModelsWrapper

MetricLogger = Callable[[int, Dict[str, float]], None]


class Trainer:
    def __init__(
        self,
        model: ModelsWrapper,
        nb_class: int,
        learning_rate: float,
        gamma: float,
        metric_logger: Optional[MetricLogger] = None,
        log_interval: int = 100,
        meter_window_size: int = 64,
        allreduce: Optional[Callable[[th.Tensor], float]] = None,
        exact_standardize_group=None,
        entropy_coef: float = 0.0,
        ppo_epochs: int = 1,
        ppo_clip: float = 0.2,
        gae_lambda: float = 1.0,
        max_grad_norm: Optional[float] = None,
        comm_lr: Optional[float] = None,
    ) -> None:
        if not entropy_coef >= 0.0:
            raise ValueError(f"entropy_coef must be >= 0, got {entropy_coef}")
        check_ppo_options(ppo_epochs, ppo_clip, gae_lambda, max_grad_norm)
        if comm_lr is not None and not comm_lr > 0.0:
            raise ValueError(f"comm_lr must be > 0 or None, got {comm_lr}")
        self.__comm_lr = None if comm_lr is None else float(comm_lr)
        self.__comm_update: Optional[CommUpdate] = None
        self.__model = model
        self.__nb_class = nb_class
        self.__lr = learning_rate
        self.__gamma = gamma
        self.__metric_logger = metric_logger
        self.__log_interval = log_interval
        self.__allreduce = allreduce
        self.__exact_group = exact_standardize_group
        self.__entropy_coef = float(entropy_coef)
        self.__ppo_epochs, self.__ppo_clip, self.__gae_lambda = int(ppo_epochs), float(ppo_clip), float(gae_lambda)
        self.__max_grad_norm = None if max_grad_norm is None else float(max_grad_norm)
        self.__ppo = ppo_options_on(ppo_epochs, ppo_clip, gae_lambda, max_grad_norm)
        self.__ppo_bufs: Optional[Tuple[th.Tensor, ...]] = None
        self.__grad_norm: Optional[th.Tensor] = None
        self.__curr_step = 0
        self.__loss_bufs: Optional[Tuple[th.Tensor, ...]] = None
        self.__conf_meter = ConfusionMeter(nb_class, window_size=meter_window_size)
        self.__meter_keys = ("loss", "path", "error", "critic") + (("entropy",) if entropy_coef > 0 else ())
        self.__meter_idx = {k: i for i, k in enumerate(self.__meter_keys)}
        if self.__ppo:
            self.__meter_idx.update(approx_kl=5, clip_frac=6)
            self.__meter_keys += ("approx_kl", "clip_frac")
        self.__meters = {k: LossMeter(window_size=meter_window_size) for k in self.__meter_keys}
        if self.__max_grad_norm is not None:
            self.__meters["grad_norm"] = LossMeter(window_size=meter_window_size)

    @property
    def curr_step(self) -> int:
        return self.__curr_step

    def __comm(self) -> Optional[CommUpdate]:
        model = self.__model
        self.__comm_update = comm_update_for(self.__comm_update, model.comm_source, model.comm_parameters,
                                             self.__comm_lr)
        return self.__comm_update

    def __exact_phases(self, call: Callable[[int], Tuple[th.Tensor, ...]]) -> None:
        if self.__exact_group is None:
            call(0)
            return
        from ..parallel import allreduce_adv_stats

        allreduce_adv_stats(call(1)[4], self.__exact_group)
        call(2)

    def train_step(self, x: th.Tensor, y: th.Tensor, sampler: EpisodeSampler) -> Tuple[EpisodeTensors, th.Tensor]:
        model = self.__model
        y = y.to(model.device)
        if self.__ppo:
            return self.__train_step_ppo(x, y, sampler)
        beta = self.__entropy_coef
        ent = beta > 0
        eng, out = sampler.run_episode_raw(x, train=True, probs=ent)
        bufs = self.__loss_bufs
        if (bufs is None or len(bufs) != (6 if ent else 5) or bufs[0].shape != out.step_preds.shape or
                (ent and bufs[5].shape != out.step_probs.shape)):
            bufs = self.__loss_bufs = eng.new_loss_bufs(out, ent)
        self.__exact_phases(lambda phase: eng.a2c_loss(out, y, self.__gamma, phase, bufs, entropy_coef=beta))
        flat = model.flat_state()
        apply_update(eng, flat, bufs[0], bufs[1], bufs[2], bufs[5] if ent else None, flat.grad_views(), self.__lr,
                     self.__allreduce, None, lambda: model.mark_updated(eng), self.__comm())
        return out, bufs[3]

    def __train_step_ppo(self, x: th.Tensor, y: th.Tensor,
                         sampler: EpisodeSampler) -> Tuple[EpisodeTensors, th.Tensor]:
        model, beta = self.__model, self.__entropy_coef
        ent = beta > 0
        _, img, draws = sampler.prepare(x)
        eng, out = sampler.run_episode_raw(img, train=True, draws=draws, probs=ent)
        if not ppo_bufs_fit(self.__ppo_bufs, out, ent):
            self.__ppo_bufs = eng.new_ppo_bufs(out, ent)
        bufs = self.__ppo_bufs
        self.__exact_phases(lambda phase: eng.advantages(out, y, self.__gamma, self.__gae_lambda, phase, bufs))
        flat = model.flat_state()
        norm = ppo_epochs_loop(
            eng, flat, out, y, bufs, self.__ppo_epochs, self.__ppo_clip, beta, self.__lr, self.__allreduce,
            self.__max_grad_norm, flat.grad_views(),
            replay=lambda: sampler.run_episode_raw(img, train=True, draws=draws, probs=ent,
                                                   forced=out.step_actions)[1],
            repack=lambda: model.mark_updated(eng), comm=self.__comm())
        if norm is not None:
            self.__grad_norm = norm
        return out, bufs[3]

    def train_epoch(self, dataloader: Iterable, epoch_index: int, episode_sampler: EpisodeSampler) -> None:
        self.__model.train()
        for x_train, y_train in dataloader:
            out, scalars = self.train_step(x_train, y_train, episode_sampler)
            self.__conf_meter.add(out.step_preds[-1].mean(dim=0), y_train)
            for k in self.__meter_keys:
                self.__meters[k].add(scalars[self.__meter_idx[k]].clone())
            if self.__max_grad_norm is not None:
                self.__meters["grad_norm"].add(self.__grad_norm.clone())
            if self.__metric_logger is not None and self.__curr_step % self.__log_interval == 0:
                self.__metric_logger(self.__curr_step, self.metrics())
            self.__curr_step += 1

    def metrics(self) -> Dict[str, float]:
        m = {
            "error": self.__meters["error"].loss(),
            "path_loss": self.__meters["path"].loss(),
            "loss": self.__meters["loss"].loss(),
            "critic_loss": self.__meters["critic"].loss(),
            "train_prec": self.__conf_meter.precision().mean().item(),
            "train_rec": self.__conf_meter.recall().mean().item(),
        }
        if "entropy" in self.__meters:
            m["entropy"] = self.__meters["entropy"].loss()
        for k in ("approx_kl", "clip_frac", "grad_norm"):
            if k in self.__meters:
                m[k] = self.__meters[k].loss()
        return m

    def eval_epoch(self, dataloader: Iterable, epoch_index: int, episode_sampler: EpisodeSampler) -> ConfusionMeter:
        self.__model.eval()
        conf_meter = ConfusionMeter(self.__nb_class, None)
        with th.no_grad():
            for x_test, y_test in dataloader:
                out = episode_sampler.run_episode_get_last_step(x_test)
                conf_meter.add(out.prediction.mean(dim=0), y_test)
        return conf_meter
```

Measured before the change: 9.349 million agent-env-steps/s.

## Fuse Adam with single-launch weight repack, fuse episode-begin setup, skip unused t=0 dh GEMMs

Adds marl_adam_pack_step, which runs Adam and then repacks all weight layouts through one table-driven pack kernel, replacing the separate per-layout pack pass after each update. Episode start replaces the position conversion, state loads, image builds and the first step's position encoding with one fused begin kernel. In the backward pass at t=0, the GEMMs whose outputs would only feed gradients into the initial hidden state are skipped, while keeping the original batch's kernel plan. These changes cut kernel launch count and redundant work per iteration, at the cost of a large kernel-argument table and more complex env-gated code paths.

```diff
diff --git a/include/marl_hip.h b/include/marl_hip.h
--- a/include/marl_hip.h
+++ b/include/marl_hip.h
@@ -161,6 +161,12 @@
 int marl_adam_step(float* params, const float* grads, float* exp_avg, float* exp_avg_sq,
                    int64_t n, int64_t step, float lr, float beta1, float beta2, float eps,
                    float grad_scale, const void* counters, void* stream);
+
+int marl_adam_pack_step(float* params, const float* grads, float* exp_avg, float* exp_avg_sq,
+                        int64_t n, int64_t step, float lr, float beta1, float beta2, float eps,
+                        float grad_scale, const void* counters, const marl_config* cfg,
+                        const float* const* params_host, void* weights_ws, size_t weights_ws_bytes,
+                        void* stream);
 
 int marl_step_forward(const marl_config* cfg, const void* weights_ws, size_t weights_ws_bytes,
                       void* episode_ws, size_t episode_ws_bytes,
diff --git a/marlclassification_amd/_lib.py b/marlclassification_amd/_lib.py
--- a/marlclassification_amd/_lib.py
+++ b/marlclassification_amd/_lib.py
@@ -57,7 +57,7 @@
 EXPORTS = (
     "marl_abi_version marl_last_error marl_param_numel marl_workspace_sizes marl_pack_weights "
     "marl_patch_gather marl_transition marl_episode_forward marl_episode_backward "
-    "marl_a2c_loss_fwd_bwd marl_adam_step marl_step_forward marl_gemm_nt marl_gemm_tn "
+    "marl_a2c_loss_fwd_bwd marl_adam_step marl_adam_pack_step marl_step_forward marl_gemm_nt marl_gemm_tn "
     "marl_gemm_tn_scratch marl_gemm_nt_weights marl_gemm_weight_image_bytes marl_ln_silu_fwd marl_debug_buffer "
     "marl_profile_begin marl_profile_end marl_normalize_positions "
     "marl_cnn_wgrad marl_cnn_wgrad_scratch marl_tune marl_tune_get marl_draw_episode "
@@ -113,6 +113,7 @@
     lib.marl_ppo_loss_fwd_bwd.argtypes = ([_cfgp, _vp, _sz] + [_vp] * 7 + [_f, _vp, _f] + [_vp] * 6)
     lib.marl_grad_clip.argtypes = [_vp, _i64, _f, _f, _vp, _vp, _sz, _vp]
     lib.marl_adam_step.argtypes = [_vp, _vp, _vp, _vp, _i64, _i64, _f, _f, _f, _f, _f, _vp, _vp]
+    lib.marl_adam_pack_step.argtypes = (lib.marl_adam_step.argtypes[:-1] + [_cfgp, C.POINTER(_vp), _vp, _sz, _vp])
     lib.marl_step_forward.argtypes = ([_cfgp, _vp, _sz, _vp, _sz] + [_vp] * 15 + [_vp, _u64, _u64, _vp, _vp] +
                                       [_vp])
     lib.marl_step_forward_train.argtypes = lib.marl_step_forward.argtypes
diff --git a/marlclassification_amd/csrc/common.h b/marlclassification_amd/csrc/common.h
--- a/marlclassification_amd/csrc/common.h
+++ b/marlclassification_amd/csrc/common.h
@@ -112,7 +112,7 @@
                    int m, int n, const float* bias = nullptr, int accumulate = 0);
 void gemm_add_seg(GemmProb& p, const float* a, int lda, const float* b, int ldb, int k);
 
-int launch_gemm_nt(const GemmBatch& batch, hipStream_t st);
+int launch_gemm_nt(const GemmBatch& batch, hipStream_t st, const GemmBatch* plan_like = nullptr);
 int launch_gemm_lstm(const GemmBatch& batch, hipStream_t st);
 
 int split_mode();
@@ -135,7 +135,7 @@
     SplitRegistryScope(const SplitRegistryScope&) = delete;
     ~SplitRegistryScope() { split_registry_reset(); }
 };
-int launch_gemm_nt_split(const GemmBatch& batch, int max_m, int max_n, int64_t blocks128, hipStream_t st);
+int launch_gemm_nt_split(const GemmBatch& batch, int max_m, int max_n, bool wide, hipStream_t st);
 int launch_gemm_lstm_split(const GemmBatch& batch, int max_m, int max_n, hipStream_t st);
 int launch_gemm_tn_split(const float* a, int lda, const float* b, int ldb, float* out, int ldo,
                          int64_t stride, int ni, int nj, int64_t rows, int64_t rows_per_split,
@@ -177,6 +177,7 @@
                const float* bias = nullptr, int accumulate = 0);
 void g3_add_seg(G3Prob& p, const void* a3, int a_row0, const void* b3, int b_row0, int k);
 int launch_gemm_nt3(const G3Batch& batch, hipStream_t st, int variant = 0);
+int g3_nt_plan(const G3Batch& batch);
 int launch_gemm_lstm3(const G3Batch& batch, hipStream_t st, int variant = 0);
 int g3_lstm_plan(const G3Batch& batch);
 struct G3TnArgs {
@@ -386,6 +387,28 @@
                         int R, int H, int W, int f, float* h0, float* c0, int n_b, float* hc0,
                         float* cc0, int n_a, float* noise, int64_t n_noise, hipStream_t st);
 
+constexpr int kBeginCopies = 5, kBeginImages = 2;
+struct EpisodeBegin {
+    const int64_t* pos0;
+    int32_t* pos;
+    int R, H, W;
+    const float *pe_W, *pe_b, *pe_gamma, *pe_beta;
+    float *pe_npos, *pe_z, *pe_stats, *pe_out;
+    int pe_ldz, pe_ldo, pe_nd;
+    struct Copy {
+        const float* src;
+        float* dst;
+        int n, ld, vec4;
+    } copy[kBeginCopies];
+    struct Image {
+        const float* src;
+        char* dst;
+        int k;
+    } image[kBeginImages];
+    int blocks[1 + kBeginCopies + kBeginImages];
+};
+int launch_episode_begin(EpisodeBegin& a, hipStream_t st);
+
 struct PermDesc {
     const float* src;
     float* dst;
@@ -401,6 +424,23 @@
     int count;
 };
 int launch_permute(const PermBatch& b, hipStream_t st);
+
+enum PackOut { PO_WP = 0, PO_WT, PO_WP3, PO_WT3, PO_WP3K, PO_WT3K, PO_WF, PO_BSUM };
+struct PackParam {
+    const float* src;
+    uint32_t wp, wt, wp3, wt3, wp3k, wt3k, wf;
+    int n, k;
+    int conv;
+};
+constexpr int kMaxPackJobs = 192;
+struct PackTable {
+    PackParam p[MARL_NPARAMS];
+    float* W;
+    int count;
+    uint16_t job[kMaxPackJobs];
+};
+static_assert(sizeof(PackTable) <= 4096, "the table travels as a kernel argument");
+int launch_pack(const PackTable& t, hipStream_t st);
 
 struct Counters {
     uint64_t rng_offset;
diff --git a/marlclassification_amd/csrc/episode.hip b/marlclassification_amd/csrc/episode.hip
--- a/marlclassification_amd/csrc/episode.hip
+++ b/marlclassification_amd/csrc/episode.hip
@@ -920,6 +920,14 @@
     }
     return enabled && panel_sample_supported(d.nA);
 }
+static bool iter_lean() {
+    static int enabled = -1;
+    if (enabled < 0) {
+        const char* e = getenv("MARL_ITER_LEAN");
+        enabled = (e && e[0] == '0') ? 0 : 1;
+    }
+    return enabled != 0;
+}
 static int step_chain(const Ctx& c, int t, const SampleArgs* sample = nullptr) {
     const Dims& d = c.d;
     PanelFwdBatch pb{};
@@ -1155,6 +1163,65 @@
     return launch_images(ib, st);
 }
 
+static int pack_weights_once(const Dims& d, const WLayout& w, const float* const* params, float* W,
+                             hipStream_t st) {
+    static_assert(MARL_P_LB_BHH == MARL_P_LB_BIH + 1 && MARL_P_LA_BHH == MARL_P_LA_BIH + 1, "b_hh follows b_ih");
+    if (w.total >> 32) {
+        set_error("adam_pack_step: weights workspace above 2^32 floats");
+        return MARL_ELIMIT;
+    }
+    PackTable t{};
+    t.W = W;
+    t.count = 0;
+    int rc = MARL_OK;
+    auto job = [&](int i, int out) {
+        if (t.count == kMaxPackJobs) rc = MARL_ELIMIT;
+        else t.job[t.count++] = (uint16_t)(i * 8 + out);
+    };
+    for (int i = 0; i < MARL_NPARAMS; ++i) {
+        const ParamMeta m = param_meta(d, i);
+        if (m.kind == PK_NONE) continue;
+        if (!params[i]) {
+            set_error("parameter %d is null", i);
+            return MARL_EINVAL;
+        }
+        PackParam& p = t.p[i];
+        p.src = params[i];
+        p.wp = (uint32_t)w.wp[i];
+        p.wt = (uint32_t)w.wt[i];
+        p.wp3 = (uint32_t)w.wp3[i];
+        p.wt3 = (uint32_t)w.wt3[i];
+        p.wp3k = (uint32_t)w.wp3k[i];
+        p.wt3k = (uint32_t)w.wt3k[i];
+        p.wf = (uint32_t)w.wf[i];
+        p.n = m.n;
+        p.k = m.kind == PK_VEC ? 0 : m.k;
+        p.conv = m.kind == PK_CONV;
+        job(i, PO_WP);
+        if (m.kind == PK_VEC) continue;
+        job(i, PO_WT);
+        if (m.kind == PK_MATRIX) {
+            job(i, PO_WP3);
+            job(i, PO_WT3);
+            if (w.wp3k[i]) {
+                job(i, PO_WP3K);
+                job(i, PO_WT3K);
+            }
+        } else if (w.wf[i]) {
+            job(i, PO_WF);
+        }
+    }
+    t.p[MARL_P_LB_BIH].wt = (uint32_t)w.bsum_b;
+    t.p[MARL_P_LA_BIH].wt = (uint32_t)w.bsum_a;
+    job(MARL_P_LB_BIH, PO_BSUM);
+    job(MARL_P_LA_BIH, PO_BSUM);
+    if (rc != MARL_OK) {
+        set_error("adam_pack_step: more than %d layouts", kMaxPackJobs);
+        return rc;
+    }
+    return launch_pack(t, st);
+}
+
 static void register_split_images(const Dims& d, const WLayout& w, const float* W) {
     split_registry_reset();
     for (int i = 0; i < MARL_NPARAMS; ++i) {
@@ -1450,6 +1517,7 @@
         }
         hipStream_t st = cs.st;
         float* ddbar = c.at(c.e.DDBAR) + (size_t)t * s_nmo;
+        const bool no_dh = t == 0 && !sb && iter_lean();
         {
             GemmBatch gb{};
             gb.p[0] = gemm_prob(c.at(c.e.GB, t), d.ld_gb, c.wt(MARL_P_LB_WHH), d.ld_gb, 4 * d.n_b,
@@ -1485,14 +1553,35 @@
                     g.p[3] = g3_prob(c.img(c.e.GA3), r0, c.wt3k(MARL_P_LA_WIH), d.nf, 4 * d.n_a,
                                      c.at(c.e.DDBAR2) + (size_t)t * s_nmo, d.ld_dbl, R, d.n_mo + d.n_d);
                     g.count = 4;
-                    MARL_TRY(launch_gemm_nt3(g, c.st));
+                    if (no_dh) {
+                        const int plan = g3_nt_plan(g);
+                        g.p[0] = g.p[2];
+                        g.p[1] = g.p[3];
+                        g.count = 2;
+                        MARL_TRY(launch_gemm_nt3(g, c.st, plan));
+                    } else {
+                        MARL_TRY(launch_gemm_nt3(g, c.st));
+                    }
+                } else if (no_dh) {
+                    GemmBatch rest{};
+                    rest.p[0] = gb.p[2];
+                    rest.p[1] = gb.p[3];
+                    rest.count = 2;
+                    MARL_TRY(launch_gemm_nt(rest, c.st, &gb));
                 } else {
                     MARL_TRY(launch_gemm_nt(gb, c.st));
                 }
             } else {
                 gb.p[2] = p;
                 gb.count = 3;
-                MARL_TRY(launch_gemm_nt(gb, c.st));
+                if (no_dh) {
+                    GemmBatch rest{};
+                    rest.p[0] = p;
+                    rest.count = 1;
+                    MARL_TRY(launch_gemm_nt(rest, c.st, &gb));
+                } else {
+                    MARL_TRY(launch_gemm_nt(gb, c.st));
+                }
             }
         }
         float* dad1 = c.at(c.e.DAD1) + (size_t)t * s_nm2;
@@ -1956,8 +2045,39 @@
         return MARL_ELIMIT;
     }
     const Dims& d = c.d;
-    MARL_TRY(launch_i64_to_i32(pos0, c.POSs(0), d.R * 2, c.st));
-    MARL_TRY(load_state(c, h0, c0, hc0, cc0, nullptr));
+    const bool lean = iter_lean();
+    if (lean) {
+        EpisodeBegin b{};
+        b.pos0 = pos0;
+        b.pos = c.POSs(0);
+        b.R = (int)d.R;
+        b.H = d.H;
+        b.W = d.W;
+        b.pe_W = c.wp(MARL_P_POS_W);
+        b.pe_b = c.wp(MARL_P_POS_B);
+        b.pe_gamma = c.wp(MARL_P_POS_LNW);
+        b.pe_beta = c.wp(MARL_P_POS_LNB);
+        b.pe_npos = c.at(c.e.NPOS, 0);
+        b.pe_z = c.at(c.e.ZPOS, 0);
+        b.pe_stats = c.at(c.e.STPOS, 0);
+        b.pe_out = c.at(c.e.U, 0) + d.nf + d.n_mo;
+        b.pe_ldz = d.ld_nd;
+        b.pe_ldo = d.ld_nin;
+        b.pe_nd = d.n_d;
+        b.copy[0] = {h0, c.Hs(0), d.n_b, d.ld_nb, 0};
+        b.copy[1] = {c0, c.Cs(0), d.n_b, d.ld_nb, 0};
+        b.copy[2] = {hc0, c.HCs(0), d.n_a, d.ld_na, 0};
+        b.copy[3] = {cc0, c.CCs(0), d.n_a, d.ld_na, 0};
+        b.copy[4] = {nullptr, c.MSGs(0), d.n_m, d.ld_nm, 0};
+        if (c.e.g3) {
+            b.image[0] = {h0, c.img(c.e.H3), d.n_b};
+            b.image[1] = {hc0, c.img(c.e.HC3), d.n_a};
+        }
+        MARL_TRY(launch_episode_begin(b, c.st));
+    } else {
+        MARL_TRY(launch_i64_to_i32(pos0, c.POSs(0), d.R * 2, c.st));
+        MARL_TRY(load_state(c, h0, c0, hc0, cc0, nullptr));
+    }
     StepIn in;
     in.img = img;
     in.img_u8 = cfg->img_u8 != 0;
@@ -1975,7 +2095,7 @@
             MARL_TRY(g_side.order(c2.st, c.st));
         else if (!decoded_ahead)
             MARL_TRY(step_decode(c, t));
-        MARL_TRY(step_pos_lstm(c, t, in, t > 0));
+        MARL_TRY(step_pos_lstm(c, t, in, t > 0 || lean));
         SampleArgs a;
         fill_sample_args(c, cfg, t, a);
         a.noise = noise ? noise + (size_t)t * d.R * d.nA : nullptr;
@@ -2400,6 +2520,28 @@
                        static_cast<hipStream_t>(stream), static_cast<const Counters*>(counters));
 }
 
+int marl_adam_pack_step(float* params, const float* grads, float* exp_avg, float* exp_avg_sq, int64_t n,
+                        int64_t step, float lr, float beta1, float beta2, float eps, float grad_scale,
+                        const void* counters, const marl_config* cfg, const float* const* params_host,
+                        void* weights_ws, size_t weights_ws_bytes, void* stream) {
+    Dims d;
+    MARL_TRY(make_dims(cfg, d));
+    if (!params_host || !weights_ws) {
+        set_error("adam_pack_step: null argument");
+        return MARL_EINVAL;
+    }
+    WLayout w;
+    make_wlayout(d, w);
+    if (weights_ws_bytes < w.total * sizeof(float)) {
+        set_error("adam_pack_step: weights workspace too small (%zu of %zu bytes)", weights_ws_bytes,
+                  w.total * sizeof(float));
+        return MARL_ESIZE;
+    }
+    MARL_TRY(marl_adam_step(params, grads, exp_avg, exp_avg_sq, n, step, lr, beta1, beta2, eps, grad_scale, counters,
+                            stream));
+    return pack_weights_once(d, w, params_host, static_cast<float*>(weights_ws), static_cast<hipStream_t>(stream));
+}
+
 }
 
 static int step_forward(const marl_config* cfg, const void* weights_ws, size_t weights_ws_bytes, void* episode_ws,
diff --git a/marlclassification_amd/csrc/gemm.hip b/marlclassification_amd/csrc/gemm.hip
--- a/marlclassification_amd/csrc/gemm.hip
+++ b/marlclassification_amd/csrc/gemm.hip
@@ -850,7 +850,7 @@
     return MARL_OK;
 }
 
-int launch_gemm_nt(const GemmBatch& batch, hipStream_t st) {
+int launch_gemm_nt(const GemmBatch& batch, hipStream_t st, const GemmBatch* plan_like) {
     if (batch.count < 1 || batch.count > kMaxGemmBatch) return MARL_EINVAL;
     int max_m = 0, max_n = 0;
     int64_t blocks128 = 0;
@@ -868,10 +868,19 @@
                     batch.count, batch.p[i].m, batch.p[i].n, batch.p[i].seg[0].k,
                     batch.p[i].nseg > 1 ? batch.p[i].seg[1].k : 0, batch.p[i].accumulate,
                     batch.p[i].bias != nullptr, batch.p[i].seg[0].lda, batch.p[i].ldc);
+    int plan_n = max_n;
+    if (plan_like) {
+        plan_n = 0;
+        blocks128 = 0;
+        for (int i = 0; i < plan_like->count; ++i) {
+            plan_n = plan_like->p[i].n > plan_n ? plan_like->p[i].n : plan_n;
+            blocks128 += cdiv(plan_like->p[i].m, 128) * cdiv(plan_like->p[i].n, 128);
+        }
+    }
     prof_before(1, st);
     if (split_mode()) {
-        MARL_TRY(launch_gemm_nt_split(batch, max_m, max_n, blocks128, st));
-    } else if (blocks128 >= 256 && max_n >= 96) {
+        MARL_TRY(launch_gemm_nt_split(batch, max_m, max_n, blocks128 >= 384 && plan_n >= 96, st));
+    } else if (blocks128 >= 256 && plan_n >= 96) {
         const int g = gemm_groups();
         dim3 grid((unsigned)cdiv(max_m, 128 * g), (unsigned)cdiv(max_n, 128), (unsigned)batch.count);
         if (g == 2)
diff --git a/marlclassification_amd/csrc/gemm3.hip b/marlclassification_amd/csrc/gemm3.hip
--- a/marlclassification_amd/csrc/gemm3.hip
+++ b/marlclassification_amd/csrc/gemm3.hip
@@ -1370,22 +1370,31 @@
     return MARL_OK;
 }
 
+int g3_nt_plan(const G3Batch& batch) {
+    int max_n = 0;
+    int64_t blocks128 = 0;
+    for (int i = 0; i < batch.count; ++i) {
+        max_n = batch.p[i].n > max_n ? batch.p[i].n : max_n;
+        blocks128 += cdiv(batch.p[i].m, 128) * cdiv(batch.p[i].n, 128);
+    }
+    int variant = tune_get("g3_nt_variant", 0);
+    if (!variant) {
+        variant = max_n >= 96 && blocks128 >= 256 ? 2 : 7;
+        if (variant == 2 && blocks128 >= 1024 && batch.count == 1 && max_n % 256 == 0) variant = 21;
+    }
+    return variant;
+}
+
 int launch_gemm_nt3(const G3Batch& batch, hipStream_t st, int variant) {
     if (batch.count < 1 || batch.count > kMaxG3) return MARL_EINVAL;
     int max_m = 0, max_n = 0;
-    int64_t blocks128 = 0;
     for (int i = 0; i < batch.count; ++i) {
         MARL_TRY(check_g3(batch.p[i], false));
         if (!batch.p[i].c) return MARL_EINVAL;
         max_m = batch.p[i].m > max_m ? batch.p[i].m : max_m;
         max_n = batch.p[i].n > max_n ? batch.p[i].n : max_n;
-        blocks128 += cdiv(batch.p[i].m, 128) * cdiv(batch.p[i].n, 128);
-    }
-    if (!variant) variant = tune_get("g3_nt_variant", 0);
-    if (!variant) {
-        variant = max_n >= 96 && blocks128 >= 256 ? 2 : 7;
-        if (variant == 2 && blocks128 >= 1024 && batch.count == 1 && max_n % 256 == 0) variant = 21;
-    }
+    }
+    if (!variant) variant = g3_nt_plan(batch);
     prof_before(1, st);
     int rc;
     if (variant == 1)
diff --git a/marlclassification_amd/csrc/gemm_split.hip b/marlclassification_amd/csrc/gemm_split.hip
--- a/marlclassification_amd/csrc/gemm_split.hip
+++ b/marlclassification_amd/csrc/gemm_split.hip
@@ -601,8 +601,8 @@
     return MARL_OK;
 }
 
-int launch_gemm_nt_split(const GemmBatch& batch, int max_m, int max_n, int64_t blocks128, hipStream_t st) {
-    if (blocks128 >= 384 && max_n >= 96) {
+int launch_gemm_nt_split(const GemmBatch& batch, int max_m, int max_n, bool wide, hipStream_t st) {
+    if (wide) {
         dim3 grid((unsigned)cdiv(max_m, 128), (unsigned)cdiv(max_n, 128), (unsigned)batch.count);
         return launch_nt_split_variant<128, false>(grid, batch, st);
     }
diff --git a/marlclassification_amd/csrc/rowops.hip b/marlclassification_amd/csrc/rowops.hip
--- a/marlclassification_amd/csrc/rowops.hip
+++ b/marlclassification_amd/csrc/rowops.hip
@@ -1204,6 +1204,37 @@
     return MARL_OK;
 }
 
+__device__ __forceinline__ void pos_embed_row(int64_t r, float p0, float p1, const float* __restrict__ W,
+                                              const float* __restrict__ b, const float* __restrict__ gamma,
+                                              const float* __restrict__ beta, float* __restrict__ npos4,
+                                              float* __restrict__ z, int ldz, float* __restrict__ stats,
+                                              float* __restrict__ out, int ldo, int nd) {
+    if (npos4) {
+        npos4[r * 4] = p0;
+        npos4[r * 4 + 1] = p1;
+    }
+    float* zr = z + r * ldz;
+    float s = 0.f;
+    for (int j = 0; j < nd; ++j) {
+        const float v = b[j] + p0 * W[4 * j] + p1 * W[4 * j + 1];
+        zr[j] = v;
+        s += v;
+    }
+    const float mean = s / (float)nd;
+    float q = 0.f;
+    for (int j = 0; j < nd; ++j) {
+        const float d = zr[j] - mean;
+        q += d * d;
+    }
+    const float rstd = 1.0f / sqrtf(q / (float)nd + 1e-5f);
+    if (stats) {
+        stats[r * 2] = mean;
+        stats[r * 2 + 1] = rstd;
+    }
+    float* orow = out + r * ldo;
+    for (int j = 0; j < nd; ++j) orow[j] = silu_f((zr[j] - mean) * rstd * gamma[j] + beta[j]);
+}
+
 __global__ void pos_embed_fwd_kernel(const int32_t* __restrict__ pos,
                                      const float* __restrict__ npos_in, int H, int W_,
                                      const float* __restrict__ W, const float* __restrict__ b,
@@ -1215,30 +1246,64 @@
     if (r >= rows) return;
     const float p0 = npos_in ? npos_in[r * 2] : (float)pos[r * 2] / (float)H;
     const float p1 = npos_in ? npos_in[r * 2 + 1] : (float)pos[r * 2 + 1] / (float)W_;
-    if (npos4) {
-        npos4[r * 4] = p0;
-        npos4[r * 4 + 1] = p1;
-    }
-    float* zr = z + r * ldz;
-    float s = 0.f;
-    for (int j = 0; j < nd; ++j) {
-        const float v = b[j] + p0 * W[4 * j] + p1 * W[4 * j + 1];
-        zr[j] = v;
-        s += v;
-    }
-    const float mean = s / (float)nd;
-    float q = 0.f;
-    for (int j = 0; j < nd; ++j) {
-        const float d = zr[j] - mean;
-        q += d * d;
-    }
-    const float rstd = 1.0f / sqrtf(q / (float)nd + 1e-5f);
-    if (stats) {
-        stats[r * 2] = mean;
-        stats[r * 2 + 1] = rstd;
-    }
-    float* orow = out + r * ldo;
-    for (int j = 0; j < nd; ++j) orow[j] = silu_f((zr[j] - mean) * rstd * gamma[j] + beta[j]);
+    pos_embed_row(r, p0, p1, W, b, gamma, beta, npos4, z, ldz, stats, out, ldo, nd);
+}
+
+__global__ __launch_bounds__(256) void episode_begin_kernel(const EpisodeBegin A) {
+    int part = 0, blk = (int)blockIdx.x;
+    while (blk >= A.blocks[part]) blk -= A.blocks[part++];
+    const int64_t idx = (int64_t)blk * 256 + threadIdx.x;
+    if (part == 0) {
+        if (idx >= A.R) return;
+        const int32_t y = (int32_t)A.pos0[idx * 2], x = (int32_t)A.pos0[idx * 2 + 1];
+        A.pos[idx * 2] = y;
+        A.pos[idx * 2 + 1] = x;
+        pos_embed_row(idx, (float)y / (float)A.H, (float)x / (float)A.W, A.pe_W, A.pe_b, A.pe_gamma, A.pe_beta,
+                      A.pe_npos, A.pe_z, A.pe_ldz, A.pe_stats, A.pe_out, A.pe_ldo, A.pe_nd);
+    } else if (part <= kBeginCopies) {
+        const EpisodeBegin::Copy& c = A.copy[part - 1];
+        const int cols = c.src ? c.n : c.ld;
+        if (c.vec4) {
+            if (idx < (int64_t)A.R * cols / 4)
+                reinterpret_cast<float4*>(c.dst)[idx] =
+                    c.src ? reinterpret_cast<const float4*>(c.src)[idx] : make_float4(0.f, 0.f, 0.f, 0.f);
+        } else if (idx < (int64_t)A.R * cols) {
+            const int64_t r = idx / cols;
+            const int j = (int)(idx - r * cols);
+            c.dst[r * c.ld + j] = c.src ? c.src[r * c.n + j] : 0.f;
+        }
+    } else {
+        const EpisodeBegin::Image& g = A.image[part - 1 - kBeginCopies];
+        const int steps = (g.k + 15) >> 4;
+        if (idx >= (int64_t)((A.R + 31) & ~31) * steps * 2) return;
+        const int64_t r = idx / (steps * 2);
+        const int k0 = (int)(idx - r * steps * 2) * 8;
+        float v[8];
+#pragma unroll
+        for (int q = 0; q < 8; ++q) v[q] = (r < A.R && k0 + q < g.k) ? g.src[r * g.k + k0 + q] : 0.f;
+        img_store8(g.dst + img_off(r, k0 >> 4, steps), k0, v);
+    }
+}
+
+int launch_episode_begin(EpisodeBegin& a, hipStream_t st) {
+    int64_t total = a.blocks[0] = (int)cdiv(a.R, 256);
+    for (int i = 0; i < kBeginCopies; ++i) {
+        EpisodeBegin::Copy& c = a.copy[i];
+        const int cols = c.src ? c.n : c.ld;
+        c.vec4 = (cols & 3) == 0 && (c.src ? c.n == c.ld : 1) && (reinterpret_cast<uintptr_t>(c.dst) & 15) == 0 &&
+                 (reinterpret_cast<uintptr_t>(c.src) & 15) == 0;
+        total += a.blocks[1 + i] = (int)cdiv((int64_t)a.R * cols / (c.vec4 ? 4 : 1), 256);
+    }
+    for (int i = 0; i < kBeginImages; ++i)
+        total += a.blocks[1 + kBeginCopies + i] =
+            a.image[i].dst ? (int)cdiv((int64_t)((a.R + 31) & ~31) * ((a.image[i].k + 15) >> 4) * 2, 256) : 0;
+    if (total >= (1ll << 31)) {
+        set_error("episode_begin: %lld workgroups", (long long)total);
+        return MARL_ELIMIT;
+    }
+    hipLaunchKernelGGL(episode_begin_kernel, dim3((unsigned)total), dim3(256), 0, st, a);
+    MARL_LAUNCH_CHECK();
+    return MARL_OK;
 }
 
 int launch_pos_embed_fwd(const int32_t* pos, const float* npos_in, int h, int w, const float* W,
@@ -1420,6 +1485,118 @@
     if (gx > 1024) gx = 1024;
     if (gx < 1) gx = 1;
     hipLaunchKernelGGL(permute_kernel, dim3((unsigned)gx, (unsigned)b.count), dim3(256), 0, st, b);
+    MARL_LAUNCH_CHECK();
+    return MARL_OK;
+}
+
+__device__ __forceinline__ float pack_wp_at(const PackParam& p, int r, int c) {
+    if (p.conv) {
+        const int ci = p.k / 9;
+        c = (c % ci) * 9 + c / ci;
+    }
+    return p.src[(int64_t)r * p.k + c];
+}
+template <bool T>
+__device__ __forceinline__ float pack_at(const PackParam& p, int r, int c) {
+    return T ? pack_wp_at(p, c, r) : pack_wp_at(p, r, c);
+}
+
+template <bool T>
+__device__ void pack_copy(const PackParam& p, float* dst, int rows, int cols, int ld, int64_t i0, int64_t stride) {
+    const int64_t tot = (int64_t)rows * cols;
+    for (int64_t idx = i0; idx < tot; idx += stride) {
+        const int r = (int)(idx / cols), c = (int)(idx % cols);
+        dst[(int64_t)r * ld + c] = pack_at<T>(p, r, c);
+    }
+}
+template <bool T>
+__device__ void pack_split(const PackParam& p, uint32_t* dst, int rows, int k, int64_t i0, int64_t stride) {
+    const int kt = (k + 31) / 32;
+    const int64_t tot = (int64_t)rows * kt * 16;
+    for (int64_t idx = i0; idx < tot; idx += stride) {
+        const int pr = (int)(idx & 15);
+        const int64_t rt = idx >> 4;
+        const int r = (int)(rt / kt);
+        const int kk = (int)(rt % kt) * 32 + pr * 2;
+        const float x = kk < k ? pack_at<T>(p, r, kk) : 0.f;
+        const float y = kk + 1 < k ? pack_at<T>(p, r, kk + 1) : 0.f;
+        uint32_t p0, p1, p2;
+        split_pair(x, y, p0, p1, p2);
+        uint32_t* o = dst + rt * 48 + pr;
+        o[0] = p0;
+        o[16] = p1;
+        o[32] = p2;
+    }
+}
+template <bool T>
+__device__ void pack_image(const PackParam& p, char* dst, int rows, int k, int64_t i0, int64_t stride) {
+    const int steps = (k + 15) >> 4;
+    const int64_t tot = (int64_t)((rows + 31) & ~31) * steps * 2;
+    for (int64_t idx = i0; idx < tot; idx += stride) {
+        const int r = (int)(idx / (steps * 2));
+        const int k0 = (int)(idx - (int64_t)r * steps * 2) * 8;
+        float v[8];
+#pragma unroll
+        for (int q = 0; q < 8; ++q) v[q] = (r < rows && k0 + q < k) ? pack_at<T>(p, r, k0 + q) : 0.f;
+        img_store8(dst + img_off(r, k0 >> 4, steps), k0, v);
+    }
+}
+
+__global__ __launch_bounds__(256) void pack_kernel(const PackTable B) {
+    const int job = B.job[blockIdx.y];
+    const PackParam& p = B.p[job >> 3];
+    const int64_t i0 = (int64_t)blockIdx.x * blockDim.x + threadIdx.x, stride = (int64_t)gridDim.x * blockDim.x;
+    switch (job & 7) {
+        case PO_WP:
+            if (p.k == 0) {
+                for (int64_t i = i0; i < p.n; i += stride) B.W[p.wp + i] = p.src[i];
+            } else {
+                pack_copy<false>(p, B.W + p.wp, p.n, p.k, (p.k + 3) & ~3, i0, stride);
+            }
+            break;
+        case PO_WT: pack_copy<true>(p, B.W + p.wt, p.k, p.n, (p.n + 3) & ~3, i0, stride); break;
+        case PO_WP3: pack_split<false>(p, reinterpret_cast<uint32_t*>(B.W + p.wp3), p.n, p.k, i0, stride); break;
+        case PO_WT3: pack_split<true>(p, reinterpret_cast<uint32_t*>(B.W + p.wt3), p.k, p.n, i0, stride); break;
+        case PO_WP3K: pack_image<false>(p, reinterpret_cast<char*>(B.W + p.wp3k), p.n, p.k, i0, stride); break;
+        case PO_WT3K: pack_image<true>(p, reinterpret_cast<char*>(B.W + p.wt3k), p.k, p.n, i0, stride); break;
+        case PO_WF: {
+            const int rows4 = (p.k / 16) * 4;
+            const int64_t tot = (int64_t)(p.n / 16) * rows4 * 64;
+            for (int64_t idx = i0; idx < tot; idx += stride) {
+                const int r = (int)(idx >> 6), c = (int)(idx & 63);
+                B.W[p.wf + idx] = pack_wp_at(p, (r / rows4) * 16 + (c >> 2), (r % rows4) * 4 + (c & 3));
+            }
+            break;
+        }
+        default: {
+            const float* b2 = B.p[(job >> 3) + 1].src;
+            for (int64_t i = i0; i < p.n; i += stride) B.W[p.wt + i] = p.src[i] + b2[i];
+        }
+    }
+}
+
+static int64_t pack_job_threads(const PackParam& p, int out) {
+    const int rows = (out & 1) ? p.k : p.n, k = (out & 1) ? p.n : p.k;
+    switch (out) {
+        case PO_WP: return p.k == 0 ? p.n : (int64_t)p.n * p.k;
+        case PO_WT: case PO_WF: return (int64_t)p.n * p.k;
+        case PO_WP3: case PO_WT3: return (int64_t)rows * ((k + 31) / 32) * 16;
+        case PO_WP3K: case PO_WT3K: return (int64_t)((rows + 31) & ~31) * ((k + 15) >> 4) * 2;
+        default: return p.n;
+    }
+}
+
+int launch_pack(const PackTable& t, hipStream_t st) {
+    if (t.count <= 0) return MARL_OK;
+    if (t.count > kMaxPackJobs) return MARL_EINVAL;
+    int64_t mx = 0;
+    for (int i = 0; i < t.count; ++i) {
+        const int64_t n = pack_job_threads(t.p[t.job[i] >> 3], t.job[i] & 7);
+        mx = n > mx ? n : mx;
+    }
+    int64_t gx = cdiv(mx, 256);
+    gx = gx > 64 ? 64 : (gx < 1 ? 1 : gx);
+    hipLaunchKernelGGL(pack_kernel, dim3((unsigned)gx, (unsigned)t.count), dim3(256), 0, st, t);
     MARL_LAUNCH_CHECK();
     return MARL_OK;
 }
diff --git a/marlclassification_amd/engine.py b/marlclassification_amd/engine.py
--- a/marlclassification_amd/engine.py
+++ b/marlclassification_amd/engine.py
@@ -590,14 +590,23 @@
         self, params: th.Tensor, grads: th.Tensor, exp_avg: th.Tensor, exp_avg_sq: th.Tensor,
         step: int, lr: float, betas: Tuple[float, float] = (0.9, 0.999), eps: float = 1e-8,
         grad_scale: float = 1.0, counters: Optional[th.Tensor] = None,
+        pack: Optional[Dict[str, th.Tensor]] = None,
     ) -> None:
         for t in (params, grads, exp_avg, exp_avg_sq):
             if not t.is_cuda or t.dtype != th.float32 or not t.is_contiguous():
                 raise RuntimeError("adam buffers must be contiguous fp32 GPU tensors")
-        check(self.lib.marl_adam_step(
-            params.data_ptr(), grads.data_ptr(), exp_avg.data_ptr(), exp_avg_sq.data_ptr(),
-            params.numel(), step, lr, betas[0], betas[1], eps, grad_scale, _ptr(counters),
-            _stream(self.device)))
+        args = (params.data_ptr(), grads.data_ptr(), exp_avg.data_ptr(), exp_avg_sq.data_ptr(),
+                params.numel(), step, lr, betas[0], betas[1], eps, grad_scale, _ptr(counters))
+        if pack is None:
+            check(self.lib.marl_adam_step(*args, _stream(self.device)))
+            return
+        assert self.cfg is not None, "configure() first"
+        wws = self.weights_ws()
+        check(self.lib.marl_adam_pack_step(*args, C.byref(self.cfg), self._table(pack), wws.data_ptr(), _nbytes(wws),
+                                           _stream(self.device)))
+        self.pack_generation += 1
+        self._packed_generation = self.weights_generation
+        self._packed_params = pack
 
     def step_forward(
         self, obs: th.Tensor, msg: th.Tensor, norm_pos: th.Tensor, h: th.Tensor, c: th.Tensor,
diff --git a/marlclassification_amd/fused.py b/marlclassification_amd/fused.py
--- a/marlclassification_amd/fused.py
+++ b/marlclassification_amd/fused.py
@@ -145,7 +145,7 @@
 
 
 def apply_update(eng: HipEngine, flat: "FlatParams", gp, gl, gv, g_probs, gviews, lr: float, allreduce,
-                 max_grad_norm: Optional[float], repack: Callable[[], None],
+                 max_grad_norm: Optional[float], pviews, packed: Callable[[], None],
                  comm: Optional[CommUpdate] = None) -> Optional[th.Tensor]:
     bucketed = hasattr(allreduce, "before_backward")
     if bucketed:
@@ -162,16 +162,16 @@
         norm = eng.grad_clip(flat.grads, max_grad_norm, grad_scale=scale)
         scale = 1.0
     flat.step += 1
-    eng.adam(flat.params, flat.grads, flat.exp_avg, flat.exp_avg_sq, flat.step, lr, grad_scale=scale)
+    eng.adam(flat.params, flat.grads, flat.exp_avg, flat.exp_avg_sq, flat.step, lr, grad_scale=scale, pack=pviews)
+    packed()
     if comm is not None:
         comm.step(eng.comm_live, allreduce, rank_scale)
-    repack()
     return norm
 
 
 def ppo_epochs_loop(eng: HipEngine, flat: "FlatParams", out: EpisodeTensors, y: th.Tensor, bufs, epochs: int,
                     clip: float, beta: float, lr: float, allreduce, max_grad_norm: Optional[float], gviews,
-                    replay: Callable[[], EpisodeTensors], repack: Callable[[], None],
+                    replay: Callable[[], EpisodeTensors], pviews, packed: Callable[[], None],
                     comm: Optional[CommUpdate] = None) -> Optional[th.Tensor]:
     gp, gl, gv, _, _, advn, ret = bufs[:7]
     gpr = bufs[7] if beta > 0 else None
@@ -184,7 +184,7 @@
                 raise RuntimeError("PPO replay wrote over the rollout's log-probabilities (persistent output "
                                    "tensors?): the ratios would all be 1")
         eng.ppo_loss(cur, y, old_logp, advn, ret, clip, bufs, entropy_coef=beta)
-        norm = apply_update(eng, flat, gp, gl, gv, gpr, gviews, lr, allreduce, max_grad_norm, repack, comm)
+        norm = apply_update(eng, flat, gp, gl, gv, gpr, gviews, lr, allreduce, max_grad_norm, pviews, packed, comm)
     return norm
 
 
@@ -229,6 +229,9 @@
 
     def pack(self) -> None:
         self.engine.pack(self._pviews)
+        self._packed()
+
+    def _packed(self) -> None:
         self._packed_gen = self.engine.weights_generation
 
     def rollout(self, img: th.Tensor, draws: EpisodeDraws, train: bool,
@@ -279,8 +282,7 @@
                     gp, gl, gv, scalars = bufs[:4]
                     eng.episode_backward(gp, gl, gv, gviews, g_probs=bufs[5] if beta > 0 else None)
                     eng.adam(self.flat.params, self.flat.grads, self.flat.exp_avg,
-                             self.flat.exp_avg_sq, 1, self.lr, counters=cnt)
-                    eng.pack(self._pviews)
+                             self.flat.exp_avg_sq, 1, self.lr, counters=cnt, pack=self._pviews)
                     eng.counters_tick(cnt, self.lr)
                 except BaseException:
                     try:
@@ -317,7 +319,7 @@
         bufs = eng.a2c_loss(out, y, self.gamma, 0, self._loss_bufs, entropy_coef=beta)
         gp, gl, gv, scalars = bufs[:4]
         apply_update(eng, self.flat, gp, gl, gv, bufs[5] if beta > 0 else None, self._gviews, self.lr,
-                     self.allreduce, None, self.pack, self._comm())
+                     self.allreduce, None, self._pviews, self._packed, self._comm())
         return out, scalars
 
     def _comm(self) -> Optional[CommUpdate]:
@@ -339,7 +341,7 @@
             eng, self.flat, out, y, bufs, self.ppo_epochs, self.ppo_clip, beta, self.lr, self.allreduce,
             self.max_grad_norm, self._gviews,
             replay=lambda: self.rollout(img, draws, True, forced_actions=out.step_actions, probs=ent),
-            repack=self.pack, comm=self._comm())
+            pviews=self._pviews, packed=self._packed, comm=self._comm())
         if norm is not None:
             self.last_grad_norm = norm
         return out, bufs[3]
diff --git a/marlclassification_amd/networks/models.py b/marlclassification_amd/networks/models.py
--- a/marlclassification_amd/networks/models.py
+++ b/marlclassification_amd/networks/models.py
@@ -304,6 +304,7 @@
             eng.pack(flat.param_views())
             self.__packed_token[id(eng)] = token
 
-    def mark_updated(self, eng: HipEngine) -> None:
-        eng.pack(self.flat_state().param_views())
+    def mark_updated(self, eng: HipEngine, packed: bool = False) -> None:
+        if not packed:
+            eng.pack(self.flat_state().param_views())
         self.__packed_token = {id(eng): self._version_token() + (eng.weights_token(),)}
diff --git a/marlclassification_amd/training/trainer.py b/marlclassification_amd/training/trainer.py
--- a/marlclassification_amd/training/trainer.py
+++ b/marlclassification_amd/training/trainer.py
@@ -99,7 +99,8 @@
         self.__exact_phases(lambda phase: eng.a2c_loss(out, y, self.__gamma, phase, bufs, entropy_coef=beta))
         flat = model.flat_state()
         apply_update(eng, flat, bufs[0], bufs[1], bufs[2], bufs[5] if ent else None, flat.grad_views(), self.__lr,
-                     self.__allreduce, None, lambda: model.mark_updated(eng), self.__comm())
+                     self.__allreduce, None, flat.param_views(), lambda: model.mark_updated(eng, packed=True),
+                     self.__comm())
         return out, bufs[3]
 
     def __train_step_ppo(self, x: th.Tensor, y: th.Tensor,
@@ -118,7 +119,7 @@
             self.__max_grad_norm, flat.grad_views(),
             replay=lambda: sampler.run_episode_raw(img, train=True, draws=draws, probs=ent,
                                                    forced=out.step_actions)[1],
-            repack=lambda: model.mark_updated(eng), comm=self.__comm())
+            pviews=flat.param_views(), packed=lambda: model.mark_updated(eng, packed=True), comm=self.__comm())
         if norm is not None:
             self.__grad_norm = norm
         return out, bufs[3]
```

After: 9.367 million agent-env-steps/s, median of 6. About the same (+0.2%).
